# samuel-watson/glmmrMCML

Hardware: AMD Instinct MI355X
Metric: MCML iters/sec x m chains (simlik evals/sec) (higher is better)
Workload: dtype f64

## Files before the change

glmmrmcml_amd/api.py:

```python
import ctypes as C

import numpy as np

from . import _lib

c_dp = C.POINTER(C.c_double)
c_ip = C.POINTER(C.c_int32)

REDUCE_FN = C.CFUNCTYPE(C.c_int, C.c_void_p, C.c_void_p, C.c_int)


class Problem(C.Structure):
    _fields_ = [("cov", c_ip), ("cov_rows", C.c_int), ("data", c_dp), ("data_len", C.c_int),
                ("eff_range", c_dp), ("eff_len", C.c_int), ("Z", c_dp), ("X", c_dp), ("y", c_dp),
                ("n", C.c_int), ("Q", C.c_int), ("P", C.c_int), ("family", C.c_char_p),
                ("link", C.c_char_p)]


class DevOpts(C.Structure):
    _fields_ = [("device", C.c_int), ("stream", C.c_void_p), ("rank", C.c_int), ("world", C.c_int),
                ("reduce", REDUCE_FN), ("reduce_user", C.c_void_p)]


class HmcOpts(C.Structure):
# ... 62 lines not shown

def get_default_la_operator():
    return _LA_OP_NAME[_lib.lib().glmmr_mcml_get_default_la_operator()]


def la_component_launches():
    f = _lib.lib().glmmr_mcml_dbg_la_component_launches
    f.restype = C.c_longlong
    return int(f())


class _default_la_operator:

    def __init__(self, operator):
        self.operator = operator

    def __enter__(self):
        if self.operator is not None:
            self.prev = get_default_la_operator()
            set_default_la_operator(self.operator)

    def __exit__(self, *a):
        if self.operator is not None:
            set_default_la_operator(self.prev)


def traj_launches():
    f = _lib.lib().glmmr_mcml_dbg_traj_launches
    f.restype = C.c_longlong
    return int(f())


def dbg_dgemm_at(A, B, C0, K, alpha=1.0, beta=0.0, tile=-1):
    A = np.array(A, dtype=np.float64, order="F"); B = np.array(B, dtype=np.float64, order="F")
    K2 = K + (K & 1)
    assert A.shape[0] == K2 and B.shape[0] == K2, "operands hold round_up(K, 2) rows"
    M, N = A.shape[1], B.shape[1]
    out = B if C0 is None else np.array(C0, dtype=np.float64, order="F")
    assert C0 is None or out.shape == (M, N)
    _lib.check(_lib.lib().glmmr_mcml_dbg_dgemm_at(M, N, int(K), _p(A), K2, _p(B), K2, C.c_double(alpha), C.c_double(beta),
                                                  _p(out), out.shape[0], int(tile)))
    return out[:M]


def rccl_unique_id():
    buf = (C.c_ubyte * 128)()
    _lib.check(_lib.lib().glmmr_mcml_rccl_unique_id(buf))
    return bytes(buf)


def _f(a):
    return np.asfortranarray(np.asarray(a, dtype=np.float64))


def _i(a):
    return np.asfortranarray(np.asarray(a, dtype=np.int32))


def _p(a):
    return None if a is None else a.ctypes.data_as(c_dp)


class Context:

    def __init__(self, cov, data, eff_range, Z=None, X=None, y=None, family=None, link=None,
                 device=0, stream=None, rank=0, world=1, reduce=None):
        L = _lib.lib()
        self._cov = _i(cov)
        assert self._cov.ndim == 2 and self._cov.shape[1] == 5, "cov must be rows x 5"
        self._data = _f(data).ravel()
        self._eff = _f(eff_range).ravel()
        p = Problem()
        p.cov = self._cov.ctypes.data_as(c_ip); p.cov_rows = self._cov.shape[0]
        p.data = _p(self._data); p.data_len = self._data.size
        p.eff_range = _p(self._eff); p.eff_len = self._eff.size
        self.n = self.P = 0
        if Z is not None:
            self._Z = _f(Z); self._X = _f(X); self._y = _f(y).ravel()
            self.n, self.Q = self._Z.shape
            self.P = self._X.shape[1]
            assert self._X.shape[0] == self.n and self._y.size == self.n
            p.Z = _p(self._Z); p.X = _p(self._X); p.y = _p(self._y)
            p.n = self.n; p.Q = self.Q; p.P = self.P
            p.family = family.encode(); p.link = link.encode()
        o = DevOpts()
        o.device = device; o.stream = stream; o.rank = rank; o.world = world
        self._reduce_cb = REDUCE_FN(reduce) if reduce is not None else REDUCE_FN()
        o.reduce = self._reduce_cb
        self._h = C.c_void_p()
        self._world = int(world)
        _lib.check(L.glmmr_mcml_ctx_create(C.byref(p), C.byref(o), C.byref(self._h)))
        self.family, self.link = family, link
        if Z is None:
            self.Q = int(sum(self._cov[np.r_[True, self._cov[1:, 0] != self._cov[:-1, 0]], 1]))
        self.mcols = 0

    def close(self):
        if getattr(self, "_h", None) is not None and self._h.value:
            _lib.lib().glmmr_mcml_ctx_destroy(self._h)
            self._h = C.c_void_p()

    def __del__(self):
        try:
            self.close()
        except Exception:
            pass

    def __enter__(self):
        return self

    def __exit__(self, *a):
        self.close()

    def comm_init_rccl(self, unique_id, rank, world):
        buf = (C.c_ubyte * 128).from_buffer_copy(bytes(unique_id))
        _lib.check(_lib.lib().glmmr_mcml_ctx_comm_init_rccl(self._h, buf, int(rank), int(world)))
        self._world = int(world)

    def comm_allreduce(self, vals):
        v = np.ascontiguousarray(vals, dtype=np.float64).copy()
        _lib.check(_lib.lib().glmmr_mcml_ctx_comm_allreduce(self._h, _p(v), v.size))
        return v

    def comm_stats(self):
        calls = C.c_longlong(); dbl = C.c_longlong(); nat = C.c_int()
        _lib.check(_lib.lib().glmmr_mcml_ctx_comm_stats(self._h, C.byref(calls), C.byref(dbl), C.byref(nat)))
        return dict(calls=calls.value, doubles=dbl.value, native=bool(nat.value))

    def set_u(self, u, niter=None):
        u = _f(u)
        if u.ndim == 1:
            u = u.reshape(-1, 1, order="F")
        self.mcols = u.shape[1]
        _lib.check(_lib.lib().glmmr_mcml_set_u(self._h, _p(u), u.shape[0], u.shape[1],
                                               u.shape[1] if niter is None else niter))

    def get_u(self):
        u = np.zeros((self.Q, self.mcols), order="F")
        _lib.check(_lib.lib().glmmr_mcml_get_u(self._h, _p(u), self.Q))
        return u

    def get_u_all(self, world=None):
        w = int(world) if world else max(1, int(getattr(self, "_world", 1)))
        u = np.zeros((self.Q, self.mcols * w), order="F")
        nc = C.c_int()
        _lib.check(_lib.lib().glmmr_mcml_get_u_all(self._h, _p(u), self.Q, C.byref(nc)))
        assert nc.value == u.shape[1], (nc.value, u.shape)
        return u

    def shard_stats(self):
        out = (C.c_longlong * 6)()
        _lib.check(_lib.lib().glmmr_mcml_ctx_shard_stats(self._h, out))
        return dict(gathers=out[0], gather_doubles=out[1], theta_rounds=out[2], theta_evals_own=out[3],
                    theta_evals_all=out[4])

    def emulate_world(self, world, mode):
        _lib.check(_lib.lib().glmmr_mcml_dbg_emulate_world(self._h, int(world), int(mode)))
        self._world = int(world) if world and world > 1 else 1

    def mvn_ll(self, theta):
        theta = _f(theta).ravel()
        out = C.c_double()
        _lib.check(_lib.lib().glmmr_mcml_ctx_mvn_ll(self._h, _p(theta), C.byref(out)))
        return out.value

    def mvn_ll_batch(self, thetas):
        th = np.ascontiguousarray(np.atleast_2d(np.asarray(thetas, dtype=np.float64)))
        out = np.zeros(th.shape[0])
        _lib.check(_lib.lib().glmmr_mcml_ctx_mvn_ll_batch(self._h, _p(th), th.shape[0], _p(out)))
        return out

    def mvn_workspace(self, cand=-1):
        f = _lib.lib().glmmr_mcml_dbg_mvn_workspace
        dims = (C.c_int * 4)()
        _lib.check(f(self._h, int(cand), None, 0, None, 0, dims))
        d, m = dims[0], dims[2]
        L = np.zeros((d, d), order="F"); X = np.zeros((m, d), order="F")
        _lib.check(f(self._h, int(cand), _p(L), d, _p(X), m, dims))
        return L, X, tuple(dims)

    def dbg_chol(self, A, B=None, linv=True):
        A = np.array(A, dtype=np.float64, order="F")
        n = A.shape[0]
        assert A.shape == (n, n)
        out = dict(A=A)
        m = 0
        if B is not None:
            B = _f(B).reshape(n, -1, order="F")
            m = B.shape[1]
            for k in ("fwd", "trans", "potrs"):
                out[k] = np.zeros((n, m), order="F")
        nblk = (n + 127) // 128
        li = np.zeros((nblk, 128, 128)) if linv else None
        _lib.check(_lib.lib().glmmr_mcml_dbg_chol(self._h, n, _p(A), n, m, _p(B), n, _p(out.get("fwd")), _p(out.get("trans")),
                                                  _p(out.get("potrs")), _p(li)))
        if linv:
            out["linv"] = li.transpose(0, 2, 1)
        return out

    def gen_D(self, theta, chol=False):
        theta = _f(theta).ravel()
        D = np.zeros((self.Q, self.Q), order="F")
        _lib.check(_lib.lib().glmmr_mcml_ctx_gen_D(self._h, _p(theta), int(chol), _p(D), self.Q))
        return D

    def loglik(self, beta, var_par):
        beta = _f(beta).ravel()
        out = C.c_double()
        _lib.check(_lib.lib().glmmr_mcml_ctx_loglik(self._h, _p(beta), C.c_double(var_par), C.byref(out)))
        return out.value

    def mcnr(self, beta, var_par):
        beta = _f(beta).ravel()
        bout = np.zeros(self.P); sig = C.c_double()
        stats = np.zeros(self.P * self.P + self.P + 1)
        _lib.check(_lib.lib().glmmr_mcml_ctx_mcnr(self._h, _p(beta), C.c_double(var_par), _p(bout),
                                                  C.byref(sig), _p(stats)))
        P = self.P
        return dict(beta=bout, sigma=sig.value, XtWX=stats[:P * P].reshape(P, P, order="F"),
                    XtWr=stats[P * P:P * P + P], sigma_sum=stats[-1])

    def update_L(self, theta):
        theta = _f(theta).ravel()
        _lib.check(_lib.lib().glmmr_mcml_ctx_update_L(self._h, _p(theta)))

    def set_L(self, Lmat):
        Lmat = _f(Lmat)
        _lib.check(_lib.lib().glmmr_mcml_ctx_set_L(self._h, _p(Lmat), Lmat.shape[0]))

    def log_prob_grad(self, beta, var_par, V):
        beta = _f(beta).ravel(); V = _f(V)
        lp = np.zeros(V.shape[1]); G = np.zeros_like(V, order="F")
        _lib.check(_lib.lib().glmmr_mcml_dbg_log_prob_grad(self._h, _p(beta), C.c_double(var_par), _p(V),
                                                           V.shape[1], _p(lp), _p(G)))
        return lp, G

    def hmc_sample(self, beta, var_par, warmup, nsamp, lambda_, max_steps, target_accept, seed,
                   chains=1, chain_offset=0, iter_idx=0, adapt=100, inj_init=None, inj_mom=None,
                   want_trace=False):
        beta = _f(beta).ravel()
        o = HmcOpts(warmup, nsamp, adapt, lambda_, max_steps, target_accept, chains, chain_offset)
        d = HmcDiag()
        ii = None if inj_init is None else _f(inj_init)
        im = None if inj_mom is None else _f(inj_mom)
        total = warmup + (nsamp if chains == 1 else -(-nsamp // chains))
        flags = np.zeros((chains, total), dtype=np.uint8, order="F") if want_trace else None
        probs = np.zeros((chains, total), order="F") if want_trace else None
        ncols = C.c_int()
        _lib.check(_lib.lib().glmmr_mcml_ctx_hmc_sample(
            self._h, _p(beta), C.c_double(var_par), C.byref(o), C.c_uint64(seed), C.c_uint32(iter_idx),
            _p(ii), _p(im), None if flags is None else flags.ctypes.data_as(C.POINTER(C.c_uint8)),
            _p(probs), C.byref(d), C.byref(ncols)))
        self.mcols = ncols.value
        diag = dict(accept_rate=d.accept_rate, mean_e=d.mean_e, min_e=d.min_e, max_e=d.max_e,
                    max_steps_used=d.max_steps_used, leapfrog_total=d.leapfrog_total)
        if want_trace:
            return diag, flags, probs
        return diag

    def nuts_sample(self, beta, var_par, warmup, nsamp, seed, chains=1, chain_offset=0, iter_idx=0, max_treedepth=10,
                    adapt_delta=0.8, stepsize=1.0, want_trace=False, metric="diag_e"):
        beta = _f(beta).ravel()
        o = NutsOpts(warmup, nsamp, max_treedepth, adapt_delta, stepsize, chains, chain_offset,
                     {"diag_e": 0, "unit_e": 1}[metric])
        d = NutsDiag()
        total = warmup + -(-nsamp // chains)
        c_ip_ = C.POINTER(C.c_int)
        tr = None
        if want_trace:
            tr = dict(depth=np.zeros((chains, total), dtype=np.int32, order="F"),
                      nleap=np.zeros((chains, total), dtype=np.int32, order="F"),
                      eps=np.zeros((chains, total), order="F"), accept=np.zeros((chains, total), order="F"))
        ncols = C.c_int()
        _lib.check(_lib.lib().glmmr_mcml_ctx_nuts_sample(
            self._h, _p(beta), C.c_double(var_par), C.byref(o), C.c_uint64(seed), C.c_uint32(iter_idx),
            None if tr is None else tr["depth"].ctypes.data_as(c_ip_), None if tr is None else tr["nleap"].ctypes.data_as(c_ip_),
            None if tr is None else _p(tr["eps"]), None if tr is None else _p(tr["accept"]), C.byref(d), C.byref(ncols)))
        self.mcols = ncols.value
        diag = dict(mean_e=d.mean_e, min_e=d.min_e, max_e=d.max_e, divergent=d.divergent, treedepth_hits=d.treedepth_hits,
                    batched_leapfrogs=d.batched_leapfrogs, stepsize_search_leapfrogs=d.stepsize_search_leapfrogs,
                    packs=d.packs)
        return (diag, tr) if want_trace else diag

    def _ext(self, seed, chains, maxfun, theta_batch=0):
        return Ext(int(seed or 0), int(chains or 1), int(maxfun or 0), 0, int(theta_batch or 0))

    def npar(self):
        return _lib.lib().glmmr_mcml_ctx_npar(self._h)

    def theta_log(self, enable=None, last=None):
        w = self.npar() + 1
        n = C.c_int()
        _lib.check(_lib.lib().glmmr_mcml_dbg_theta_log(self._h, -1, None, 0, C.byref(n)))
        rows = n.value if last is None else min(int(last), n.value)
        out = np.zeros((rows, w))
        _lib.check(_lib.lib().glmmr_mcml_dbg_theta_log(self._h, -1 if enable is None else int(bool(enable)),
                                                       _p(out) if rows else None, rows, C.byref(n)))
        return out

    def last_kernels(self):
        names = {-1: None, 0: "skinny", 1: "band", 2: "dlds", 3: "reg", 4: "sparse", 5: "component", 6: "exact"}
        f = C.c_int(); b = C.c_int()
        _lib.check(_lib.lib().glmmr_mcml_ctx_last_kernels(self._h, C.byref(f), C.byref(b)))
        return names[f.value], names[b.value]

    def band_plan(self, chains, which="fwd"):
        out = (C.c_int * 10)()
# ... 339 lines not shown
```

glmmrmcml_amd/csrc/cabi.hip:

```cpp
#include "../../include/glmmr_mcml_c.h"
#include "ctx.h"
#include <algorithm>
#include <atomic>
#include <random>
#include "sparse_plan.h"

using namespace mcml;


namespace mcml {
int hmc_sample(Ctx& c, const double* beta, double var_par, const glmmr_mcml_hmc_opts* o, uint64_t seed,
               uint32_t iter_idx, const double* inj_init, const double* inj_mom, uint8_t* flags_out,
               double* probs_out, glmmr_mcml_hmc_diag* diag, int* ncols_out);
int nuts_sample(Ctx& c, const double* beta, double var_par, const glmmr_mcml_nuts_opts* o, uint64_t seed, uint32_t iter_idx,
                int* depth_out, int* nleap_out, double* eps_out, double* accept_out, glmmr_mcml_nuts_diag* diag,
                int* ncols_out);
bool hmc_exact_applicable(const Ctx& c);
int hmc_exact_sample(Ctx& c, const double* beta, double var_par, const glmmr_mcml_hmc_opts* o, uint64_t seed, uint32_t iter_idx,
                     const double* inj_z, glmmr_mcml_hmc_diag* diag, int* ncols_out);
}

static std::atomic<int> g_default_traj{-1};
static int default_trajectory()
{
// ... 230 lines not shown
    if (!sp.active) return MCML_OK;
    out12[1] = sp.factored ? 1 : 0; out12[2] = sp.W; out12[3] = sp.nnz; out12[4] = sp.nnz_z; out12[5] = sp.nnz_l;
    out12[6] = sp.nblk; out12[7] = sp.max_blk; out12[8] = cm_long_rows(c) ? 1 : 0; out12[9] = cm_fuse_width(c);
    return MCML_OK;
}

extern "C" int glmmr_mcml_set_default_trajectory(int mode)
{
    MCML_REQUIRE(mode == 0 || mode == 1, "set_default_trajectory: mode must be 0 (per step) or 1 (component)");
    g_default_traj.store(mode);
    return MCML_OK;
}

extern "C" int glmmr_mcml_get_default_trajectory(void) { return default_trajectory(); }

namespace mcml { long long cm_traj_launch_count(); }
extern "C" long long glmmr_mcml_dbg_traj_launches(void) { return cm_traj_launch_count(); }

extern "C" int glmmr_mcml_ctx_set_trajectory(glmmr_mcml_ctx* h, int mode)
{
    MCML_REQUIRE(h && (mode == 0 || mode == 1), "set_trajectory: mode must be 0 (per step) or 1 (component)");
    h->c.traj_mode = mode;
    return MCML_OK;
}

extern "C" int glmmr_mcml_dbg_component_plan(glmmr_mcml_ctx* h, int chains, long long* out11)
{
    MCML_REQUIRE(h && chains >= 1 && out11, "dbg_component_plan: bad argument");
    const Ctx& c = h->c;
    const ComponentPlan& p = c.cp.plan;
    for (int i = 0; i < 11; ++i) out11[i] = 0;
    out11[0] = c.traj_mode; out11[9] = CP_MAX_VARS;
    if (!c.sp.active) return MCML_OK;
    const bool feasible = c.cp.ready && p.feasible;
    out11[1] = feasible ? 1 : 0; out11[2] = (feasible && c.traj_mode == 1) ? 1 : 0;
    out11[3] = p.ncomp; out11[4] = p.max_vars; out11[5] = p.max_rows; out11[6] = p.empty_comps;
    if (!feasible) return MCML_OK;
    const int waves = cp_waves(p, cp_forced_waves());
    out11[7] = p.nitems(); out11[8] = waves; out11[10] = cp_lds_bytes(p.max_vars, waves);
    return MCML_OK;
}

extern "C" int glmmr_mcml_set_default_draws(int mode)
{
    MCML_REQUIRE(mode == 0 || mode == 1, "set_default_draws: mode must be 0 (hmc) or 1 (exact)");
    g_default_draws.store(mode);
    return MCML_OK;
}

extern "C" int glmmr_mcml_get_default_draws(void) { return default_draws(); }

extern "C" int glmmr_mcml_ctx_set_draws(glmmr_mcml_ctx* h, int mode)
{
    MCML_REQUIRE(h && (mode == 0 || mode == 1), "set_draws: mode must be 0 (hmc) or 1 (exact)");
    h->c.draws_mode = mode;
    return MCML_OK;
}

extern "C" int glmmr_mcml_dbg_draws_plan(glmmr_mcml_ctx* h, int* out4)
{
    MCML_REQUIRE(h && out4, "dbg_draws_plan: null argument");
    const Ctx& c = h->c;
    const long long bytes = (long long)sizeof(double) * pad_ld(c.Q) * c.Q;
    out4[0] = c.draws_mode; out4[1] = hmc_exact_applicable(c) ? 1 : 0; out4[2] = c.Q;
    out4[3] = bytes > 0x7fffffffLL ? 0x7fffffff : (int)bytes;
    return MCML_OK;
}

extern "C" int glmmr_mcml_ctx_exact_sample(glmmr_mcml_ctx* h, const double* beta, double var_par,
                                           const glmmr_mcml_hmc_opts* opts, uint64_t seed, uint32_t iter_idx,
                                           const double* inj_z, glmmr_mcml_hmc_diag* diag, int* ncols_out)
{
    MCML_REQUIRE(h && beta && opts, "exact_sample: null argument");
    MCML_HIP(hipSetDevice(h->c.device));
    return hmc_exact_sample(h->c, beta, var_par, opts, seed, iter_idx, inj_z, diag, ncols_out);
}

extern "C" int glmmr_mcml_dbg_exact_phases(glmmr_mcml_ctx* h, int enable, double* out5)
{
    MCML_REQUIRE(h, "dbg_exact_phases: null context");
    if (out5) for (int i = 0; i < 5; ++i) out5[i] = h->c.exact.ms[i];
    h->c.exact.prof = enable != 0;
    return MCML_OK;
}

extern "C" int glmmr_mcml_dbg_trsm_compare(glmmr_mcml_ctx* h, int m, int reps, double* trans_ms, double* fwd_ms)
{
    MCML_REQUIRE(h && m > 0 && reps > 0 && reps <= 64, "dbg_trsm_compare: bad argument");
    Ctx& c = h->c;
    MCML_HIP(hipSetDevice(c.device));
    MCML_REQUIRE(c.last_kernel[0] == KERNEL_EXACT && c.exact.M.d() && c.exact.M.rows == c.Q && c.U.d() && c.mcols >= m,
                 "dbg_trsm_compare: the last sampler call on this context must be an exact one with at least %d columns", m);
    DevMat T;
    MCML_TRY(T.alloc(c.Q, m));
    hipEvent_t e0, e1;
    MCML_HIP(hipEventCreate(&e0)); MCML_HIP(hipEventCreate(&e1));
    int rc = MCML_OK;
    for (int which = 0; which < 2 && rc == MCML_OK; ++which) {
        double* out = which ? fwd_ms : trans_ms;
        if (!out) continue;
        std::vector<float> ms;
        for (int r = 0; r < reps && rc == MCML_OK; ++r) {
            if (hipMemcpy2DAsync(T.d(), sizeof(double) * T.ld, c.U.d(), sizeof(double) * c.U.ld, sizeof(double) * c.Q, m,
                                 hipMemcpyDeviceToDevice, c.stream) != hipSuccess) { rc = MCML_EHIP; break; }
            (void)hipEventRecord(e0, c.stream);
            rc = which ? trsm_left_lower(c, c.exact.M.d(), c.exact.M.ld, c.Q, T.d(), T.ld, m)
                       : trsm_left_lower_trans(c, c.exact.M.d(), c.exact.M.ld, c.Q, T.d(), T.ld, m);
            (void)hipEventRecord(e1, c.stream);
            if (hipEventSynchronize(e1) != hipSuccess) rc = MCML_EHIP;
            float t = 0;
            if (rc == MCML_OK && hipEventElapsedTime(&t, e0, e1) == hipSuccess) ms.push_back(t);
        }
        if (rc == MCML_OK && !ms.empty()) { std::sort(ms.begin(), ms.end()); *out = ms[ms.size() / 2]; }
    }
    (void)hipEventDestroy(e0); (void)hipEventDestroy(e1);
    if (rc == MCML_EHIP) set_error("dbg_trsm_compare: HIP call failed");
    return rc;
}

extern "C" int glmmr_mcml_set_default_la_operator(int mode)
{
    MCML_REQUIRE(mode >= 0 && mode <= 2, "set_default_la_operator: mode must be 0 (dense), 1 (component) or 2 (component_wide)");
    g_default_la.store(mode);
    return MCML_OK;
}

extern "C" int glmmr_mcml_get_default_la_operator(void) { return default_la_operator(); }

extern "C" int glmmr_mcml_ctx_set_la_operator(glmmr_mcml_ctx* h, int mode)
{
    MCML_REQUIRE(h && mode >= 0 && mode <= 2, "set_la_operator: mode must be 0 (dense), 1 (component) or 2 (component_wide)");
    h->c.la_mode = mode;
    return MCML_OK;
}

namespace mcml { long long la_component_launch_count(); }
extern "C" long long glmmr_mcml_dbg_la_component_launches(void) { return la_component_launch_count(); }

extern "C" int glmmr_mcml_dbg_la_plan(glmmr_mcml_ctx* h, long long* out8)
{
    MCML_REQUIRE(h && out8, "dbg_la_plan: null argument");
    const Ctx& c = h->c;
    const ComponentPlan& p = c.cp.plan;
    const long long v[8] = {c.la_mode, c.la_last_op, p.ncomp, p.max_vars, p.max_rows, c.la_launches, c.la_dense_bytes, c.la_waves};
    for (int i = 0; i < 8; ++i) out8[i] = v[i];
    return MCML_OK;
}

extern "C" int glmmr_mcml_ctx_shard_stats(glmmr_mcml_ctx* h, long long* out6)
{
    MCML_REQUIRE(h && out6, "shard_stats: null argument");
    const Ctx& c = h->c;
    out6[0] = c.gather_calls; out6[1] = c.gather_doubles; out6[2] = c.theta_rounds; out6[3] = c.theta_evals_own;
    out6[4] = c.theta_evals_all; out6[5] = 0;
    return MCML_OK;
}

extern "C" int glmmr_mcml_dbg_emulate_world(glmmr_mcml_ctx* h, int world, int mode)
{
    MCML_REQUIRE(h, "emulate_world: null context");
    Ctx& c = h->c;
    MCML_REQUIRE(c.world <= 1 && !c.comm, "emulate_world: the context is rank %d of a real group of %d", c.rank, c.world);
    MCML_REQUIRE(world <= 1 || mode == 1 || mode == 2, "emulate_world: mode must be 1 (record) or 2 (replay)");
    if (world <= 1) { c.emu_world = 0; c.emu_mode = 0; c.emu_trace.clear(); c.emu_pos = 0; c.uall_valid = false; return MCML_OK; }
    if (c.emu_world != world) { c.emu_trace.clear(); c.uall_valid = false; }
    c.emu_world = world; c.emu_mode = mode; c.emu_pos = 0;
    if (mode == 1) c.emu_trace.clear();
    return MCML_OK;
}

extern "C" int glmmr_mcml_ctx_mvn_ll(glmmr_mcml_ctx* h, const double* theta, double* out)
{
    MCML_REQUIRE(h && theta && out, "mvn_ll: null argument");
    Ctx& c = h->c;
    MCML_HIP(hipSetDevice(c.device));
    double s = 0;
    MCML_TRY(mvn_loglik_sum(c, theta, &s));
    double tot[2] = {s, (double)c.mcols};
    MCML_TRY(allreduce_host(c, tot, 2));
    *out = tot[0] / tot[1];
    return MCML_OK;
}

extern "C" int glmmr_mcml_ctx_mvn_ll_batch(glmmr_mcml_ctx* h, const double* thetas, int k, double* out)
{
    MCML_REQUIRE(h && thetas && out && k >= 1 && k <= 64, "mvn_ll_batch: bad argument");
    Ctx& c = h->c;
    MCML_HIP(hipSetDevice(c.device));
    MCML_REQUIRE(c.mcols > 0 && c.U.d(), "mvn_ll: no samples set");
    std::vector<double> tot(k + 1, 0.0);
    std::vector<int> rcs(k, 0);
    MCML_TRY(mvn_loglik_batch(c, thetas, k, c.U.d(), c.U.ld, c.mcols, tot.data(), rcs.data()));
    for (int j = 0; j < k; ++j) if (rcs[j] == MCML_ENOTPD) tot[j] = NAN;
    tot[k] = (double)c.mcols;
    MCML_TRY(allreduce_host(c, tot.data(), k + 1));
    for (int j = 0; j < k; ++j) out[j] = tot[j] / tot[k];
    return MCML_OK;
}

extern "C" int glmmr_mcml_ctx_gen_D(glmmr_mcml_ctx* h, const double* theta, int chol, double* out, int ldo)
{
    MCML_REQUIRE(h && theta && out, "gen_D: null argument");
    Ctx& c = h->c;
    MCML_REQUIRE(ldo >= c.Q, "gen_D: ldo too small");
    MCML_HIP(hipSetDevice(c.device));
    MCML_TRY(mvn_gen_L(c, theta, chol != 0));
    return download_matrix(out, ldo, c.L.d(), c.L.ld, c.Q, c.Q, c.stream);
}

int mcml::mcnr_finish(int P, const double* stats, const double* beta, double* beta_out, double* sigma_out)
{
    const double m = stats[P * P + P + 1];
    MCML_REQUIRE(m > 0, "mcnr: no samples");
    std::vector<double> A(stats, stats + P * P), B((size_t)P * P, 0.0);
    for (auto& v : A) v *= (double)1 / m;
    for (int i = 0; i < P; i++) B[i + (size_t)i * P] = 1.0;
    for (int c = 0; c < P; c++) {
        int p = c; double best = fabs(A[c + (size_t)c * P]);
        for (int i = c + 1; i < P; i++) if (fabs(A[i + (size_t)c * P]) > best) { best = fabs(A[i + (size_t)c * P]); p = i; }
        if (best == 0.0 || best != best) { set_error("mcnr: X'WX is singular"); return MCML_ESINGULAR; }
        if (p != c) for (int j = 0; j < P; j++) { std::swap(A[c + (size_t)j * P], A[p + (size_t)j * P]); std::swap(B[c + (size_t)j * P], B[p + (size_t)j * P]); }
        double d = A[c + (size_t)c * P];
        for (int j = 0; j < P; j++) { A[c + (size_t)j * P] /= d; B[c + (size_t)j * P] /= d; }
        for (int i = 0; i < P; i++) if (i != c) {
            double f = A[i + (size_t)c * P];
            if (f != 0.0) for (int j = 0; j < P; j++) { A[i + (size_t)j * P] -= f * A[c + (size_t)j * P]; B[i + (size_t)j * P] -= f * B[c + (size_t)j * P]; }
        }
    }
    for (int a = 0; a < P; a++) {
        double inc = 0;
        for (int b = 0; b < P; b++) inc += B[a + (size_t)b * P] * (stats[P * P + b] / m);
        beta_out[a] = beta[a] + inc;
    }
    *sigma_out = stats[P * P + P] / m;
    return MCML_OK;
}

extern "C" int glmmr_mcml_ctx_loglik(glmmr_mcml_ctx* h, const double* beta, double var_par, double* out)
{
    MCML_REQUIRE(h && beta && out, "loglik: null argument");
    Ctx& c = h->c;
    MCML_HIP(hipSetDevice(c.device));
    MCML_TRY(model_update_beta(c, beta));
    double s = 0;
    MCML_TRY(model_loglik_sum(c, var_par, &s));
    double tot[2] = {s, (double)c.niter};
    MCML_TRY(allreduce_host(c, tot, 2));
    *out = tot[0] / tot[1];
    return MCML_OK;
}

extern "C" int glmmr_mcml_ctx_mcnr(glmmr_mcml_ctx* h, const double* beta, double var_par,
                                   double* beta_out, double* sigma_out, double* stats_out)
{
    MCML_REQUIRE(h && beta && beta_out && sigma_out, "mcnr: null argument");
    Ctx& c = h->c;
    MCML_HIP(hipSetDevice(c.device));
    MCML_TRY(model_update_beta(c, beta));
    std::vector<double> st((size_t)c.P * c.P + c.P + 2);
    MCML_TRY(model_mcnr_stats(c, var_par, st.data()));
    if (stats_out) memcpy(stats_out, st.data(), sizeof(double) * ((size_t)c.P * c.P + c.P + 1));
    return mcnr_finish(c.P, st.data(), beta, beta_out, sigma_out);
}

extern "C" int glmmr_mcml_ctx_update_L(glmmr_mcml_ctx* h, const double* theta)
{
    MCML_REQUIRE(h && theta, "update_L: null argument");
    Ctx& c = h->c;
    MCML_HIP(hipSetDevice(c.device));
    MCML_TRY(mvn_gen_L(c, theta, true));
    MCML_TRY(model_update_L(c));
    return c.sync();
}

extern "C" int glmmr_mcml_ctx_set_L(glmmr_mcml_ctx* h, const double* L, int ldl)
{
    MCML_REQUIRE(h && L, "set_L: null argument");
    Ctx& c = h->c;
    MCML_REQUIRE(ldl >= c.Q, "set_L: ldl too small");
    MCML_HIP(hipSetDevice(c.device));
    MCML_TRY(upload_matrix(c.L, L, c.Q, c.Q, ldl, c.stream));
    c.have_L = true;
    c.l_foreign = true;
    MCML_TRY(model_update_L(c));
    return c.sync();
}

extern "C" int glmmr_mcml_ctx_hmc_sample(glmmr_mcml_ctx* h, const double* beta, double var_par,
                                         const glmmr_mcml_hmc_opts* opts, uint64_t seed, uint32_t iter_idx,
                                         const double* inj_init, const double* inj_mom, uint8_t* flags_out,
                                         double* probs_out, glmmr_mcml_hmc_diag* diag, int* ncols_out)
{
    MCML_REQUIRE(h && beta && opts, "hmc_sample: null argument");
    MCML_HIP(hipSetDevice(h->c.device));
    return hmc_sample(h->c, beta, var_par, opts, seed, iter_idx, inj_init, inj_mom, flags_out, probs_out,
                      diag, ncols_out);
}

extern "C" int glmmr_mcml_ctx_nuts_sample(glmmr_mcml_ctx* h, const double* beta, double var_par,
                                          const glmmr_mcml_nuts_opts* opts, uint64_t seed, uint32_t iter_idx,
                                          int* depth_out, int* nleap_out, double* eps_out, double* accept_out,
                                          glmmr_mcml_nuts_diag* diag, int* ncols_out)
{
    MCML_REQUIRE(h && beta && opts, "nuts_sample: null argument");
    MCML_HIP(hipSetDevice(h->c.device));
    return nuts_sample(h->c, beta, var_par, opts, seed, iter_idx, depth_out, nleap_out, eps_out, accept_out, diag,
                       ncols_out);
}

extern "C" int glmmr_mcml_dbg_log_prob_grad(glmmr_mcml_ctx* h, const double* beta, double var_par,
                                            const double* V, int ncols, double* lp, double* G)
{
    MCML_REQUIRE(h && beta && V && lp && G && ncols > 0, "log_prob_grad: bad argument");
    MCML_HIP(hipSetDevice(h->c.device));
    return hmc_dbg_log_prob_grad(h->c, beta, var_par, V, ncols, lp, G);
}

extern "C" int glmmr_mcml_mvn_ll(const int32_t* cov, int cov_rows, const double* data, int data_len,
                                 const double* eff_range, int eff_len, const double* gamma, int ngamma,
                                 const double* u, int Q, int m, double* out)
{
    glmmr_mcml_problem p{};
    p.cov = cov; p.cov_rows = cov_rows; p.data = data; p.data_len = data_len;
    p.eff_range = eff_range; p.eff_len = eff_len; p.Q = Q;
    glmmr_mcml_ctx* h = nullptr;
    MCML_TRY(glmmr_mcml_ctx_create(&p, nullptr, &h));
    int rc = MCML_OK;
    if (ngamma < h->c.cov.npar) {
        set_error("mvn_ll: %d covariance parameters given, the functions need %d", ngamma, h->c.cov.npar);
        rc = MCML_EINVAL;
    }
    if (!rc) rc = glmmr_mcml_set_u(h, u, Q, m, m);
    if (!rc) rc = glmmr_mcml_ctx_mvn_ll(h, gamma, out);
    glmmr_mcml_ctx_destroy(h);
    return rc;
}

namespace mcml {
int drv_optim(Ctx& c, const double* start, int nstart, int trace, int mcnr, const glmmr_mcml_ext* e,
              double* beta, double* theta, double* sigma);
int drv_simlik(Ctx& c, const double* start, int nstart, int trace, const glmmr_mcml_ext* e, double* beta,
               double* theta, double* sigma);
int drv_hess(Ctx& c, const double* start, int nstart, double tol, int trace, double* H);
int drv_aic(Ctx& c, const double* beta_par, int nbeta, const double* cov_par, int ncov, double* out);
int drv_full(Ctx& c, const double* start, int nstart, int mcnr, int m, int maxiter, int warmup, double tol,
             int verbose, double lambda, int trace, int refresh, int maxsteps, double target_accept,
             const glmmr_mcml_ext* e, double* beta_out, double* theta_out, double* sigma_out,
             int* converged_out, int* iters_out, glmmr_mcml_hmc_diag* last_diag);
int drv_la(Ctx& c, const double* start, int nstart, int nr, int usehess, double tol, int verbose, int trace,
           int maxiter, const glmmr_mcml_ext* e, double* beta, double* theta, double* sigma, double* se, double* u,
           int* converged, int* iters);
int drv_la_probe(Ctx& c, const double* start, int nstart, int kind, const double* v, double var_par,
                 const double* par, int npar, double* out, double* v_out, double* beta_out, double* sigma_out);
}

extern "C" int glmmr_mcml_sample_cols(int m, int chains)
{
    if (m <= 0) return 0;
    if (chains <= 1) return m + 1;
    return chains * ((m + chains - 1) / chains);
}

extern "C" int glmmr_mcml_ctx_profile(glmmr_mcml_ctx* h, int enable, int reset, double* out8)
{
    MCML_REQUIRE(h, "profile: null context");
    Ctx& c = h->c;
    KernelProf& p = c.prof;
    if (out8) {
        out8[0] = p.ms[0]; out8[1] = (double)p.cnt[0]; out8[2] = p.ms[1]; out8[3] = (double)p.cnt[1];
        const double C = (double)c.hmc.C, dense = 2.0 * c.n * (double)c.Q * C;
        double ff = dense, fb = dense, kind = 0;
        if (c.sp.active) { ff = fb = 2.0 * (double)c.sp.nnz * C; kind = 2; }
        else {
            if (c.band_fwd) { ff = 2.0 * 80.0 * 32.0 * (double)c.band_fwd_tiles * C; kind = 1; }
            if (c.band_bwd) { fb = 2.0 * 80.0 * 32.0 * (double)c.band_bwd_tiles * C; kind = 1; }
        }
        out8[4] = ff; out8[5] = fb; out8[6] = dense; out8[7] = kind;
    }
    if (reset) for (int i = 0; i < 4; ++i) { p.ms[i] = 0; p.cnt[i] = 0; p.seen[i] = 0; }
    if (enable && !p.on) {
        MCML_HIP(hipSetDevice(c.device));
        while (p.ev.size() < 4096) { hipEvent_t e; if (hipEventCreate(&e) != hipSuccess) { (void)hipGetLastError(); break; } p.ev.push_back(e); }
    }
    p.on = enable != 0;
    return MCML_OK;
}

extern "C" int glmmr_mcml_ctx_profile_launches(glmmr_mcml_ctx* h, long long* fwd, long long* bwd)
{
    MCML_REQUIRE(h, "profile_launches: null context");
    if (fwd) *fwd = h->c.prof.seen[0];
    if (bwd) *bwd = h->c.prof.seen[1];
    return MCML_OK;
}

extern "C" int glmmr_mcml_ctx_ncols(glmmr_mcml_ctx* h) { return h ? h->c.mcols : 0; }
extern "C" int glmmr_mcml_ctx_npar(glmmr_mcml_ctx* h) { return h ? h->c.cov.npar : 0; }

extern "C" int glmmr_mcml_ctx_optim(glmmr_mcml_ctx* h, const double* start, int nstart, int trace, int mcnr,
                                    const glmmr_mcml_ext* ext, double* beta, double* theta, double* sigma)
{
    MCML_REQUIRE(h && start && beta && theta && sigma, "optim: null argument");
    MCML_REQUIRE(h->c.n > 0, "optim: context has no model");
    MCML_HIP(hipSetDevice(h->c.device));
    return drv_optim(h->c, start, nstart, trace, mcnr, ext, beta, theta, sigma);
}

extern "C" int glmmr_mcml_ctx_simlik(glmmr_mcml_ctx* h, const double* start, int nstart, int trace,
                                     const glmmr_mcml_ext* ext, double* beta, double* theta, double* sigma)
{
    MCML_REQUIRE(h && start && beta && theta && sigma, "simlik: null argument");
    MCML_REQUIRE(h->c.n > 0, "simlik: context has no model");
    MCML_HIP(hipSetDevice(h->c.device));
    return drv_simlik(h->c, start, nstart, trace, ext, beta, theta, sigma);
}

extern "C" int glmmr_mcml_ctx_hess(glmmr_mcml_ctx* h, const double* start, int nstart, double tol, int trace,
                                   double* H)
{
    MCML_REQUIRE(h && start && H, "hess: null argument");
    MCML_REQUIRE(h->c.n > 0 && tol > 0, "hess: context has no model / bad tol");
    MCML_HIP(hipSetDevice(h->c.device));
    return drv_hess(h->c, start, nstart, tol, trace, H);
}

extern "C" int glmmr_mcml_ctx_aic(glmmr_mcml_ctx* h, const double* beta_par, int nbeta, const double* cov_par,
                                  int ncov, double* out)
{
    MCML_REQUIRE(h && beta_par && cov_par && out, "aic: null argument");
    MCML_REQUIRE(h->c.n > 0, "aic: context has no model");
    MCML_HIP(hipSetDevice(h->c.device));
    return drv_aic(h->c, beta_par, nbeta, cov_par, ncov, out);
}

extern "C" int glmmr_mcml_ctx_full(glmmr_mcml_ctx* h, const double* start, int nstart, int mcnr, int m,
                                   int maxiter, int warmup, double tol, int verbose, double lambda, int trace,
                                   int refresh, int maxsteps, double target_accept, const glmmr_mcml_ext* ext,
                                   double* beta, double* theta, double* sigma, int* converged, int* iters,
                                   glmmr_mcml_hmc_diag* diag)
{
    MCML_REQUIRE(h && start && beta && theta && sigma, "mcml_full: null argument");
    MCML_REQUIRE(h->c.n > 0, "mcml_full: context has no model");
    MCML_HIP(hipSetDevice(h->c.device));
    return drv_full(h->c, start, nstart, mcnr, m, maxiter, warmup, tol, verbose, lambda, trace, refresh, maxsteps,
                    target_accept, ext, beta, theta, sigma, converged, iters, diag);
}

extern "C" int glmmr_mcml_ctx_la(glmmr_mcml_ctx* h, const double* start, int nstart, int nr, int usehess, double tol,
                                 int verbose, int trace, int maxiter, const glmmr_mcml_ext* ext, double* beta,
                                 double* theta, double* sigma, double* se, double* u, int* converged, int* iters)
{
    MCML_REQUIRE(h && start && beta && theta && sigma, "mcml_la: null argument");
    MCML_HIP(hipSetDevice(h->c.device));
    return drv_la(h->c, start, nstart, nr, usehess, tol, verbose, trace, maxiter, ext, beta, theta, sigma, se, u,
                  converged, iters);
}

extern "C" int glmmr_mcml_dbg_leaf_profile(glmmr_mcml_ctx* h, unsigned long long* out10)
{
    MCML_REQUIRE(h && out10, "leaf_profile: null argument");
    return potrf_leaf_profile(h->c, out10);
}

extern "C" int glmmr_mcml_dbg_la_probe(glmmr_mcml_ctx* h, const double* start, int nstart, int kind, const double* v,
                                       double var_par, const double* par, int npar, double* out, double* v_out,
                                       double* beta_out, double* sigma_out)
{
    MCML_REQUIRE(h && start, "la_probe: null argument");
    MCML_REQUIRE(kind >= 0 && kind <= 3, "la_probe: kind %d", kind);
    MCML_REQUIRE(kind == 3 ? (v_out && beta_out && sigma_out) : (par && out && npar > 0), "la_probe: null output");
    MCML_HIP(hipSetDevice(h->c.device));
    return drv_la_probe(h->c, start, nstart, kind, v, var_par, par, npar, out, v_out, beta_out, sigma_out);
}

namespace {
struct CtxGuard {
    glmmr_mcml_ctx* h = nullptr;
    ~CtxGuard() { if (h) glmmr_mcml_ctx_destroy(h); }
};
int open_ctx(const glmmr_mcml_problem* prob, const glmmr_mcml_ext* ext, CtxGuard& g)
{
    glmmr_mcml_dev_opts o{};
    o.device = ext ? ext->device : 0; o.world = 1;
    return glmmr_mcml_ctx_create(prob, &o, &g.h);
}
int check_pattern(const Ctx& c, const int32_t* Ap, const int32_t* Ai, int nnz)
{
    MCML_REQUIRE(Ap && Ai && nnz >= 0, "sparse: null pattern");
    std::vector<int> blk(c.Q);
    for (int b = 0; b < c.cov.B; ++b) for (int k = 0; k < c.cov.blocks[b].dim; ++k) blk[c.cov.blocks[b].matstart + k] = b;
    MCML_REQUIRE(Ap[0] == 0 && Ap[c.Q] == nnz, "sparse: Ap does not describe %d columns / %d entries", c.Q, nnz);
    for (int j = 0; j < c.Q; ++j)
        for (int p = Ap[j]; p < Ap[j + 1]; ++p) {
            MCML_REQUIRE(Ai[p] >= 0 && Ai[p] < c.Q, "sparse: row index out of range");
            MCML_REQUIRE(blk[Ai[p]] == blk[j], "sparse: entry (%d,%d) lies outside the covariance blocks", Ai[p], j);
        }
    return MCML_OK;
}
}

extern "C" int glmmr_mcml_optim(const glmmr_mcml_problem* prob, const double* u, int ucols, const double* start,
                                int nstart, int trace, int mcnr, const glmmr_mcml_ext* ext, double* beta,
                                double* theta, double* sigma)
{
    CtxGuard g;
    MCML_TRY(open_ctx(prob, ext, g));
    MCML_TRY(glmmr_mcml_set_u(g.h, u, prob->Q, ucols, ucols));
    return glmmr_mcml_ctx_optim(g.h, start, nstart, trace, mcnr, ext, beta, theta, sigma);
}

extern "C" int glmmr_mcml_simlik(const glmmr_mcml_problem* prob, const double* u, int ucols, const double* start,
                                 int nstart, int trace, const glmmr_mcml_ext* ext, double* beta, double* theta,
                                 double* sigma)
{
    CtxGuard g;
    MCML_TRY(open_ctx(prob, ext, g));
    MCML_TRY(glmmr_mcml_set_u(g.h, u, prob->Q, ucols, ucols));
    return glmmr_mcml_ctx_simlik(g.h, start, nstart, trace, ext, beta, theta, sigma);
}

static int sparse_factor_nnz(const Ctx& c)
{
    long nnz = 0;
    for (const auto& b : c.cov.blocks) if (!b.all_gr) nnz += (long)b.dim * (b.dim - 1) / 2;
    return (int)nnz;
}

extern "C" int glmmr_mcml_sparse_factor_nnz(const int32_t* cov, int cov_rows, const double* data, int data_len)
{
    CovSpec cs;
    if (cs.parse(cov, cov_rows, data, data_len, nullptr, 0)) return -1;
    long nnz = 0;
    for (const auto& b : cs.blocks) if (!b.all_gr) nnz += (long)b.dim * (b.dim - 1) / 2;
    return (int)nnz;
}

static int sparse_factor(Ctx& c, const double* theta, int32_t* Lp, int32_t* Li, double* Lx, double* D)
{
    MCML_TRY(mvn_gen_L(c, theta, true));
    std::vector<double> blk;
    int nz = 0;
    for (const auto& b : c.cov.blocks) {
        blk.assign((size_t)b.dim * b.dim, 0.0);
        MCML_TRY(download_matrix(blk.data(), b.dim, c.L.at(b.matstart, b.matstart), c.L.ld, b.dim, b.dim, c.stream));
        for (int j = 0; j < b.dim; ++j) {
            const double d = blk[j + (size_t)j * b.dim];
            Lp[b.matstart + j] = nz;
            D[b.matstart + j] = d * d;
            if (!b.all_gr)
                for (int i = j + 1; i < b.dim; ++i) { Li[nz] = b.matstart + i; Lx[nz] = blk[i + (size_t)j * b.dim] / d; ++nz; }
        }
    }
    Lp[c.Q] = nz;
    return MCML_OK;
}

extern "C" int glmmr_mcml_optim_sparse(const glmmr_mcml_problem* prob, const int32_t* Ap, const int32_t* Ai,
                                       int nnz, const double* u, int ucols, const double* start, int nstart,
                                       int trace, int mcnr, const glmmr_mcml_ext* ext, double* beta, double* theta,
                                       double* sigma, int32_t* Lp, int32_t* Li, double* Lx, double* D, int lcap)
{
    CtxGuard g;
    MCML_TRY(open_ctx(prob, ext, g));
    MCML_TRY(check_pattern(g.h->c, Ap, Ai, nnz));
    MCML_TRY(glmmr_mcml_set_u(g.h, u, prob->Q, ucols, ucols));
    MCML_TRY(glmmr_mcml_ctx_optim(g.h, start, nstart, trace, mcnr, ext, beta, theta, sigma));
    if (Lp && Li && Lx && D) {
        MCML_REQUIRE(lcap >= sparse_factor_nnz(g.h->c), "optim_sparse: factor needs %d entries, %d given",
                     sparse_factor_nnz(g.h->c), lcap);
        MCML_TRY(sparse_factor(g.h->c, theta, Lp, Li, Lx, D));
    }
    return MCML_OK;
}

extern "C" int glmmr_mcml_simlik_sparse(const glmmr_mcml_problem* prob, const int32_t* Ap, const int32_t* Ai,
                                        int nnz, const double* u, int ucols, const double* start, int nstart,
// ... 174 lines not shown
```

glmmrmcml_amd/csrc/covspec.h:

```cpp
#pragma once
#include "common.h"

namespace mcml {

constexpr int MAX_COV_PAR = 32;
struct ThetaArg { double v[MAX_COV_PAR]; };

struct CovBlock {
    int dim;
    int r0, r1;
    int ncol;
    int doff;
    int matstart;
    int all_gr;
};

struct CovSpec {
    int rows = 0, B = 0, N = 0, npar = 0;
    std::vector<int32_t> cov;
    std::vector<double> data;
    std::vector<double> eff;
    std::vector<CovBlock> blocks;

    static int fn_npar(int fn) {
        static const int t[15] = {0, 1, 1, 1, 2, 2, 1, 2, 2, 2, 2, 2, 2, 2, 1};
        return (fn >= 1 && fn <= 14) ? t[fn] : -1;
    }
    static bool fn_built(int fn) { return fn == 1 || fn == 2 || fn == 3 || fn == 4 || fn == 7 || fn == 14; }
    int c(int r, int col) const { return cov[r + (size_t)col * rows]; }

    int parse(const int32_t* cov_, int rows_, const double* data_, int data_len,
              const double* eff_, int eff_len)
    {
        MCML_REQUIRE(cov_ && rows_ > 0, "cov: empty");
        rows = rows_;
        cov.assign(cov_, cov_ + (size_t)rows * 5);
        eff.assign(eff_ ? eff_ : nullptr, eff_ ? eff_ + (eff_len > 0 ? eff_len : 0) : nullptr);
        blocks.clear();
        N = 0; npar = 0;
        int r = 0;
        size_t doff = 0;
        while (r < rows) {
            CovBlock b{};
            b.dim = c(r, 1); b.r0 = r; b.ncol = 0; b.all_gr = 1; b.matstart = N; b.doff = (int)doff;
            MCML_REQUIRE(b.dim > 0, "cov row %d: block dimension %d", r, b.dim);
            int id = c(r, 0);
            while (r < rows && c(r, 0) == id) {
                int fn = c(r, 2), nv = c(r, 3), pi = c(r, 4);
                MCML_REQUIRE(c(r, 1) == b.dim, "cov row %d: dimension differs within block", r);
                if (fn_npar(fn) < 0 || !fn_built(fn)) {
                    set_error("cov row %d: covariance function id %d is not built (gr, fexp0, ar1, "
                              "sqexp, fexp, sqexp0 only)", r, fn);
                    return MCML_EUNSUPPORTED;
                }
                MCML_REQUIRE(nv >= 0 && pi >= 0, "cov row %d: negative field", r);
                MCML_REQUIRE(pi + fn_npar(fn) <= MAX_COV_PAR, "more than %d covariance parameters", MAX_COV_PAR);
                if (pi + fn_npar(fn) > npar) npar = pi + fn_npar(fn);
                if (fn != 1) b.all_gr = 0;
                b.ncol += nv;
                ++r;
            }
            b.r1 = r;
            doff += (size_t)b.dim * b.ncol;
            N += b.dim;
            blocks.push_back(b);
        }
        B = (int)blocks.size();
        MCML_REQUIRE((size_t)data_len >= doff, "data has %d values, the blocks need %zu", data_len, doff);
        data.assign(data_, data_ + doff);
        return MCML_OK;
    }
};

__host__ __device__ static inline double cov_term(int fn, double dist, const double* g, double val)
{
    switch (fn) {
    case 1: return (dist == 0) ? val * g[0] * g[0] : 0.0;
    case 2: return val * exp(-1.0 * dist / g[0]);
    case 3: return val * pow(g[0], dist);
    case 4: return val * g[0] * exp(-1.0 * dist * dist / (g[1] * g[1]));
    case 7: return val * g[0] * exp(-1.0 * dist / g[1]);
    case 14: return val * exp(-1.0 * dist * dist / (g[0] * g[0]));
    }
    return val;
}

}
```

glmmrmcml_amd/csrc/ctx.h:

```cpp
#pragma once
#include "common.h"
#include "covspec.h"
#include "band_plan.h"
#include "component_plan.h"
#include "step_ahead.h"

namespace mcml {

constexpr int CHOL_NB = 128;
constexpr int SMALL_BLOCK = 32;

typedef int (*reduce_fn)(void* user, double* dev_buf, int n);

enum { KERNEL_SKINNY = 0, KERNEL_BAND = 1, KERNEL_DLDS = 2, KERNEL_REG = 3, KERNEL_SPARSE = 4, KERNEL_COMPONENT = 5,
       KERNEL_EXACT = 6 };

struct StepRing {
    static constexpr int SLOTS = StepAhead::SLOTS;
    unsigned long long* h = nullptr;
    unsigned long long* d = nullptr;
    unsigned seq = 0;
    StepRing() = default;
    StepRing(const StepRing&) = delete;
    StepRing& operator=(const StepRing&) = delete;
// ... 57 lines not shown
        if (nev >= ev.size())
            for (int i = 0; i < 512; ++i) { hipEvent_t e; if (hipEventCreate(&e) != hipSuccess) return -1; ev.push_back(e); }
        return (int)nev++;
    }
    int begin(hipStream_t s, int k, bool chain = false) {
        if (!on) return -1;
        ++seen[k];
        if (skip) return -1;
        int st = (chain && last_stop >= 0) ? last_stop : fresh();
        if (st < 0) return -1;
        if (!(chain && last_stop >= 0)) (void)hipEventRecord(ev[st], s);
        if (used >= kind.size()) { kind.resize(used + 512); e0.resize(used + 512); e1.resize(used + 512); }
        kind[used] = k; e0[used] = st; e1[used] = -1;
        return (int)used++;
    }
    void end(hipStream_t s, int slot) {
        if (slot < 0) return;
        const int sp = fresh();
        if (sp < 0) return;
        (void)hipEventRecord(ev[sp], s);
        e1[slot] = sp; last_stop = sp;
    }
    void unchain() { last_stop = -1; }
    void collect() {
        for (size_t i = 0; i < used; ++i) {
            float t = 0;
            if (e1[i] >= 0 && hipEventElapsedTime(&t, ev[e0[i]], ev[e1[i]]) == hipSuccess) { ms[kind[i]] += t; cnt[kind[i]] += 1; }
        }
        used = 0; nev = 0; last_stop = -1;
    }
    ~KernelProf() { for (auto e : ev) (void)hipEventDestroy(e); }
};

struct CholGraph {
    hipGraphExec_t exec = nullptr;
    const double* A = nullptr; const double* linv = nullptr; int lda = 0, n = 0, extra = 0, seen = 0;
    long long used = 0;
    hipGraph_t tmpl = nullptr;
    hipEvent_t t0 = nullptr, t1 = nullptr;
    float eager_ms = 0.f, best_ms = 0.f;
    hipGraphExec_t best = nullptr;
    int tries = 0, trial_launches = 0;
    bool timed = false, settled = false;
    void release() {
        if (best && best != exec) (void)hipGraphExecDestroy(best);
        best = nullptr;
        if (exec) { (void)hipGraphExecDestroy(exec); exec = nullptr; }
        if (tmpl) { (void)hipGraphDestroy(tmpl); tmpl = nullptr; }
        if (t0) { (void)hipEventDestroy(t0); t0 = nullptr; }
        if (t1) { (void)hipEventDestroy(t1); t1 = nullptr; }
    }
};
struct CholGraphCache {
    static constexpr int CAP = 2;
    std::vector<CholGraph> g;
    long long tick = 0;
    void clear() { for (CholGraph& e : g) e.release(); g.clear(); }
    ~CholGraphCache() { clear(); }
    CholGraphCache() = default;
    CholGraphCache(const CholGraphCache&) = delete;
    CholGraphCache& operator=(const CholGraphCache&) = delete;
    CholGraphCache(CholGraphCache&& o) noexcept : g(std::move(o.g)), tick(o.tick) { o.g.clear(); }
    CholGraphCache& operator=(CholGraphCache&& o) noexcept { if (this != &o) { clear(); g = std::move(o.g); tick = o.tick; o.g.clear(); } return *this; }
    CholGraph& find(const double* A, const double* linv, int lda, int n, int extra) {
        ++tick;
        for (CholGraph& e : g)
            if (e.A == A && e.linv == linv && e.lda == lda && e.n == n && e.extra == extra) { e.used = tick; return e; }
        size_t old = 0;
        for (size_t i = 1; i < g.size(); ++i)
            if (g[i].used < g[old].used) old = i;
        if ((int)g.size() >= CAP) {
            g[old].release();
            g[old] = CholGraph();
            std::swap(g[old], g.back());
        } else g.push_back(CholGraph());
        CholGraph& e = g.back();
        e.A = A; e.linv = linv; e.lda = lda; e.n = n; e.extra = extra; e.seen = 0; e.used = tick;
        return e;
    }
};

struct ExactState {
    DevMat M, T;
    DevBuf b;
    bool prof = false;
    double ms[5] = {0, 0, 0, 0, 0};
};

struct Ctx {
    int device = 0;
    hipStream_t stream = nullptr;
    bool own_stream = false;

    int n = 0, Q = 0, P = 0, flink = 0, link_code = 0;
    int z_width = 0;
    DevBuf z_idx, z_val;
    std::vector<int> h_zidx; std::vector<double> h_zval;
    SparseZL sp;
    ComponentDev cp;
    int traj_mode = 0;
    int draws_mode = 0;
    ExactState exact;
    bool no_sparse_zl = false;
    int la_mode = 0;
    int la_last_op = 0;
    int la_waves = 0;
    long long la_launches = 0, la_dense_bytes = 0;
    bool l_foreign = false;
    CovSpec cov;
    DevMat Z, X;
    DevBuf y;
    DevBuf d_cov, d_data, d_blocks, d_rowblock;

    DevMat U;
    int mcols = 0;
    int niter = 0;
    int m_global = 0, niter_global = 0;
    DevMat ZU;
    bool zu_valid = false;

    DevMat L, ZL, ZLT;
    BandPlan plan_fwd, plan_bwd;
    DevBuf kr_scratch;
    bool band_fwd = false, band_bwd = false;
    long band_fwd_tiles = 0, band_bwd_tiles = 0;
    DevBuf xb;
    bool have_L = false;

    DevMat Dwork;
    DevBuf linv;
    DevBuf partials;
    DevBuf scalars;
    int* errflag() const { return reinterpret_cast<int*>(scalars.d() + 16); }
    int maxdim_large = 0;
    int n_small = 0, n_diag_rows = 0;
    DevBuf small_ids;

    int last_kernel[2] = {-1, -1};
    HmcState hmc;
    NutsState nuts;
    KernelProf prof;

    int rank = 0, world = 1;
    reduce_fn reduce = nullptr;
    void* reduce_user = nullptr;
    void* comm = nullptr;
    long long coll_calls = 0, coll_doubles = 0;
    long long gather_calls = 0, gather_doubles = 0;
    DevMat Uall;
    bool uall_valid = false;
    bool theta_log_on = false;
    std::vector<double> theta_log;
    long long theta_rounds = 0, theta_evals_own = 0, theta_evals_all = 0;
    int emu_world = 0, emu_mode = 0;
    std::vector<std::vector<double>> emu_trace; size_t emu_pos = 0;
    DevBuf reduce_buf;
    DevBuf scratch;

    hipStream_t aux = nullptr;
    hipStream_t aux_lo = nullptr;
    hipEvent_t ev_col = nullptr, ev_leaf = nullptr;
    CholGraphCache chol_graphs;
    std::vector<hipEvent_t> ev_ring;
    DevMat Dbatch;
    DevBuf bscal;
    struct MvnWs { int d = 0, dp = 0, m = 0, ld = 0, kb = 0; } mvn_ws[2];
    ~Ctx() {
        for (hipEvent_t e : ev_ring) if (e) (void)hipEventDestroy(e);
        comm_release_hook();
        if (ev_col) (void)hipEventDestroy(ev_col);
        if (ev_leaf) (void)hipEventDestroy(ev_leaf);
        if (aux) (void)hipStreamDestroy(aux);
        if (aux_lo) (void)hipStreamDestroy(aux_lo);
    }

    int sync() { MCML_HIP(hipStreamSynchronize(stream)); return MCML_OK; }
    void comm_release_hook();
};

void comm_release(Ctx& c);
int allreduce_dev(Ctx& c, double* dev, int n);
int allgather_dev(Ctx& c, const double* send, double* recv, size_t count);
int gather_samples(Ctx& c);
inline int comm_world(const Ctx& c) { return c.emu_world > 1 ? c.emu_world : c.world; }
inline void Ctx::comm_release_hook() { comm_release(*this); }

int mvn_setup(Ctx& c);
int mvn_loglik_sum(Ctx& c, const double* theta, double* sum_out);
int mvn_loglik_sum_on(Ctx& c, const double* theta, const double* U, int ldu, int m, double* sum_out);
int mvn_loglik_batch(Ctx& c, const double* thetas, int k, const double* U, int ldu, int m, double* sums, int* rcs);
int mvn_gen_L(Ctx& c, const double* theta, bool chol);
int potrf_lower(Ctx& c, double* A, int n, int lda);
int potrf_leaf_profile(Ctx& c, unsigned long long* host10);
int potrf_lower_checked(Ctx& c, double* A, int n, int lda);
int potrs_lower_vec(Ctx& c, const double* L, int ldl, int n, double* x, double* tmp);
int trsm_left_lower(Ctx& c, const double* L, int ldl, int n, double* U, int ldu, int m);
int trsm_left_lower_trans(Ctx& c, const double* R, int ldr, int n, double* T, int ldt, int m);

int build_M_dense(Ctx& c, const double* W, double w0, DevMat& M, DevMat& ZLTW, bool lower_only);

int model_setup(Ctx& c, const double* Z, const double* X, const double* y);
int allreduce_host(Ctx& c, double* vals, int n);
int model_update_beta(Ctx& c, const double* beta);
int model_update_zu(Ctx& c);
int model_update_L(Ctx& c);
int model_sparse_setup(Ctx& c);
int model_loglik_sum(Ctx& c, double var_par, double* sum_out);
int model_mcnr_stats(Ctx& c, double var_par, double* stats );
int mcnr_finish(int P, const double* stats, const double* beta, double* beta_out, double* sigma_out);

struct glmmr_mcml_hmc_opts_fwd;
int hmc_dbg_log_prob_grad(Ctx& c, const double* beta, double var_par, const double* V, int ncols, double* lp,
                          double* G);

int device_sum(Ctx& c, const double* partials, int n, double* dev_out);

}

struct glmmr_mcml_ctx { mcml::Ctx c; };
```

glmmrmcml_amd/csrc/debug_hooks.hip:

```cpp
#include "dgemm_mfma.h"
#include "dgemm_dl.h"
#include "dgemm_band.h"

using namespace mcml;

extern "C" int glmmr_mcml_dbg_dgemm(int M, int N, int K, const double* A, int lda,
                                    const double* B, int ldb, int b_nmajor,
                                    double alpha, double beta, double* C, int ldc,
                                    int lower_only, int force_tile)
{
    int ndev = 0;
    if (hipGetDeviceCount(&ndev) != hipSuccess || ndev == 0) {
        set_error("no HIP device: libglmmr_mcml_hip has no CPU fallback");
        return MCML_ENODEVICE;
    }
    hipStream_t s = nullptr;
    DevMat dA, dB, dC;
    if (force_tile == 40) {
        MCML_REQUIRE(!b_nmajor && !lower_only, "dbg_dgemm: the direct-to-LDS kernel takes a K-major B and all tiles");
        const int kpad = round_up(K, 32);
        MCML_TRY(dA.alloc(M, K, 32));
        MCML_HIP(hipMemset(dA.d(), 0, sizeof(double) * (size_t)dA.ld * dA.cols_alloc));
        MCML_HIP(hipMemcpy2D(dA.d(), sizeof(double) * dA.ld, A, sizeof(double) * lda, sizeof(double) * M, K, hipMemcpyHostToDevice));
        MCML_TRY(dB.alloc(kpad, N));
// ... 130 lines not shown
    BandPlan plan;
    plan.reset(M, K, hk);
    if (tiles_executed) *tiles_executed = (int)plan.tiles;
    EpiAxpby epi{dC.d(), dC.ld, 1.0, 0.0};
    MCML_TRY(launch_gemm_band(s, plan, N, dA.d(), dA.ld, dB.d(), dB.ld, epi));
    MCML_TRY(download_matrix(C, ldc, dC.d(), dC.ld, M, N, s));
    return MCML_OK;
}

extern "C" int glmmr_mcml_dbg_band_clocks(int M, int N, int iters, int mode, double* out3)
{
    int ndev = 0;
    if (hipGetDeviceCount(&ndev) != hipSuccess || ndev == 0) {
        set_error("no HIP device: libglmmr_mcml_hip has no CPU fallback");
        return MCML_ENODEVICE;
    }
    hipStream_t s = nullptr;
    if (getenv("GLMMR_MCML_DBG_STREAM")) MCML_HIP(hipStreamCreateWithFlags(&s, hipStreamNonBlocking));
    std::vector<double> hA((size_t)M * M, 0.0), hB((size_t)M * N);
    uint64_t x = 88172645463325252ULL;
    auto rnd = [&]() { x ^= x << 13; x ^= x >> 7; x ^= x << 17; return (double)(x >> 11) / 9007199254740992.0 * 2 - 1; };
    const bool cst = getenv("GLMMR_MCML_DBG_DATA") && !strcmp(getenv("GLMMR_MCML_DBG_DATA"), "const");
    const bool dec = getenv("GLMMR_MCML_DBG_DATA") && !strcmp(getenv("GLMMR_MCML_DBG_DATA"), "decay");
    for (int j = 0; j < M; ++j) for (int i = j; i < M; ++i) hA[i + (size_t)j * M] = cst ? 1.0 : dec ? rnd() * std::exp(-(double)(i - j) / 40.0) : rnd();
    for (auto& v : hB) v = cst ? 1.0 : rnd();
    DevMat dA, dB, dC;
    MCML_TRY(dA.alloc(M, M, 32));
    MCML_HIP(hipMemset(dA.d(), 0, sizeof(double) * (size_t)dA.ld * dA.cols_alloc));
    MCML_HIP(hipMemcpy2D(dA.d(), sizeof(double) * dA.ld, hA.data(), sizeof(double) * M, sizeof(double) * M, M, hipMemcpyHostToDevice));
    MCML_TRY(dB.alloc(round_up(M, 32), N));
    MCML_HIP(hipMemset(dB.d(), 0, sizeof(double) * (size_t)dB.ld * N));
    MCML_HIP(hipMemcpy2D(dB.d(), sizeof(double) * dB.ld, hB.data(), sizeof(double) * M, sizeof(double) * M, N, hipMemcpyHostToDevice));
    MCML_TRY(dC.alloc(M, N));
    const int nbands = (M + BD_BM - 1) / BD_BM;
    DevBuf kr, clk;
    MCML_TRY(kr.ensure(sizeof(int) * 2 * nbands));
    MCML_TRY(clk.ensure(16));
    MCML_HIP(hipMemset(clk.p, 0, 16));
    hipLaunchKernelGGL(k_band_ranges, dim3(nbands), dim3(256), 0, s, dA.d(), dA.ld, M, M, kr.as<int>());
    std::vector<int> hk(2 * nbands);
    MCML_HIP(hipMemcpy(hk.data(), kr.p, sizeof(int) * 2 * nbands, hipMemcpyDeviceToHost));
    BandPlan plan;
    plan.reset(M, M, hk);
    const double tiles = (double)plan.tiles;
    EpiAxpby epi{dC.d(), dC.ld, 1.0, 0.0};
    if (mode < 0) {
        for (int i = 0; i < 3; i++)
            MCML_TRY((launch_gemm_band<EpiAxpby, false>(s, plan, N, dA.d(), dA.ld, dB.d(), dB.ld, epi)));
        hipEvent_t f0, f1;
        MCML_HIP(hipEventCreate(&f0));
        MCML_HIP(hipEventCreate(&f1));
        MCML_HIP(hipEventRecord(f0, s));
        for (int i = 0; i < iters; i++)
            MCML_TRY((launch_gemm_band<EpiAxpby, false>(s, plan, N, dA.d(), dA.ld, dB.d(), dB.ld, epi)));
        MCML_HIP(hipEventRecord(f1, s));
        MCML_HIP(hipEventSynchronize(f1));
        float fms = 0;
        MCML_HIP(hipEventElapsedTime(&fms, f0, f1));
        out3[0] = fms / iters; out3[1] = 0;
        out3[2] = 2.0 * 80.0 * 32.0 * tiles * N / (fms / iters * 1e-3) / 1e12;
        (void)hipEventDestroy(f0);
        (void)hipEventDestroy(f1);
        return MCML_OK;
    }
    if (mode & 16) {
        BandPlanDev* d = nullptr;
        MCML_TRY(plan.device_plan((N + BD_BN - 1) / BD_BN, s, &d));
        const int nb = d->nwg * d->gn;
        DevBuf st;
        MCML_TRY(st.ensure(sizeof(unsigned long long) * (8 + 8 * (size_t)nb)));
        for (int rep = 0; rep < 3; ++rep) {
            MCML_HIP(hipMemset(st.p, 0, sizeof(unsigned long long) * (8 + 8 * (size_t)nb)));
            MCML_TRY((launch_gemm_band<EpiAxpby, true>(s, plan, N, dA.d(), dA.ld, dB.d(), dB.ld, epi, st.as<unsigned long long>(), mode)));
            MCML_HIP(hipDeviceSynchronize());
        }
        std::vector<unsigned long long> h(8 + 8 * (size_t)nb);
        MCML_HIP(hipMemcpy(h.data(), st.p, sizeof(unsigned long long) * h.size(), hipMemcpyDeviceToHost));
        unsigned long long t0 = ~0ULL;
        for (int w = 0; w < nb; ++w) if (h[8 + 8 * w] && h[8 + 8 * w] < t0) t0 = h[8 + 8 * w];
        double mx[5] = {0, 0, 0, 0, 0}, sm[5] = {0, 0, 0, 0, 0};
        for (int w = 0; w < nb; ++w)
            for (int i = 0; i < 5; ++i) { double v = (double)(h[8 + 8 * w + i] - t0) * 0.01; sm[i] += v; if (v > mx[i]) mx[i] = v; }
        printf("band stamps (us from the first workgroup's start; %d workgroups, mean / max):\n", nb);
        const char* nm[5] = {"start", "ring filled", "K loop done", "epilogue issued", "end"};
        for (int i = 0; i < 5; ++i) printf("  %-16s %7.2f / %7.2f\n", nm[i], sm[i] / nb, mx[i]);
        if (mode & 32) for (int w = 0; w < nb; ++w) {
            printf("  wg %3d:", w);
            for (int i = 0; i < 5; ++i) printf(" %7.2f", (double)(h[8 + 8 * w + i] - t0) * 0.01);
            printf("\n");
        }
        fflush(stdout);
        out3[0] = out3[1] = out3[2] = 0;
        return MCML_OK;
    }
    for (int i = 0; i < 3; i++)
        MCML_TRY((launch_gemm_band<EpiAxpby, true>(s, plan, N, dA.d(), dA.ld, dB.d(), dB.ld, epi)));
    hipEvent_t e0, e1;
    MCML_HIP(hipEventCreate(&e0));
    MCML_HIP(hipEventCreate(&e1));
    MCML_HIP(hipEventRecord(e0, s));
    for (int i = 0; i < iters; i++)
        MCML_TRY((launch_gemm_band<EpiAxpby, true>(s, plan, N, dA.d(), dA.ld, dB.d(), dB.ld, epi, clk.as<unsigned long long>(), mode)));
    MCML_HIP(hipEventRecord(e1, s));
    MCML_HIP(hipEventSynchronize(e1));
    float ms = 0;
    MCML_HIP(hipEventElapsedTime(&ms, e0, e1));
    unsigned long long hc[2] = {0, 0};
    MCML_HIP(hipMemcpy(hc, clk.p, 16, hipMemcpyDeviceToHost));
    out3[0] = ms / iters;
    out3[1] = hc[1] ? (double)hc[0] / (double)hc[1] * 100.0 : 0.0;
    out3[2] = 2.0 * 80.0 * 32.0 * tiles * N / (ms / iters * 1e-3) / 1e12;
    (void)hipEventDestroy(e0);
    (void)hipEventDestroy(e1);
    return MCML_OK;
}

extern "C" const char* glmmr_mcml_last_error(void) { return mcml::last_error(); }

#include "rng.h"
__global__ void k_dbg_normals(uint64_t seed, uint32_t chain, uint32_t prop, uint32_t tag, int n, double* out)
{
    int i = blockIdx.x * blockDim.x + threadIdx.x;
    if (i < n) out[i] = rng_normal(seed, (uint32_t)i, chain, prop, tag);
}
__global__ void k_dbg_minstd(uint32_t seed, int n, double* out)
{
    if (threadIdx.x || blockIdx.x) return;
    uint32_t x = seed % 2147483647u;
    if (x == 0) x = 1;
    for (int i = 0; i < n; ++i) out[i] = minstd_canonical(x);
}
extern "C" int glmmr_mcml_dbg_normals(uint64_t seed, uint32_t chain, uint32_t prop, uint32_t tag, int n,
                                      double* out)
{
    DevBuf b;
    MCML_TRY(b.ensure(sizeof(double) * (size_t)n));
    hipLaunchKernelGGL(k_dbg_normals, dim3((n + 255) / 256), dim3(256), 0, nullptr, seed, chain, prop, tag, n, b.d());
    MCML_HIP(hipGetLastError());
    MCML_HIP(hipMemcpy(out, b.p, sizeof(double) * (size_t)n, hipMemcpyDeviceToHost));
    return MCML_OK;
}
extern "C" int glmmr_mcml_dbg_minstd(uint32_t seed, int n, double* out)
{
    DevBuf b;
    MCML_TRY(b.ensure(sizeof(double) * (size_t)n));
    hipLaunchKernelGGL(k_dbg_minstd, dim3(1), dim3(64), 0, nullptr, seed, n, b.d());
    MCML_HIP(hipGetLastError());
    MCML_HIP(hipMemcpy(out, b.p, sizeof(double) * (size_t)n, hipMemcpyDeviceToHost));
    return MCML_OK;
}

#include "../../include/glmmr_mcml_c.h"
#include "optim.h"
#include <cmath>
extern "C" int glmmr_mcml_dbg_bobyqa(glmmr_mcml_objective f, void* user, int n, const double* x0,
                                     const double* lower, const double* upper, double rhobeg, double rhoend,
                                     int maxfun, double* x_out, double* f_out, int* nfev_out)
{
    MCML_REQUIRE(f && n > 0 && x0 && x_out, "dbg_bobyqa: bad argument");
    objective_fn obj = [&](const std::vector<double>& x, double* v) { *v = f(x.data(), n, user); return 0; };
    std::vector<double> x(x0, x0 + n), lo(n, -HUGE_VAL), up(n, HUGE_VAL);
    if (lower) lo.assign(lower, lower + n);
    if (upper) up.assign(upper, upper + n);
    BobyqaOpts o; o.rhobeg = rhobeg; o.rhoend = rhoend; if (maxfun > 0) o.maxfun = maxfun;
    BobyqaResult r;
    MCML_TRY(bobyqa(obj, x, lo, up, o, &r));
    for (int i = 0; i < n; ++i) x_out[i] = r.x[i];
    if (f_out) *f_out = r.fval;
    if (nfev_out) *nfev_out = r.nfev;
    return MCML_OK;
}
extern "C" int glmmr_mcml_dbg_bobyqa_batch(glmmr_mcml_objective f, void* user, int n, const double* x0,
                                           const double* lower, const double* upper, double rhobeg, double rhoend,
                                           int maxfun, int width, double* x_out, double* f_out, int* nfev_out,
                                           int* rounds_out)
{
    MCML_REQUIRE(f && n > 0 && x0 && x_out && width >= 1, "dbg_bobyqa_batch: bad argument");
    batch_objective_fn obj = [&](const std::vector<std::vector<double>>& X, std::vector<double>* F) {
        F->resize(X.size());
        for (size_t i = 0; i < X.size(); ++i) (*F)[i] = f(X[i].data(), n, user);
        return 0; };
    std::vector<double> x(x0, x0 + n), lo(n, -HUGE_VAL), up(n, HUGE_VAL);
    if (lower) lo.assign(lower, lower + n);
    if (upper) up.assign(upper, upper + n);
    BobyqaOpts o; o.rhobeg = rhobeg; o.rhoend = rhoend; if (maxfun > 0) o.maxfun = maxfun;
    BobyqaResult r;
    MCML_TRY(bobyqa_batch(obj, x, lo, up, o, width, &r));
    for (int i = 0; i < n; ++i) x_out[i] = r.x[i];
    if (f_out) *f_out = r.fval;
    if (nfev_out) *nfev_out = r.nfev;
    if (rounds_out) *rounds_out = r.rounds;
    return MCML_OK;
}
extern "C" int glmmr_mcml_dbg_bobyqa_rounds(glmmr_mcml_batch_objective fb, void* user, int n, const double* x0,
                                            const double* lower, const double* upper, double rhobeg, double rhoend,
                                            int maxfun, int width, double* x_out, double* f_out, int* nfev_out,
                                            int* rounds_out)
{
    MCML_REQUIRE(fb && n > 0 && x0 && x_out && width >= 1, "dbg_bobyqa_rounds: bad argument");
    batch_objective_fn obj = [&](const std::vector<std::vector<double>>& X, std::vector<double>* F) {
        const int k = (int)X.size();
        std::vector<double> flat((size_t)n * k);
        for (int j = 0; j < k; ++j) for (int i = 0; i < n; ++i) flat[(size_t)j * n + i] = X[j][i];
        F->assign(k, 0.0);
        return fb(flat.data(), n, k, F->data(), user); };
    std::vector<double> x(x0, x0 + n), lo(n, -HUGE_VAL), up(n, HUGE_VAL);
    if (lower) lo.assign(lower, lower + n);
    if (upper) up.assign(upper, upper + n);
    BobyqaOpts o; o.rhobeg = rhobeg; o.rhoend = rhoend; if (maxfun > 0) o.maxfun = maxfun;
    BobyqaResult r;
    MCML_TRY(bobyqa_batch(obj, x, lo, up, o, width, &r));
    for (int i = 0; i < n; ++i) x_out[i] = r.x[i];
    if (f_out) *f_out = r.fval;
    if (nfev_out) *nfev_out = r.nfev;
    if (rounds_out) *rounds_out = r.rounds;
    return MCML_OK;
}
extern "C" int glmmr_mcml_dbg_fd_hessian(glmmr_mcml_objective f, void* user, int n, const double* x, double ndeps,
                                         int usebounds, const double* lower, const double* upper, double* H)
{
    MCML_REQUIRE(f && n > 0 && x && H, "dbg_fd_hessian: bad argument");
    objective_fn obj = [&](const std::vector<double>& xx, double* v) { *v = f(xx.data(), n, user); return 0; };
    std::vector<double> xv(x, x + n), nd(n, ndeps), lo(n, -HUGE_VAL), up(n, HUGE_VAL), h;
    if (lower) lo.assign(lower, lower + n);
    if (upper) up.assign(upper, upper + n);
    MCML_TRY(fd_hessian(obj, xv, nd, usebounds != 0, lo, up, &h));
    for (int i = 0; i < n * n; ++i) H[i] = h[i];
    return MCML_OK;
}

extern "C" int glmmr_mcml_dbg_copy_roundtrip(const double* in, long long ld_in, double* out, long long ld_out, long long rows, long long cols)
{
    MCML_REQUIRE(in && out && rows > 0 && cols > 0 && ld_in >= rows && ld_out >= rows, "copy_roundtrip: bad arguments");
    const size_t ldd = (size_t)rows + 3;
    DevBuf buf;
    MCML_TRY(buf.ensure(sizeof(double) * ldd * (size_t)cols));
    MCML_HIP(hipMemset(buf.p, 0xff, sizeof(double) * ldd * (size_t)cols));
    MCML_TRY(copy_h2d_2d(buf.p, sizeof(double) * ldd, in, sizeof(double) * (size_t)ld_in, sizeof(double) * (size_t)rows, (size_t)cols, 0));
    MCML_TRY(copy_d2h_2d(out, sizeof(double) * (size_t)ld_out, buf.p, sizeof(double) * ldd, sizeof(double) * (size_t)rows, (size_t)cols, 0));
    MCML_HIP(hipDeviceSynchronize());
    return MCML_OK;
}
```

glmmrmcml_amd/csrc/drivers.hip:

```cpp
#include "../../include/glmmr_mcml_c.h"
#include "ctx.h"
#include "optim.h"
#include "trace.h"
#include <algorithm>
#include <cmath>
#include <cstring>
#include <map>
#include <memory>
#include <random>

namespace mcml {

int hmc_sample(Ctx& c, const double* beta, double var_par, const glmmr_mcml_hmc_opts* o, uint64_t seed,
               uint32_t iter_idx, const double* inj_init, const double* inj_mom, uint8_t* flags_out,
               double* probs_out, glmmr_mcml_hmc_diag* diag, int* ncols_out);

static bool is_gaussian(int flink) { return flink == 7 || flink == 8; }
static bool has_var_par(int flink) { return flink == 7 || flink == 8 || flink == 12; }

static int eval_loglik(Ctx& c, const double* beta, double var_par, double* ll)
{
    MCML_TRY(model_update_beta(c, beta));
    double s = 0;
    MCML_TRY(model_loglik_sum(c, var_par, &s));
    double tot[2] = {s, (double)c.niter};
    MCML_TRY(allreduce_host(c, tot, 2));
    *ll = tot[0] / tot[1];
    return MCML_OK;
}

static int eval_mvn(Ctx& c, const double* theta, double* logl)
{
    double s = 0;
    int rc = mvn_loglik_sum(c, theta, &s);
    if (rc == MCML_ENOTPD) { *logl = -HUGE_VAL; return MCML_OK; }
    MCML_TRY(rc);
    double tot[2] = {s, (double)c.mcols};
    MCML_TRY(allreduce_host(c, tot, 2));
    *logl = tot[0] / tot[1];
    if (c.theta_log_on) { c.theta_log.insert(c.theta_log.end(), theta, theta + c.cov.npar); c.theta_log.push_back(*logl); }
    return MCML_OK;
}

struct McmlOptim {
    Ctx& c;
    int P, R;
    std::vector<double> beta, theta, cov_par_fix;
    double sigma;
    int trace, maxfun;
    int theta_batch = 0;
    double model_var_par;

    McmlOptim(Ctx& ctx, const double* start, int trace_, int maxfun_, double var_par0)
        : c(ctx), P(ctx.P), R(ctx.cov.npar), trace(trace_), maxfun(maxfun_), model_var_par(var_par0)
    {
        beta.assign(start, start + P);
        theta.assign(start + P, start + P + R);
        cov_par_fix = theta;
        sigma = is_gaussian(c.flink) ? start[P + R] : 0;
    }

    BobyqaOpts bopts() const { BobyqaOpts o; o.iprint = trace; if (maxfun > 0) o.maxfun = maxfun; return o; }

    int d_optim_sharded(int width)
    {
        MCML_TRY(gather_samples(c));
        const int wr = comm_world(c), mall = c.mcols * wr;
        batch_objective_fn fb = [&](const std::vector<std::vector<double>>& Zs, std::vector<double>* F) -> int {
            const int nc = (int)Zs.size();
            std::vector<double> vals(nc, 0.0);
            const bool emu = c.world <= 1 && !c.comm && c.emu_world > 1;
            int first_rc = MCML_OK;
            const int r_lo = (emu && c.emu_mode == 1) ? 0 : c.rank, r_hi = (emu && c.emu_mode == 1) ? wr : c.rank + 1;
            for (int rr = r_lo; rr < r_hi; ++rr) {
                std::vector<int> own;
                for (int j = 0; j < nc; ++j) if ((j % wr) == rr) own.push_back(j);
                if (own.empty()) continue;
                std::vector<double> ths((size_t)R * own.size()), sums(own.size(), 0.0);
                std::vector<int> rcs(own.size(), 0);
                for (size_t q = 0; q < own.size(); ++q)
                    for (int i = 0; i < R; ++i) ths[q * R + i] = std::exp(Zs[own[q]][i]);
                const int brc = mvn_loglik_batch(c, ths.data(), (int)own.size(), c.Uall.d(), c.Uall.ld, mall, sums.data(), rcs.data());
                for (size_t q = 0; q < own.size(); ++q) {
                    const int j = own[q];
                    const int rc = (rcs[q] == MCML_OK && brc != MCML_OK) ? brc : rcs[q];
                    if (rc != MCML_OK && getenv("GLMMR_MCML_BOBYQA_TRACE")) fprintf(stderr, "theta-step: candidate %d (theta %.6g %.6g) rc %d brc %d: %s\n", j, ths[q * R], R > 1 ? ths[q * R + 1] : 0.0, rcs[q], brc, last_error());
                    if (rc == MCML_ENOTPD) vals[j] = HUGE_VAL;
                    else if (rc != MCML_OK) { vals[j] = NAN; if (first_rc == MCML_OK) first_rc = rc; }
                    else vals[j] = -1 * (sums[q] / mall);
                    if (rr == c.rank) ++c.theta_evals_own;
                    if (c.theta_log_on && rc == MCML_OK) { c.theta_log.insert(c.theta_log.end(), ths.begin() + q * R, ths.begin() + (q + 1) * R); c.theta_log.push_back(sums[q] / mall); }
                }
            }
            c.theta_rounds += 1; c.theta_evals_all += nc;
            if (!emu) MCML_TRY(allreduce_host(c, vals.data(), nc));
            else if (c.emu_mode == 1) c.emu_trace.push_back(vals);
            else {
                MCML_REQUIRE(c.emu_pos < c.emu_trace.size() && (int)c.emu_trace[c.emu_pos].size() == nc,
                             "rank emulation: replay ran past its record (round %zu)", c.emu_pos);
                const std::vector<double>& rec = c.emu_trace[c.emu_pos++];
                for (int j = 0; j < nc; ++j) {
                    if ((j % wr) == c.rank) MCML_REQUIRE(vals[j] == rec[j] || (vals[j] != vals[j]), "rank emulation: replayed value differs from the recorded one (%.17g vs %.17g)", vals[j], rec[j]);
                    else vals[j] = rec[j];
                }
            }
            if (first_rc != MCML_OK) return first_rc;
            for (double v : vals)
                if (v != v) { set_error("theta-step: a rank failed to evaluate its candidate"); return MCML_EHIP; }
            *F = vals;
            return MCML_OK; };
        std::vector<double> z(R), lo(R, std::log(1e-6)), up(R, HUGE_VAL);
        for (int i = 0; i < R; ++i) z[i] = std::log(std::max(theta[i], 1e-6));
        BobyqaOpts o = bopts();
        o.rhobeg = 0.25; o.rhoend = 1e-7;
        BobyqaResult r;
        MCML_TRY(bobyqa_batch(fb, z, lo, up, o, width, &r));
        for (int i = 0; i < R; ++i) theta[i] = std::exp(r.x[i]);
        return MCML_OK;
    }

    int d_optim()
    {
        static const bool shard = !(getenv("GLMMR_MCML_THETA_SHARD") && !strcmp(getenv("GLMMR_MCML_THETA_SHARD"), "0"));
        const int wr = comm_world(c);
        const bool dense_only = c.maxdim_large > 0 && c.n_small == 0 && c.n_diag_rows == 0;
        const int k = wr > 1 ? (theta_batch > 0 ? theta_batch : dense_only ? std::max(1, 8 / wr) : 1) : batch_width();
        if ((wr > 1 && shard) || k > 1) return d_optim_sharded(wr * std::max(1, k));
        objective_fn f = [&](const std::vector<double>& par, double* v) {
            double logl; MCML_TRY(eval_mvn(c, par.data(), &logl)); *v = -1 * logl; return (int)MCML_OK; };
        std::vector<double> lo(R, 1e-6), up(R, HUGE_VAL);
        BobyqaResult r;
        MCML_TRY(bobyqa(f, theta, lo, up, bopts(), &r));
        theta = r.x;
        return MCML_OK;
    }

    int l_optim()
    {
        if (c.flink == 12) { set_error("l_optim: beta family is not built (reference reads par[P] out of range, defect D8)"); return MCML_EUNSUPPORTED; }
        const bool g = is_gaussian(c.flink);
        objective_fn f = [&](const std::vector<double>& par, double* v) {
            model_var_par = has_var_par(c.flink) ? par[P] : 0.0;
            double ll; MCML_TRY(eval_loglik(c, par.data(), model_var_par, &ll)); *v = -1 * ll; return (int)MCML_OK; };
        std::vector<double> x = beta, lo(P, -HUGE_VAL), up(P, HUGE_VAL);
        if (g) { x.push_back(sigma); lo.push_back(0.0); up.push_back(HUGE_VAL); }
        BobyqaResult r;
        MCML_TRY(bobyqa(f, x, lo, up, bopts(), &r));
        beta.assign(r.x.begin(), r.x.begin() + P);
        if (g) sigma = r.x[P];
        return MCML_OK;
    }

    int mcnr()
    {
        MCML_TRY(model_update_beta(c, beta.data()));
        std::vector<double> st((size_t)P * P + P + 2), nb(P);
        MCML_TRY(model_mcnr_stats(c, model_var_par, st.data()));
        double s = 0;
        MCML_TRY(mcnr_finish(P, st.data(), beta.data(), nb.data(), &s));
        beta = nb; sigma = s;
        return MCML_OK;
    }

    typedef std::map<std::vector<double>, double> ThetaMemo;
    objective_fn make_F(bool importance, double fix_var_par, double denomD, bool memoise = false,
                        std::shared_ptr<ThetaMemo> memo = std::make_shared<ThetaMemo>())
    {
        return [this, importance, fix_var_par, denomD, memoise, memo](const std::vector<double>& par, double* v) {
            model_var_par = fix_var_par;
            double ll, logl;
            MCML_TRY(eval_loglik(c, par.data(), model_var_par, &ll));
            if (memoise) {
                const std::vector<double> th(par.begin() + P, par.begin() + P + R);
                auto it = memo->find(th);
                if (it != memo->end()) logl = it->second;
                else { MCML_TRY(eval_mvn(c, th.data(), &logl)); (*memo)[th] = logl; }
            } else
            MCML_TRY(eval_mvn(c, par.data() + P, &logl));
            *v = importance ? -1.0 * (ll + logl - denomD) : -1.0 * (ll + logl);
            return (int)MCML_OK; };
    }

    int batch_width() const
    {
        if (theta_batch > 0) return theta_batch;
        static const int envk = getenv("GLMMR_MCML_THETA_BATCH") ? atoi(getenv("GLMMR_MCML_THETA_BATCH")) : 0;
        if (envk > 0) return envk;
        return (c.maxdim_large > 0 && c.n_small == 0 && c.n_diag_rows == 0) ? 8 : 1;
    }

    int f_optim_batch(int width, double denomD)
    {
        const double fix_var_par = sigma;
        batch_objective_fn fb = [&](const std::vector<std::vector<double>>& Zs, std::vector<double>* F) -> int {
            const int nc = (int)Zs.size();
            std::vector<double> ths((size_t)R * nc), sums(nc, 0.0);
            std::vector<int> rcs(nc, 0);
            for (int j = 0; j < nc; ++j) for (int i = 0; i < R; ++i) ths[(size_t)j * R + i] = std::exp(Zs[j][P + i]);
            MCML_TRY(mvn_loglik_batch(c, ths.data(), nc, c.U.d(), c.U.ld, c.mcols, sums.data(), rcs.data()));
            F->assign(nc, 0.0);
            for (int j = 0; j < nc; ++j) {
                model_var_par = fix_var_par;
                double ll = 0;
                MCML_TRY(eval_loglik(c, Zs[j].data(), model_var_par, &ll));
                const double logl = rcs[j] == MCML_OK ? sums[j] / c.mcols : -HUGE_VAL;
                (*F)[j] = -1.0 * (ll + logl - denomD);
            }
            return MCML_OK; };
        std::vector<double> x = beta, lo(P, -HUGE_VAL), up;
        for (int i = 0; i < R; ++i) { x.push_back(std::log(std::max(theta[i], 1e-6))); lo.push_back(std::log(1e-6)); }
        up.assign(x.size(), HUGE_VAL);
        BobyqaOpts o = bopts();
        o.rhobeg = 0.25; o.rhoend = 1e-7;
        BobyqaResult r;
        MCML_TRY(bobyqa_batch(fb, x, lo, up, o, width, &r));
        beta.assign(r.x.begin(), r.x.begin() + P);
        for (int i = 0; i < R; ++i) theta[i] = std::exp(r.x[P + i]);
        return MCML_OK;
    }

    int f_optim()
    {
        const bool g = is_gaussian(c.flink);
        double denomD = 0;
        MCML_TRY(eval_mvn(c, cov_par_fix.data(), &denomD));
        if (comm_world(c) == 1 && batch_width() > 1) return f_optim_batch(batch_width(), denomD);
        objective_fn f = make_F(true, sigma, denomD);
        std::vector<double> x = beta, lo(P, -HUGE_VAL), up;
        for (int i = 0; i < R; ++i) { x.push_back(theta[i]); lo.push_back(1e-6); }
        if (g) { x.push_back(sigma); lo.push_back(0.0); }
        up.assign(x.size(), HUGE_VAL);
        BobyqaResult r;
        MCML_TRY(bobyqa(f, x, lo, up, bopts(), &r));
        beta.assign(r.x.begin(), r.x.begin() + P);
        theta.assign(r.x.begin() + P, r.x.begin() + P + R);
        if (g) sigma = r.x[P + R];
        return MCML_OK;
    }

    int f_hess(double tol, double* H)
    {
        auto memo = std::make_shared<ThetaMemo>();
        objective_fn f = make_F(false, sigma, 0.0, true, memo);
        const int nv = P + R;
        std::vector<double> x = beta, lo(P, -HUGE_VAL), up(nv, HUGE_VAL), nd(nv, tol), h;
        for (int i = 0; i < R; ++i) { x.push_back(theta[i]); lo.push_back(1e-6); }
        if (comm_world(c) == 1 && c.maxdim_large > 0) {
            std::vector<std::vector<double>> want;
            objective_fn dry = [&](const std::vector<double>& par, double* v) {
                std::vector<double> th(par.begin() + P, par.begin() + P + R);
                if (std::find(want.begin(), want.end(), th) == want.end()) want.push_back(th);
                *v = 0.0; return (int)MCML_OK; };
            std::vector<double> hdry;
            MCML_TRY(fd_hessian(dry, x, nd, true, lo, up, &hdry));
            std::vector<double> ths((size_t)R * want.size()), sums(want.size(), 0.0);
            std::vector<int> rcs(want.size(), 0);
            for (size_t q = 0; q < want.size(); ++q) for (int i = 0; i < R; ++i) ths[q * R + i] = want[q][i];
            MCML_TRY(mvn_loglik_batch(c, ths.data(), (int)want.size(), c.U.d(), c.U.ld, c.mcols, sums.data(), rcs.data()));
            for (size_t q = 0; q < want.size(); ++q)
                (*memo)[want[q]] = rcs[q] == MCML_OK ? sums[q] / c.mcols : -HUGE_VAL;
        }
        MCML_TRY(fd_hessian(f, x, nd, true, lo, up, &h));
        memcpy(H, h.data(), sizeof(double) * (size_t)nv * nv);
        return MCML_OK;
    }
};

static uint64_t default_seed(const glmmr_mcml_ext* e)
{
    if (e && e->seed) return e->seed;
    std::random_device rd;
    return ((uint64_t)rd() << 32) | rd();
}

int drv_optim(Ctx& c, const double* start, int nstart, int trace, int mcnr, const glmmr_mcml_ext* e,
              double* beta, double* theta, double* sigma)
{
    const int P = c.P, R = c.cov.npar;
    MCML_REQUIRE(start && nstart >= P + R + (is_gaussian(c.flink) ? 1 : 0), "start has %d values, need %d", nstart, P + R + (is_gaussian(c.flink) ? 1 : 0));
    MCML_REQUIRE(c.mcols > 0, "no samples u set");
    McmlOptim mc(c, start, trace, e ? e->maxfun : 0, 1.0);
    mc.theta_batch = e ? e->theta_batch : 0;
    {
        PhaseRange r("mcml:beta-step");
        if (!mcnr) MCML_TRY(mc.l_optim()); else MCML_TRY(mc.mcnr());
    }
    PhaseRange r("mcml:theta-step");
    MCML_TRY(mc.d_optim());
    memcpy(beta, mc.beta.data(), sizeof(double) * P);
    memcpy(theta, mc.theta.data(), sizeof(double) * R);
    *sigma = mc.sigma;
    return MCML_OK;
}

int drv_simlik(Ctx& c, const double* start, int nstart, int trace, const glmmr_mcml_ext* e, double* beta,
               double* theta, double* sigma)
{
    const int P = c.P, R = c.cov.npar;
    MCML_REQUIRE(start && nstart >= P + R + (is_gaussian(c.flink) ? 1 : 0), "start too short");
    MCML_REQUIRE(c.mcols > 0, "no samples u set");
    McmlOptim mc(c, start, trace, e ? e->maxfun : 0, 1.0);
    mc.theta_batch = e ? e->theta_batch : 0;
    MCML_TRY(mc.f_optim());
    memcpy(beta, mc.beta.data(), sizeof(double) * P);
    memcpy(theta, mc.theta.data(), sizeof(double) * R);
    *sigma = mc.sigma;
    return MCML_OK;
}

int drv_hess(Ctx& c, const double* start, int nstart, double tol, int trace, double* H)
{
    const int P = c.P, R = c.cov.npar;
    MCML_REQUIRE(start && nstart >= P + R + (is_gaussian(c.flink) ? 1 : 0), "start too short");
    MCML_REQUIRE(c.mcols > 0, "no samples u set");
    McmlOptim mc(c, start, trace, 0, 1.0);
    return mc.f_hess(tol, H);
}

int drv_aic(Ctx& c, const double* beta_par, int nbeta, const double* cov_par, int ncov, double* out)
{
    const int P = c.P;
    const bool var = (c.flink == 7 || c.flink == 8 || c.flink == 12);
    MCML_REQUIRE(nbeta >= P + (var ? 1 : 0) && ncov >= c.cov.npar, "aic_mcml: parameter vectors too short");
    MCML_REQUIRE(c.mcols > 0, "no samples u set");
    const double var_par = var ? beta_par[P] : 0;
    const int dof = nbeta + ncov;
    double dmv, ll;
    MCML_TRY(eval_mvn(c, cov_par, &dmv));
    MCML_TRY(eval_loglik(c, beta_par, var_par, &ll));
    *out = (-2 * (ll + dmv) + 2 * dof);
    return MCML_OK;
}

int drv_full(Ctx& c, const double* start, int nstart, int mcnr, int m, int maxiter, int warmup, double tol,
             int verbose, double lambda, int trace, int refresh, int maxsteps, double target_accept,
             const glmmr_mcml_ext* e, double* beta_out, double* theta_out, double* sigma_out,
             int* converged_out, int* iters_out, glmmr_mcml_hmc_diag* last_diag)
{
    (void)refresh;
    const int P = c.P, R = c.cov.npar;
    MCML_REQUIRE(start && nstart >= P + R + 1, "mcml_full: start needs c(beta, theta, sigma|1) = %d values", P + R + 1);
    MCML_REQUIRE(m > 0 && maxiter >= 1, "mcml_full: bad m / maxiter");
    std::vector<double> theta(start + P, start + P + R), beta(start, start + P);
    double var_par = is_gaussian(c.flink) ? start[nstart - 1] : 1;
    const uint64_t seed = default_seed(e);
    const int chains = (e && e->chains > 0) ? e->chains : 1;
    MCML_TRY(mvn_gen_L(c, theta.data(), true));
    MCML_TRY(model_update_beta(c, beta.data()));
    MCML_TRY(model_update_L(c));
    McmlOptim mc(c, start, trace, e ? e->maxfun : 0, var_par);
    mc.theta_batch = e ? e->theta_batch : 0;
    double maxdiff = 1;
    int iter = 1;
    bool converged = false;
    glmmr_mcml_hmc_opts ho{};
    ho.warmup = warmup; ho.nsamp = m; ho.adapt = 100; ho.lambda = lambda; ho.max_steps = maxsteps;
    ho.target_accept = target_accept; ho.chains = chains; ho.chain_offset = c.rank * chains;
    while (maxdiff > tol && iter <= maxiter) {
        glmmr_mcml_hmc_diag dg{};
        {
            PhaseRange r("mcml:sample");
            MCML_TRY(hmc_sample(c, beta.data(), var_par, &ho, seed, (uint32_t)iter, nullptr, nullptr, nullptr,
                                nullptr, &dg, nullptr));
        }
        if (last_diag) *last_diag = dg;
        mc.model_var_par = var_par;
        {
            PhaseRange r("mcml:beta-step");
            if (!mcnr) MCML_TRY(mc.l_optim()); else MCML_TRY(mc.mcnr());
        }
        {
            PhaseRange r("mcml:theta-step");
            MCML_TRY(mc.d_optim());
        }
        const std::vector<double>& nb = mc.beta; const std::vector<double>& nt = mc.theta;
        double new_var_par = 1;
        if (is_gaussian(c.flink)) new_var_par = mc.sigma;
        else new_var_par = var_par;
        maxdiff = 0;
        for (int i = 0; i < P; ++i) maxdiff = std::max(maxdiff, std::fabs(beta[i] - nb[i]));
        for (int i = 0; i < R; ++i) maxdiff = std::max(maxdiff, std::fabs(theta[i] - nt[i]));
        maxdiff = std::max(maxdiff, std::fabs(var_par - new_var_par));
        if (maxdiff < tol) converged = true;
        beta = nb; theta = nt; var_par = new_var_par;
        if (!converged) {
            PhaseRange r("mcml:refresh");
            MCML_TRY(mvn_gen_L(c, theta.data(), true));
            MCML_TRY(model_update_beta(c, beta.data()));
            MCML_TRY(model_update_L(c));
        }
        if (verbose && c.rank == 0) {
            printf("Iter %d  beta:", iter);
            for (double b : beta) printf(" %.6g", b);
            printf("  theta:");
            for (double t : theta) printf(" %.6g", t);
            if (is_gaussian(c.flink)) printf("  sigma: %.6g", var_par);
            printf("  max diff %.4g  accept %.3f%s\n", maxdiff, dg.accept_rate, converged ? "  CONVERGED" : "");
            fflush(stdout);
        }
        ++iter;
    }
    memcpy(beta_out, beta.data(), sizeof(double) * P);
    memcpy(theta_out, theta.data(), sizeof(double) * R);
    *sigma_out = var_par;
    if (converged_out) *converged_out = converged ? 1 : 0;
    if (iters_out) *iters_out = iter - 1;
    return MCML_OK;
}

}

extern "C" int glmmr_mcml_dbg_phase_ms(int enable, int reset, double* out8)
{
    mcml::PhaseClock& pc = mcml::phase_clock();
    std::lock_guard<std::mutex> g(pc.mu);
    if (out8) for (int i = 0; i < 4; ++i) { out8[i] = pc.ms[i]; out8[4 + i] = (double)pc.n[i]; }
    if (reset) for (int i = 0; i < 4; ++i) { pc.ms[i] = 0; pc.n[i] = 0; }
    pc.on.store(enable != 0, std::memory_order_relaxed);
    return 0;
}
```

glmmrmcml_amd/csrc/mvn.hip:

```cpp
#include "ctx.h"
#include "dgemm_mfma.h"
#include "dgemm_dl.h"
#include "reduce.h"

namespace mcml {

#define LOG_2PI 1.8378770664093454835606594728112

__global__ __launch_bounds__(256) void k_sum_partials(const double* partials, int n, double* out, int accumulate)
{
    __shared__ double sh[4];
    double v = 0;
    for (int i = threadIdx.x; i < n; i += 256) v += partials[i];
    double r = block_sum(v, sh);
    if (threadIdx.x == 0) out[0] = (accumulate ? out[0] : 0.0) + r;
}

int device_sum(Ctx& c, const double* partials, int n, double* dev_out)
{
    hipLaunchKernelGGL(k_sum_partials, dim3(1), dim3(256), 0, c.stream, partials, n, dev_out, 0);
    MCML_HIP(hipGetLastError());
    return MCML_OK;
}

__device__ __forceinline__ double diag_variance(const CovBlock& blk, const int32_t* cov, int rows, const ThetaArg& th)
{
    double val = 1.0;
    for (int r = blk.r0; r < blk.r1; ++r) val = cov_term(1, 0.0, &th.v[cov[r + 4 * rows]], val);
    return val;
}

__global__ void k_diag_prep(int Q, const int* rowblock, const CovBlock* blocks, const int32_t* cov,
                            int rows, ThetaArg th, double* dd, double* dc)
{
    int k = blockIdx.x * blockDim.x + threadIdx.x;
    if (k >= Q) return;
    int b = rowblock[k];
    if (b < 0) { dd[k] = 1.0; dc[k] = 0.0; return; }
    double d = sqrt(diag_variance(blocks[b], cov, rows, th));
    dd[k] = d * d;
    dc[k] = -0.5 * log(d * d) - 0.5 * LOG_2PI;
}

__global__ __launch_bounds__(256) void k_diag_ll(const double* U, int ldu, int Q, int mcols,
                                                 const int* rowblock, const double* dd,
                                                 const double* dc, double* partials)
{
    __shared__ double sh[4];
    int k = blockIdx.x * 256 + threadIdx.x;
    double acc = 0;
    if (k < Q && rowblock[k] >= 0) {
        const double idd = dd[k], c0 = dc[k];
        for (int col = blockIdx.y; col < mcols; col += gridDim.y) {
            double u = U[k + (size_t)col * ldu];
            acc += c0 - 0.5 * u * u / idd;
        }
    }
    double r = block_sum(acc, sh);
    if (threadIdx.x == 0) partials[blockIdx.y * gridDim.x + blockIdx.x] = r;
}

__device__ __forceinline__ double cov_entry(const CovBlock& blk, const int32_t* cov, int rows,
                                            const double* bd, const ThetaArg& th, int i, int j)
{
    double val = 1.0;
    int coff = 0;
    for (int r = blk.r0; r < blk.r1; ++r) {
        const int fn = cov[r + 2 * rows], nv = cov[r + 3 * rows], pi = cov[r + 4 * rows];
        double d2 = 0.0;
        for (int p = 0; p < nv; ++p) {
            double df = bd[i + (size_t)(coff + p) * blk.dim] - bd[j + (size_t)(coff + p) * blk.dim];
            d2 += df * df;
        }
        val = cov_term(fn, sqrt(d2), &th.v[pi], val);
        coff += nv;
    }
    return val;
}

__global__ __launch_bounds__(64) void k_small_ll(const double* U, int ldu, int mcols,
                                                 const int* small_ids, const CovBlock* blocks,
                                                 const int32_t* cov, int rows, const double* data,
                                                 ThetaArg th, double* partials, int* errflag)
{
    __shared__ double S[SMALL_BLOCK * (SMALL_BLOCK + 1)];
    __shared__ double Zs[SMALL_BLOCK * 64];
    const CovBlock blk = blocks[small_ids[blockIdx.x]];
    const int dim = blk.dim, lane = threadIdx.x;
    constexpr int LS = SMALL_BLOCK + 1;
    const double* bd = data + blk.doff;
    for (int e = lane; e < dim * dim; e += 64) {
        int i = e % dim, j = e / dim;
        if (i >= j) S[i * LS + j] = cov_entry(blk, cov, rows, bd, th, i, j);
    }
    __syncthreads();
    for (int j = 0; j < dim; ++j) {
        if (lane == j) {
            double d = S[j * LS + j];
            for (int k = 0; k < j; ++k) d -= S[j * LS + k] * S[j * LS + k];
            if (!(d > 0.0)) { atomicExch(errflag, 1); d = 1.0; }
            S[j * LS + j] = sqrt(d);
        }
        __syncthreads();
        if (lane > j && lane < dim) {
            double s = S[lane * LS + j];
            for (int k = 0; k < j; ++k) s -= S[lane * LS + k] * S[j * LS + k];
            S[lane * LS + j] = s / S[j * LS + j];
        }
        __syncthreads();
    }
    double logdet = 0;
    for (int i = 0; i < dim; ++i) logdet += 2 * log(S[i * LS + i]);
    double acc = 0;
    for (int col = blockIdx.y * 64 + lane; col < mcols; col += gridDim.y * 64) {
        const double* u = U + blk.matstart + (size_t)col * ldu;
        double quad = 0;
        for (int i = 0; i < dim; ++i) {
            double lsum = 0;
            for (int j = 0; j < i; ++j) lsum += S[i * LS + j] * Zs[j * 64 + lane];
            double z = (u[i] - lsum) / S[i * LS + i];
            Zs[i * 64 + lane] = z;
            quad += z * z;
        }
        acc += (-0.5 * dim * LOG_2PI - 0.5 * logdet - 0.5 * quad);
    }
    acc = wave_sum(acc);
    if (lane == 0) partials[blockIdx.x * gridDim.y + blockIdx.y] = acc;
}

__device__ __forceinline__ void build_dense_body(double* A, int lda, int bidx, const CovBlock* blocks, const int32_t* cov,
                                                 int rows, const double* data, const ThetaArg& th, int mirror, int dpad)
{
    if ((int)blockIdx.x * 64 + 63 < (int)blockIdx.y * 16) return;
    const CovBlock blk = blocks[bidx];
    const int i = blockIdx.x * 64 + (threadIdx.x & 63);
#pragma unroll
    for (int u = 0; u < 4; ++u) {
        const int j = blockIdx.y * 16 + (threadIdx.x >> 6) * 4 + u;
        if (i >= blk.dim && i < dpad && j <= i) { A[i + (size_t)j * lda] = (i == j) ? 1.0 : 0.0; continue; }
        if (i >= blk.dim || j >= blk.dim || i < j) continue;
        const double v = cov_entry(blk, cov, rows, data + blk.doff, th, i, j);
        A[i + (size_t)j * lda] = v;
        if (mirror && i != j) A[j + (size_t)i * lda] = v;
    }
}

constexpr int MVN_MAXBATCH = 8;
struct ThetaBatch { ThetaArg t[MVN_MAXBATCH]; };

__global__ __launch_bounds__(256) void k_build_dense_batch(double* A, int lda, size_t bsA, int bidx, const CovBlock* blocks,
                                                           const int32_t* cov, int rows, const double* data,
                                                           ThetaBatch tb, int dpad)
{
    build_dense_body(A + (size_t)blockIdx.z * bsA, lda, bidx, blocks, cov, rows, data, tb.t[blockIdx.z], 0, dpad);
}

// ... 172 lines not shown
            if constexpr (PROF) prof.u = prof.now();
            const int lrow = lane < 32 ? kb + l15 : (pvalid ? prow : 0);
            const bool ld_row = lane < 16 ? (kb + lane < n) : pvalid;
            const double* srow = S + lrow * LS + kb;
#pragma unroll
            for (int c = 0; c < 16; ++c) {
                const double v = srow[c];
                const bool use = ld_row && (lane >= 32 || kb + c < n);
                a[c] = use ? v : ((lane < 32 && l15 == c) ? 1.0 : 0.0);
            }
            asm volatile("s_waitcnt lgkmcnt(0)" ::: "memory");
            if constexpr (PROF) { prof.q0 += prof.now() - prof.u; prof.u = prof.now(); }
            potrf16_col<0>(a, lane, bad, yv);  potrf16_col<1>(a, lane, bad, yv);
            potrf16_col<2>(a, lane, bad, yv);  potrf16_col<3>(a, lane, bad, yv);
            potrf16_col<4>(a, lane, bad, yv);  potrf16_col<5>(a, lane, bad, yv);
            potrf16_col<6>(a, lane, bad, yv);  potrf16_col<7>(a, lane, bad, yv);
            potrf16_col<8>(a, lane, bad, yv);  potrf16_col<9>(a, lane, bad, yv);
            potrf16_col<10>(a, lane, bad, yv); potrf16_col<11>(a, lane, bad, yv);
            potrf16_col<12>(a, lane, bad, yv); potrf16_col<13>(a, lane, bad, yv);
            potrf16_col<14>(a, lane, bad, yv); potrf16_col<15>(a, lane, bad, yv);
            if constexpr (PROF) { prof.q1 += prof.now() - prof.u; prof.u = prof.now(); }
            double* drow = S + lrow * LS + kb;
            if (n == 128) {
                double* dmy = dummy + lane;
                double* w1 = (lane < 16 || pvalid) ? drow : nullptr;
#pragma unroll
                for (int c = 0; c < 16; ++c) *(w1 ? w1 + c : dmy) = a[c];
#pragma unroll
                for (int c = 0; c < 16; ++c) *((lk == 1 && c > l15) ? drow + c : dmy) = a[c];
                if (lane < 16) xd[kb + lane] = yv;
                if (lk == 1) {
                    double* g = Linv + (kb + l15) * 128 + kb;
#pragma unroll
                    for (int c = 0; c < 16; ++c) g[c] = a[c];
                }
            } else {
#pragma unroll
                for (int c = 0; c < 16; ++c) {
                    const bool st = lane < 16 ? (l15 >= c && kb + l15 < n && kb + c < n) : (lane < 32 ? c > l15 : pvalid);
                    if (st) drow[c] = a[c];
                }
                if (lane < 16) xd[kb + lane] = yv;
                if (lk == 1) {
                    double* g = Linv + (kb + l15) * 128 + kb;
#pragma unroll
                    for (int c = 0; c < 16; ++c)
                        if (c >= l15 && kb + c < n && kb + l15 < n) g[c] = a[c];
                }
            }
            if (bad && lane == 0) atomicExch(errflag, 1);
            if constexpr (PROF) { prof.q2 += prof.now() - prof.u; prof.u = prof.now(); }
        } else if (kt >= 1) {
            rest_update(kt - 1);
            inverse_row(kt - 1);
        }
        leaf_sync();
        if constexpr (PROF) {
            prof.q3 += prof.now() - prof.u;
            prof.ta += prof.now() - prof.t; prof.t = prof.now();
        }
        for (int t = kt + 3 + wave; t < ntile; t += LEAF_NW) {
            const int r0 = t * 16;
            d4 acc = {0.0, 0.0, 0.0, 0.0};
            double pa[4], pb[4];
#pragma unroll
            for (int kc = 0; kc < 4; ++kc) {
                const int k = kc * 4 + lk;
                pa[kc] = S[(r0 + l15) * LS + kb + k];
                pb[kc] = (l15 == k) ? xd[kb + k] : (l15 > k ? S[(kb + k) * LS + kb + l15] : 0.0);
            }
#pragma unroll
            for (int kc = 0; kc < 4; ++kc) acc = __builtin_amdgcn_mfma_f64_16x16x4f64(pa[kc], pb[kc], acc, 0, 0, 0);
#pragma unroll
            for (int r = 0; r < 4; ++r) S[(r0 + lk + 4 * r) * LS + kb + l15] = acc[r];
        }
        leaf_sync();
        if constexpr (PROF) { prof.tb += prof.now() - prof.t; prof.t = prof.now(); }
        if (wave == 0) {
            for (int ti = kt + 1; ti < ntile && ti <= kt + 3; ++ti) upd_tile(ti, kt + 1, kb);
            asm volatile("" ::: "memory");
        }
        if constexpr (PROF) prof.tc += prof.now() - prof.t;
    }
    leaf_sync();
    if constexpr (PROF) prof.stamp(5);
    {
        const int i = tid & 127, j0 = tid >> 7;
        if (i < n)
            for (int j = j0; j <= i && j < n; j += LEAF_NT / 128) A[i + (size_t)j * lda] = S[i * LS + j];
    }
    if (wave >= 1) inverse_row(ntile - 1);
    if constexpr (PROF) {
        prof.stamp(9);
        if (threadIdx.x == 0) {
            prof.out[1] = prof.q3; prof.out[2] = prof.ta; prof.out[3] = prof.tb; prof.out[4] = prof.tc;
            prof.out[6] = prof.q0; prof.out[7] = prof.q1; prof.out[8] = prof.q2;
        }
    }
}

__global__ __launch_bounds__(256) void k_transpose_in(const double* A, int lda, int rows, int cols, double* AT, int ldt,
                                                      size_t bsT = 0)
{
    AT += (size_t)blockIdx.z * bsT;
    __shared__ double tile[32][33];
    const int bx = blockIdx.x * 32, by = blockIdx.y * 32;
    const int tx = threadIdx.x & 31, ty = threadIdx.x >> 5;
    for (int r = ty; r < 32; r += 8) {
        const int i = bx + tx, j = by + r;
        tile[r][tx] = (i < rows && j < cols) ? A[i + (size_t)j * lda] : 0.0;
    }
    __syncthreads();
    for (int r = ty; r < 32; r += 8) {
        const int j = by + tx, i = bx + r;
        if (i < rows && j < cols) AT[j + (size_t)i * ldt] = tile[tx][r];
    }
}

__global__ void k_copy_block(double* dst, int ldd, const double* src, int lds, int rows, int cols)
{
    int i = blockIdx.x * blockDim.x + threadIdx.x;
    if (i >= rows) return;
    for (int j = blockIdx.y; j < cols; j += gridDim.y) dst[i + (size_t)j * ldd] = src[i + (size_t)j * lds];
}

__global__ __launch_bounds__(256) void k_sumsq(const double* U, int ldu, int rows, int cols, double* partials)
{
    __shared__ double sh[4];
    int i = blockIdx.x * 256 + threadIdx.x;
    double acc = 0;
    if (i < rows)
        for (int j = blockIdx.y; j < cols; j += gridDim.y) {
            double u = U[i + (size_t)j * ldu];
            acc += u * u;
        }
    double r = block_sum(acc, sh);
    if (threadIdx.x == 0) partials[blockIdx.y * gridDim.x + blockIdx.x] = r;
}

__global__ __launch_bounds__(256) void k_logdet(const double* A, int lda, int n, double* out)
{
    __shared__ double sh[4];
    double acc = 0;
    for (int i = threadIdx.x; i < n; i += 256) acc += 2 * log(A[i + (size_t)i * lda]);
    double r = block_sum(acc, sh);
    if (threadIdx.x == 0) out[0] = r;
}

__global__ void k_finish_large(double* scal, int dim, int mcols)
{
    scal[0] += (double)mcols * (-0.5 * dim * LOG_2PI - 0.5 * scal[1]) - 0.5 * scal[2];
}

__global__ void k_zero_upper(double* A, int lda, int n)
{
    int i = blockIdx.x * blockDim.x + threadIdx.x;
    int j = blockIdx.y;
    if (i < n && j < n && i < j) A[i + (size_t)j * lda] = 0.0;
}

struct Bat { int n = 1; size_t sA = 0, sL = 0; int* err = nullptr; };

template <bool BNMAJOR>
static int chol_gemm(hipStream_t s, int M, int N, int K, const double* A, int lda, const double* B, int ldb,
                     const EpiAxpby& epi, bool lower_only, int tile, int inplace, int shift = 0, int nbatch = 1,
                     size_t bsA = 0, size_t bsB = 0)
{
    if (dl_applicable(M, N, K, A, lda, B, ldb, BNMAJOR))
        return launch_gemm_dl<BNMAJOR>(s, M, N, K, A, lda, B, ldb, epi, lower_only, tile, inplace, shift, nbatch, bsA, bsB);
    MCML_REQUIRE(nbatch == 1, "potrf: a batch of factorisations needs the LDS-DMA kernel for every panel product");
    MCML_REQUIRE(shift == 0 || !lower_only, "potrf: shifted lower-only update needs the LDS-DMA kernel");
    return launch_gemm<BNMAJOR>(s, M, N, K, A, lda, B, ldb, epi, lower_only, inplace ? inplace : -1);
}

static size_t linv_size(int n) { return (size_t)(n / CHOL_NB + 1) * CHOL_NB * CHOL_NB; }

static int leaf_prepare(Ctx& c, int n, int nbatch)
{
    const size_t bytes = sizeof(double) * linv_size(n) * nbatch;
    MCML_TRY(c.linv.ensure(bytes));
    MCML_HIP(hipMemsetAsync(c.linv.p, 0, bytes, c.stream));
    return ensure_dynamic_lds(reinterpret_cast<const void*>(&k_potrf_leaf<false>), (int)POTRF_LDS);
}

struct PotrfLaunch {
    Ctx& c; double* A; int lda; Bat bt; int* errflag;
    PotrfLaunch(Ctx& c_, double* A_, int lda_, const Bat& b)
        : c(c_), A(A_), lda(lda_), bt(b), errflag(b.err ? b.err : c_.errflag()) {}
    double* linv(int k) const { return c.linv.d() + (size_t)(k / CHOL_NB) * CHOL_NB * CHOL_NB; }
    int leaf(hipStream_t s, int k, int nb) const {
        hipLaunchKernelGGL(k_potrf_leaf<false>, dim3(bt.n), dim3(LEAF_NT), POTRF_LDS, s, A + k + (size_t)k * lda, lda, nb,
                           linv(k), errflag, bt.sA, bt.sL, LeafProf<false>());
        MCML_HIP(hipGetLastError());
        return MCML_OK;
    }
    int gemm_nt(hipStream_t s, int M, int N, int K, const double* Ap, const double* Bp, int ldb, double* Cp,
                double alpha, double beta, bool lower, int tile, int inplace, int shift) const {
        EpiAxpby epi{Cp, lda, alpha, beta, bt.sA};
        const size_t sB = (ldb == CHOL_NB) ? bt.sL : bt.sA;
        return chol_gemm<true>(s, M, N, K, Ap, lda, Bp, ldb, epi, lower, tile, inplace, shift, bt.n, bt.sA, sB);
    }
    struct Step { int k, nb, rem, R, nb2; double *A11, *A21; const double* Linv; };
    Step step(int t, int n, int extra) const {
        const int k = t * CHOL_NB, nb = (n - k < CHOL_NB) ? n - k : CHOL_NB, rem = n - k - nb;
        double* A11 = A + k + (size_t)k * lda;
        return Step{k, nb, rem, rem + extra, rem < CHOL_NB ? rem : CHOL_NB, A11, A11 + nb, linv(k)};
    }
};

static int lookahead_setup(Ctx& c)
{
    if (c.aux) return MCML_OK;
    int lo = 0, hi = 0;
    MCML_HIP(hipDeviceGetStreamPriorityRange(&lo, &hi));
    MCML_HIP(hipStreamCreateWithPriority(&c.aux, hipStreamNonBlocking, hi));
    MCML_HIP(hipStreamCreateWithPriority(&c.aux_lo, hipStreamNonBlocking, lo));
    MCML_HIP(hipEventCreateWithFlags(&c.ev_col, hipEventDisableTiming));
    MCML_HIP(hipEventCreateWithFlags(&c.ev_leaf, hipEventDisableTiming));
    return MCML_OK;
}

static int potrf_blocked(Ctx& c, double* A, int lda, int n, int extra, Bat bt = Bat())
{
    const PotrfLaunch L(c, A, lda, bt);
    const bool two = n > 2 * CHOL_NB;
    hipStream_t sM = c.stream, sL = c.stream;
    if (two) { MCML_TRY(lookahead_setup(c)); sL = c.aux; }
    const int nsteps = (n + CHOL_NB - 1) / CHOL_NB;
    constexpr int SPW = CHOL_NB * 8;
    const bool twolevel = bt.n > 1 && n > SPW + CHOL_NB;
    MCML_TRY(L.leaf(sM, 0, n < CHOL_NB ? n : CHOL_NB));
    bool forked = false;
    for (int t = 0; t < nsteps; ++t) {
        const PotrfLaunch::Step s = L.step(t, n, extra);
        const int k = s.k, nb = s.nb, rem = s.rem, R = s.R, nb2 = s.nb2;
        if (R <= 0) break;
        if (forked) { MCML_HIP(hipStreamWaitEvent(sM, c.ev_leaf, 0)); forked = false; }
        const int sp0 = twolevel ? (k / SPW) * SPW : 0, sp1 = twolevel ? (sp0 + SPW < n ? sp0 + SPW : n) : n;
        const int inner = sp1 - (k + nb);
        if (twolevel && inner == 0 && rem > 0) {
            MCML_TRY(L.gemm_nt(sM, R, nb, nb, s.A21, s.Linv, CHOL_NB, s.A21, 1.0, 0.0, false, 0, 1, 0));
            const double* Asp = A + sp1 + (size_t)sp0 * lda;
            double* Csp = A + sp1 + (size_t)sp1 * lda;
            MCML_TRY(L.gemm_nt(sM, R, rem, sp1 - sp0, Asp, Asp, lda, Csp, -1.0, 1.0, true, 0, 0, 0));
            MCML_TRY(L.leaf(sM, k + nb, nb2));
            continue;
        }
        if (nb2 > 0) {
            MCML_TRY(L.gemm_nt(sM, nb2, nb, nb, s.A21, s.Linv, CHOL_NB, s.A21, 1.0, 0.0, false, 7, 1, 0));
            double* T = s.A11 + nb + (size_t)nb * lda;
            MCML_TRY(L.gemm_nt(sM, nb2, nb2, nb, s.A21, s.A21, lda, T, -1.0, 1.0, false, 8, 0, 0));
            if (two) {
                MCML_HIP(hipEventRecord(c.ev_col, sM));
                MCML_HIP(hipStreamWaitEvent(sL, c.ev_col, 0));
            }
            MCML_TRY(L.leaf(sL, k + nb, nb2));
            if (two) { MCML_HIP(hipEventRecord(c.ev_leaf, sL)); forked = true; }
        }
        if (R - nb2 > 0)
            MCML_TRY(L.gemm_nt(sM, R - nb2, nb, nb, s.A21 + nb2, s.Linv, CHOL_NB, s.A21 + nb2, 1.0, 0.0, false, 0, 1, 0));
        if (rem > 0 && R - nb2 > 0) {
            double* C2 = s.A11 + nb + nb2 + (size_t)nb * lda;
            MCML_TRY(L.gemm_nt(sM, R - nb2, twolevel ? inner : rem, nb, s.A21 + nb2, s.A21, lda, C2, -1.0, 1.0, true, 0, 0, nb2));
        }
    }
    if (forked) MCML_HIP(hipStreamWaitEvent(sM, c.ev_leaf, 0));
    return MCML_OK;
}

static hipEvent_t ring_event(Ctx& c, size_t idx)
{
    while (c.ev_ring.size() <= idx) {
        hipEvent_t e = nullptr;
        if (hipEventCreateWithFlags(&e, hipEventDisableTiming) != hipSuccess) return nullptr;
        c.ev_ring.push_back(e);
    }
    return c.ev_ring[idx];
}
static int potrf_la2_capture(Ctx& c, double* A, int lda, int n, int extra, Bat bt = Bat())
{
    const PotrfLaunch L(c, A, lda, bt);
    hipStream_t sC = c.stream, sB = c.aux_lo;
    const int nsteps = (n + CHOL_NB - 1) / CHOL_NB;
    auto EV = [&](int step, int kind) -> hipEvent_t { return ring_event(c, (size_t)3 * (step + 1) + kind); };
    MCML_REQUIRE(ring_event(c, (size_t)3 * (nsteps + 2)) != nullptr, "potrf: could not create the capture's events");
    MCML_TRY(L.leaf(sC, 0, n < CHOL_NB ? n : CHOL_NB));
    MCML_HIP(hipEventRecord(EV(-1, 0), sC));
    MCML_HIP(hipStreamWaitEvent(sB, EV(-1, 0), 0));
    hipEvent_t last_b = nullptr;
    for (int t = 0; t < nsteps; ++t) {
        const PotrfLaunch::Step s = L.step(t, n, extra);
        const int k = s.k, nb = s.nb, rem = s.rem, R = s.R, nb2 = s.nb2;
        if (R <= 0) break;
        const int nb3 = (rem - nb2 < CHOL_NB) ? rem - nb2 : CHOL_NB;
        const int w = nb2 + nb3;
        if (nb2 > 0) {
            if (last_b) MCML_HIP(hipStreamWaitEvent(sC, last_b, 0));
            MCML_TRY(L.gemm_nt(sC, nb2, nb, nb, s.A21, s.Linv, CHOL_NB, s.A21, 1.0, 0.0, false, 7, 1, 0));
            double* T = s.A11 + nb + (size_t)nb * lda;
            MCML_TRY(L.gemm_nt(sC, nb2, nb2, nb, s.A21, s.A21, lda, T, -1.0, 1.0, false, 8, 0, 0));
            MCML_HIP(hipEventRecord(EV(t, 1), sC));
            MCML_TRY(L.leaf(sC, k + nb, nb2));
            MCML_HIP(hipEventRecord(EV(t, 0), sC));
        }
        const int Rb = R - nb2;
        if (Rb > 0) {
            MCML_TRY(L.gemm_nt(sB, Rb, nb, nb, s.A21 + nb2, s.Linv, CHOL_NB, s.A21 + nb2, 1.0, 0.0, false, 0, 1, 0));
            if (nb2 > 0) {
                MCML_HIP(hipStreamWaitEvent(sB, EV(t, 1), 0));
                double* Cb = s.A11 + nb + nb2 + (size_t)nb * lda;
                MCML_TRY(L.gemm_nt(sB, Rb, w, nb, s.A21 + nb2, s.A21, lda, Cb, -1.0, 1.0, false, 0, 0, 0));
                MCML_HIP(hipEventRecord(EV(t, 2), sB));
                last_b = EV(t, 2);
                if (rem - w > 0) {
                    double* Cc = s.A11 + nb + w + (size_t)(nb + w) * lda;
                    MCML_TRY(L.gemm_nt(sB, R - w, rem - w, nb, s.A21 + w, s.A21 + w, lda, Cc, -1.0, 1.0, true, 0, 0, 0));
                }
            }
        } else if (nb2 > 0) {
            MCML_HIP(hipStreamWaitEvent(sB, EV(t, 1), 0));
            MCML_HIP(hipEventRecord(EV(t, 2), sB));
            last_b = EV(t, 2);
        }
        if (nb2 > 0) MCML_HIP(hipStreamWaitEvent(sB, EV(t, 0), 0));
    }
    MCML_HIP(hipEventRecord(EV(nsteps, 0), sB));
    MCML_HIP(hipStreamWaitEvent(sC, EV(nsteps, 0), 0));
    return MCML_OK;
}

static bool chol_graph_on()
{
    static const bool on = !(getenv("GLMMR_MCML_CHOL_GRAPH") && !strcmp(getenv("GLMMR_MCML_CHOL_GRAPH"), "0"));
    return on;
}
static bool graph_timer_begin(Ctx& c, CholGraph& g)
{
    if (!g.t0 && (hipEventCreate(&g.t0) != hipSuccess || hipEventCreate(&g.t1) != hipSuccess)) { (void)hipGetLastError(); return false; }
    return hipEventRecord(g.t0, c.stream) == hipSuccess;
}
static void calibrate(CholGraph& g)
{
    float ms = 0.f;
    g.timed = false;
    bool done = true;
    const hipError_t ee = hipEventElapsedTime(&ms, g.t0, g.t1);
    static const bool cal_trace = getenv("GLMMR_MCML_GRAPH_TRACE") != nullptr;
    if (cal_trace) fprintf(stderr, "graph calibration: n=%d extra=%d trial %d: %.3f ms (eager %.3f, best %.3f) rc=%d\n", g.n, g.extra, g.tries, ms, g.eager_ms, g.best_ms, (int)ee);
    if (ee == hipSuccess && g.eager_ms > 0.f && g.tmpl) {
        if (!g.best || ms < g.best_ms) {
            if (g.best && g.best != g.exec) (void)hipGraphExecDestroy(g.best);
            g.best = g.exec; g.best_ms = ms;
        } else if (g.exec != g.best) (void)hipGraphExecDestroy(g.exec);
        g.exec = g.best;
        if (!(g.best_ms <= 0.93f * g.eager_ms) && g.tries < 3) {
            hipGraphExec_t ex2 = nullptr;
            if (hipGraphInstantiate(&ex2, g.tmpl, nullptr, nullptr, 0) == hipSuccess) { g.exec = ex2; ++g.tries; g.trial_launches = 0; done = false; }
            else (void)hipGetLastError();
        }
    } else (void)hipGetLastError();
    if (done) {
        g.settled = true; g.best = nullptr;
        if (g.tmpl) { (void)hipGraphDestroy(g.tmpl); g.tmpl = nullptr; }
    }
}
static int capture_and_instantiate(Ctx& c, CholGraph& g, double* A, int lda, int n, int extra, const Bat& bt)
{
    MCML_TRY(lookahead_setup(c));
    if (hipStreamBeginCapture(c.stream, hipStreamCaptureModeThreadLocal) != hipSuccess) { (void)hipGetLastError(); return MCML_OK; }
    const int rc = potrf_la2_capture(c, A, lda, n, extra, bt);
    hipGraph_t graph = nullptr;
    const hipError_t e = hipStreamEndCapture(c.stream, &graph);
    if (rc != MCML_OK || e != hipSuccess || !graph || hipGraphInstantiate(&g.exec, graph, nullptr, nullptr, 0) != hipSuccess) {
        if (graph) (void)hipGraphDestroy(graph);
        (void)hipGetLastError();
        g.exec = nullptr;
        return MCML_OK;
    }
    g.tmpl = graph; g.tries = 0; g.settled = !(g.eager_ms > 0.f); g.timed = false; g.best = nullptr; g.best_ms = 0.f;
    if (g.settled) { (void)hipGraphDestroy(g.tmpl); g.tmpl = nullptr; }
    return MCML_OK;
}
static void eager_for_good(CholGraph& g) { g.seen = -(1 << 30); }

static int potrf_graphed(Ctx& c, double* A, int lda, int n, int extra, Bat bt = Bat())
{
    if (!chol_graph_on() || n <= 2 * CHOL_NB) return potrf_blocked(c, A, lda, n, extra, bt);
    CholGraph& g = c.chol_graphs.find(A, c.linv.d(), lda, n, extra);
    if (g.exec) {
        if (!g.settled && g.timed) calibrate(g);
        const bool tm = !g.settled && g.trial_launches >= 1 && graph_timer_begin(c, g);
        MCML_HIP(hipGraphLaunch(g.exec, c.stream));
        if (tm) g.timed = hipEventRecord(g.t1, c.stream) == hipSuccess;
        ++g.trial_launches;
        return MCML_OK;
    }
    if (g.seen++ <= 1) {
        const bool tm = graph_timer_begin(c, g);
        MCML_TRY(potrf_blocked(c, A, lda, n, extra, bt));
        if (tm && hipEventRecord(g.t1, c.stream) == hipSuccess && hipEventSynchronize(g.t1) == hipSuccess)
            (void)hipEventElapsedTime(&g.eager_ms, g.t0, g.t1);
        (void)hipGetLastError();
        return MCML_OK;
    }
    MCML_TRY(capture_and_instantiate(c, g, A, lda, n, extra, bt));
    if (!g.exec) {
        eager_for_good(g);
        return potrf_blocked(c, A, lda, n, extra, bt);
    }
    g.trial_launches = 1;
    MCML_HIP(hipGraphLaunch(g.exec, c.stream));
    return MCML_OK;
}

int potrf_lower(Ctx& c, double* A, int n, int lda)
{
    MCML_REQUIRE(n > 0 && lda >= n && (lda & 1) == 0, "potrf: bad shape n=%d lda=%d", n, lda);
    MCML_TRY(leaf_prepare(c, n, 1));
    return potrf_blocked(c, A, lda, n, 0);
}

int potrf_leaf_profile(Ctx& c, unsigned long long* host10)
{
    DevMat A; DevBuf prof;
    MCML_TRY(A.alloc(128, 128));
    MCML_TRY(prof.ensure(80));
    std::vector<double> h((size_t)A.ld * 128, 0.0);
    for (int j = 0; j < 128; ++j) for (int i = 0; i < 128; ++i) h[i + (size_t)j * A.ld] = (i == j ? 130.0 : 1.0 / (1 + abs(i - j)));
    MCML_TRY(leaf_prepare(c, 128, 1));
    MCML_TRY(ensure_dynamic_lds(reinterpret_cast<const void*>(&k_potrf_leaf<true>), (int)POTRF_LDS));
    LeafProf<true> lp;
    lp.out = prof.as<unsigned long long>();
    for (int rep = 0; rep < 3; ++rep) {
        MCML_TRY(copy_h2d(A.d(), h.data(), sizeof(double) * h.size(), 0)); MCML_HIP(hipDeviceSynchronize());
        hipLaunchKernelGGL(k_potrf_leaf<true>, dim3(1), dim3(LEAF_NT), POTRF_LDS, c.stream, A.d(), A.ld, 128, c.linv.d(),
                           c.errflag(), (size_t)0, (size_t)0, lp);
        MCML_HIP(hipStreamSynchronize(c.stream));
    }
    MCML_HIP(hipMemcpy(host10, prof.p, 80, hipMemcpyDeviceToHost));
    return MCML_OK;
}

int trsm_left_lower(Ctx& c, const double* L, int ldl, int n, double* U, int ldu, int m)
{
    for (int k = 0; k < n; k += CHOL_NB) {
        const int nb = (n - k < CHOL_NB) ? n - k : CHOL_NB;
        const double* Linv = c.linv.d() + (size_t)(k / CHOL_NB) * CHOL_NB * CHOL_NB;
        double* Uk = U + k;
        {
            EpiAxpby epi{Uk, ldu, 1.0, 0.0};
            MCML_TRY(chol_gemm<false>(c.stream, nb, m, nb, Linv, CHOL_NB, Uk, ldu, epi, false, 0, 2));
        }
        const int rem = n - k - nb;
        if (rem <= 0) break;
        const double* L21 = L + (k + nb) + (size_t)k * ldl;
        EpiAxpby epi{Uk + nb, ldu, -1.0, 1.0};
        MCML_TRY(chol_gemm<false>(c.stream, rem, m, nb, L21, ldl, Uk, ldu, epi, false, 0, 0));
    }
    return MCML_OK;
}

int trsm_left_lower_trans(Ctx& c, const double* R, int ldr, int n, double* T, int ldt, int m)
{
    MCML_REQUIRE(R && T && n > 0 && m > 0, "trsm_left_lower_trans: empty operand");
    MCML_REQUIRE(ldr >= n + (n & 1) && ldt >= n + (n & 1) && (ldr & 1) == 0 && (ldt & 1) == 0,
                 "trsm_left_lower_trans: bad leading dimensions %d, %d for n = %d", ldr, ldt, n);
    MCML_REQUIRE(c.linv.bytes >= sizeof(double) * linv_size(n), "trsm_left_lower_trans: no factorisation of this size before it");
    for (int k = (n - 1) / CHOL_NB * CHOL_NB; k >= 0; k -= CHOL_NB) {
        const int nb = (n - k < CHOL_NB) ? n - k : CHOL_NB;
        const double* Linv = c.linv.d() + (size_t)(k / CHOL_NB) * CHOL_NB * CHOL_NB;
        double* Tk = T + k;
        {
            EpiAxpby epi{Tk, ldt, 1.0, 0.0};
            MCML_TRY(launch_gemm_at(c.stream, nb, m, nb, Linv, CHOL_NB, Tk, ldt, epi, 2));
        }
        if (k == 0) break;
        EpiAxpby epi{T, ldt, -1.0, 1.0};
        MCML_TRY(launch_gemm_at(c.stream, k, m, nb, R + k, ldr, Tk, ldt, epi));
    }
    return MCML_OK;
}

int mvn_setup(Ctx& c)
{
    const CovSpec& cs = c.cov;
    MCML_TRY(c.d_cov.ensure(sizeof(int32_t) * cs.cov.size()));
    MCML_TRY(copy_h2d(c.d_cov.p, cs.cov.data(), sizeof(int32_t) * cs.cov.size(), c.stream));
    MCML_TRY(c.d_data.ensure(sizeof(double) * (cs.data.size() + 1)));
    if (!cs.data.empty())
        MCML_TRY(copy_h2d(c.d_data.p, cs.data.data(), sizeof(double) * cs.data.size(), c.stream));
    MCML_TRY(c.d_blocks.ensure(sizeof(CovBlock) * cs.blocks.size()));
    MCML_TRY(copy_h2d(c.d_blocks.p, cs.blocks.data(), sizeof(CovBlock) * cs.blocks.size(), c.stream));
    std::vector<int> rowblock(cs.N, -1), small;
    c.maxdim_large = 0; c.n_small = 0; c.n_diag_rows = 0;
    for (int b = 0; b < cs.B; ++b) {
        const CovBlock& blk = cs.blocks[b];
        if (blk.all_gr) {
            for (int k = 0; k < blk.dim; ++k) rowblock[blk.matstart + k] = b;
            c.n_diag_rows += blk.dim;
        } else if (blk.dim <= SMALL_BLOCK) {
            ++c.n_small;
            small.push_back(b);
        } else if (blk.dim > c.maxdim_large) {
            c.maxdim_large = blk.dim;
        }
    }
    MCML_TRY(c.d_rowblock.ensure(sizeof(int) * (size_t)(cs.N + 1)));
    MCML_TRY(copy_h2d(c.d_rowblock.p, rowblock.data(), sizeof(int) * cs.N, c.stream));
    MCML_TRY(c.scalars.ensure(sizeof(double) * 64));
    MCML_HIP(hipMemsetAsync(c.scalars.p, 0, sizeof(double) * 64, c.stream));
    if (c.n_small) {
        MCML_TRY(c.small_ids.ensure(sizeof(int) * small.size()));
        MCML_TRY(copy_h2d(c.small_ids.p, small.data(), sizeof(int) * small.size(), c.stream));
    }
    if (c.maxdim_large) {
        MCML_TRY(c.Dwork.alloc(c.maxdim_large, c.maxdim_large));
        MCML_HIP(hipMemsetAsync(c.Dwork.d(), 0, sizeof(double) * (size_t)c.Dwork.ld * c.maxdim_large, c.stream));
        MCML_TRY(c.linv.ensure(sizeof(double) * linv_size(round_up(c.maxdim_large, 16)) * MVN_MAXBATCH));
    }
    MCML_HIP(hipStreamSynchronize(c.stream));
    return MCML_OK;
}

static int theta_arg(const Ctx& c, const double* theta, ThetaArg& th)
{
    MCML_REQUIRE(theta, "theta is null");
    memset(&th, 0, sizeof th);
    for (int i = 0; i < c.cov.npar; ++i) th.v[i] = theta[i];
    return MCML_OK;
}

static int check_errflag(Ctx& c, const char* what)
{
    int flag = 0;
    MCML_TRY(copy_d2h(&flag, c.errflag(), sizeof(int), c.stream));
    MCML_HIP(hipStreamSynchronize(c.stream));
    if (flag) {
        MCML_HIP(hipMemsetAsync(c.errflag(), 0, sizeof(int), c.stream));
        set_error("%s: covariance block is not positive definite", what);
        return MCML_ENOTPD;
    }
    return MCML_OK;
}

int potrf_lower_checked(Ctx& c, double* A, int n, int lda)
{
    MCML_TRY(potrf_lower(c, A, n, lda));
    return check_errflag(c, "potrf");
}

int mvn_loglik_sum(Ctx& c, const double* theta, double* sum_out)
{
    MCML_REQUIRE(c.mcols > 0 && c.U.d(), "mvn_ll: no samples set");
    return mvn_loglik_sum_on(c, theta, c.U.d(), c.U.ld, c.mcols, sum_out);
}

static int mvn_large_blocks(Ctx& c, DevMat& W, int kb, const ThetaArg* th, const double* Us, int ldu, int m,
                            double* scal, int sstride, int* flags)
{
    const CovSpec& cs = c.cov;
    const int32_t* dcov = c.d_cov.as<int32_t>();
    const CovBlock* dblk = c.d_blocks.as<CovBlock>();
    const int ld = W.ld, dmax = round_up(c.maxdim_large, 16);
    Bat bt; bt.n = kb; bt.sA = (size_t)ld * dmax; bt.sL = linv_size(dmax); bt.err = flags;
    ThetaBatch tb;
    memset(&tb, 0, sizeof tb);
    for (int j = 0; j < kb; ++j) tb.t[j] = th[j];
    for (int b = 0; b < cs.B; ++b) {
        const CovBlock& blk = cs.blocks[b];
        if (blk.all_gr || blk.dim <= SMALL_BLOCK) continue;
        const int d = blk.dim;
        const int dp = round_up(d, 16);
        c.mvn_ws[&W == &c.Dbatch] = Ctx::MvnWs{d, dp, m, ld, kb};
        const dim3 gb((dp + 63) / 64, (dp + 15) / 16, kb);
        if (kb == 1)
            hipLaunchKernelGGL(k_build_dense, gb, dim3(256), 0, c.stream, W.d(), ld, b, dblk, dcov, cs.rows, c.d_data.d(),
                               th[0], 0, dp);
        else
            hipLaunchKernelGGL(k_build_dense_batch, gb, dim3(256), 0, c.stream, W.d(), ld, bt.sA, b, dblk, dcov, cs.rows,
                               c.d_data.d(), tb, dp);
        hipLaunchKernelGGL(k_transpose_in, dim3((d + 31) / 32, (m + 31) / 32, kb), dim3(256), 0, c.stream,
                           Us + blk.matstart, ldu, d, m, W.d() + dp, ld, bt.sA);
        MCML_HIP(hipGetLastError());
        if (dp > d)
            for (int j = 0; j < kb; ++j)
                MCML_HIP(hipMemset2DAsync(W.d() + j * bt.sA + dp + (size_t)d * ld, sizeof(double) * ld, 0, sizeof(double) * m, dp - d, c.stream));
        MCML_TRY(leaf_prepare(c, dmax, kb));
        MCML_TRY(kb > 1 ? potrf_blocked(c, W.d(), ld, dp, m, bt) : potrf_graphed(c, W.d(), ld, dp, m, bt));
        const int gx = (m + 255) / 256, gy = d < 64 ? d : 64;
        MCML_TRY(c.partials.ensure(sizeof(double) * (size_t)(gx * gy + 16)));
        for (int j = 0; j < kb; ++j) {
            double* sj = scal + (size_t)j * sstride;
            const double* Aj = W.d() + j * bt.sA;
            hipLaunchKernelGGL(k_sumsq, dim3(gx, gy), dim3(256), 0, c.stream, Aj + dp, ld, m, d, c.partials.d());
            hipLaunchKernelGGL(k_sum_partials, dim3(1), dim3(256), 0, c.stream, c.partials.d(), gx * gy, sj + 2, 0);
            hipLaunchKernelGGL(k_logdet, dim3(1), dim3(256), 0, c.stream, Aj, ld, d, sj + 1);
            hipLaunchKernelGGL(k_finish_large, dim3(1), dim3(1), 0, c.stream, sj, d, m);
        }
        MCML_HIP(hipGetLastError());
    }
    return MCML_OK;
}

static int mvn_loglik_enqueue(Ctx& c, const double* theta, const double* Us, int ldu, int m)
{
    MCML_REQUIRE(m > 0 && Us, "mvn_ll: no samples set");
    ThetaArg th;
    MCML_TRY(theta_arg(c, theta, th));
    const CovSpec& cs = c.cov;
    const int Q = cs.N;
    double* scal = c.scalars.d();
    const int32_t* dcov = c.d_cov.as<int32_t>();
    const CovBlock* dblk = c.d_blocks.as<CovBlock>();
    const int* drb = c.d_rowblock.as<int>();
    MCML_HIP(hipMemsetAsync(scal, 0, sizeof(double) * 4, c.stream));

    if (c.n_diag_rows > 0) {
        MCML_TRY(c.partials.ensure(sizeof(double) * (size_t)(2 * Q + 65536)));
        double* dd = c.partials.d();
        double* dc = dd + Q;
        double* part = dc + Q;
        hipLaunchKernelGGL(k_diag_prep, dim3((Q + 255) / 256), dim3(256), 0, c.stream, Q, drb, dblk, dcov,
                           cs.rows, th, dd, dc);
        dim3 grid((Q + 255) / 256, 1);
        int gy = 65536 / (int)grid.x; if (gy > m) gy = m; if (gy > 64) gy = 64; if (gy < 1) gy = 1;
        grid.y = gy;
        hipLaunchKernelGGL(k_diag_ll, grid, dim3(256), 0, c.stream, Us, ldu, Q, m, drb, dd, dc, part);
        hipLaunchKernelGGL(k_sum_partials, dim3(1), dim3(256), 0, c.stream, part, (int)(grid.x * grid.y), scal, 1);
        MCML_HIP(hipGetLastError());
    }
    if (c.n_small > 0) {
        int ny = (m + 63) / 64; if (ny > 16) ny = 16;
        DevBuf& wb = c.scratch;
        MCML_TRY(wb.ensure(sizeof(double) * (size_t)c.n_small * ny + 1024));
        double* part = wb.d();
        hipLaunchKernelGGL(k_small_ll, dim3((unsigned)c.n_small, ny), dim3(64), 0, c.stream, Us, ldu, m,
                           c.small_ids.as<int>(), dblk, dcov, cs.rows, c.d_data.d(), th, part, c.errflag());
        hipLaunchKernelGGL(k_sum_partials, dim3(1), dim3(256), 0, c.stream, part, c.n_small * ny, scal, 1);
        MCML_HIP(hipGetLastError());
    }
    if (c.maxdim_large > 0) {
        if (c.Dwork.rows < c.maxdim_large + 16 + m || c.Dwork.cols < c.maxdim_large + 16) {
            MCML_TRY(c.Dwork.alloc(c.maxdim_large + 16 + m, c.maxdim_large + 16));
            MCML_HIP(hipMemsetAsync(c.Dwork.d(), 0, sizeof(double) * (size_t)c.Dwork.ld * (c.maxdim_large + 16), c.stream));
        }
        MCML_TRY(mvn_large_blocks(c, c.Dwork, 1, &th, Us, ldu, m, scal, 4, c.errflag()));
    }
    return MCML_OK;
}

int mvn_loglik_sum_on(Ctx& c, const double* theta, const double* Us, int ldu, int m, double* sum_out)
{
    MCML_TRY(mvn_loglik_enqueue(c, theta, Us, ldu, m));
    MCML_TRY(copy_d2h(sum_out, c.scalars.d(), sizeof(double), c.stream));
    MCML_TRY(check_errflag(c, "mvn_ll"));
    return MCML_OK;
}

int mvn_loglik_batch(Ctx& c, const double* thetas, int k, const double* Us, int ldu, int m, double* sums, int* rcs)
{
    MCML_REQUIRE(k >= 1 && thetas && sums && rcs && m > 0 && Us, "mvn_ll batch: bad arguments");
    const int R = c.cov.npar;
    const bool batchable = k > 1 && c.maxdim_large > 0 && c.n_small == 0 && c.n_diag_rows == 0;
    if (!batchable) {
        int first_rc = MCML_OK;
        for (int j = 0; j < k; ++j) {
            rcs[j] = mvn_loglik_sum_on(c, thetas + (size_t)j * R, Us, ldu, m, sums + j);
            if (rcs[j] != MCML_OK && rcs[j] != MCML_ENOTPD && first_rc == MCML_OK) first_rc = rcs[j];
        }
        return first_rc;
    }
    for (int j0 = 0; j0 < k; j0 += MVN_MAXBATCH) {
        const int kb = (k - j0 < MVN_MAXBATCH) ? k - j0 : MVN_MAXBATCH;
        ThetaArg th[MVN_MAXBATCH];
        for (int j = 0; j < kb; ++j) MCML_TRY(theta_arg(c, thetas + (size_t)(j0 + j) * R, th[j]));
        const int dmax = round_up(c.maxdim_large, 16);
        if (c.Dbatch.rows < dmax + m || c.Dbatch.cols < kb * dmax) {
            MCML_TRY(c.Dbatch.alloc(dmax + m, MVN_MAXBATCH * dmax));
            MCML_HIP(hipMemsetAsync(c.Dbatch.d(), 0, sizeof(double) * (size_t)c.Dbatch.ld * MVN_MAXBATCH * dmax, c.stream));
        }
        MCML_TRY(c.bscal.ensure(sizeof(double) * 5 * MVN_MAXBATCH));
        MCML_HIP(hipMemsetAsync(c.bscal.p, 0, sizeof(double) * 5 * MVN_MAXBATCH, c.stream));
        int* bflags = reinterpret_cast<int*>(c.bscal.d() + 4 * MVN_MAXBATCH);
        MCML_TRY(mvn_large_blocks(c, c.Dbatch, kb, th, Us, ldu, m, c.bscal.d(), 4, bflags));
        double hs[4 * MVN_MAXBATCH]; int hf[MVN_MAXBATCH];
        MCML_TRY(copy_d2h(hs, c.bscal.p, sizeof(double) * 4 * kb, c.stream));
        MCML_TRY(copy_d2h(hf, bflags, sizeof(int) * kb, c.stream));
        MCML_HIP(hipStreamSynchronize(c.stream));
        for (int j = 0; j < kb; ++j) { sums[j0 + j] = hs[4 * j]; rcs[j0 + j] = hf[j] ? MCML_ENOTPD : MCML_OK; }
    }
    return MCML_OK;
}

__global__ void k_diag_fill(double* L, int ldl, int Q, const int* rowblock, const CovBlock* blocks,
                            const int32_t* cov, int rows, ThetaArg th, int chol)
{
    int k = blockIdx.x * blockDim.x + threadIdx.x;
    if (k >= Q) return;
    int b = rowblock[k];
    if (b < 0) return;
    const double val = diag_variance(blocks[b], cov, rows, th);
    L[k + (size_t)k * ldl] = chol ? sqrt(val) : val;
}

int mvn_gen_L(Ctx& c, const double* theta, bool chol)
{
    ThetaArg th;
    MCML_TRY(theta_arg(c, theta, th));
    const CovSpec& cs = c.cov;
    const int Q = cs.N;
    MCML_TRY(c.L.alloc(Q, Q));
    MCML_HIP(hipMemsetAsync(c.L.d(), 0, sizeof(double) * (size_t)c.L.ld * Q, c.stream));
    const int32_t* dcov = c.d_cov.as<int32_t>();
    const CovBlock* dblk = c.d_blocks.as<CovBlock>();
    if (c.n_diag_rows > 0)
        hipLaunchKernelGGL(k_diag_fill, dim3((Q + 255) / 256), dim3(256), 0, c.stream, c.L.d(), c.L.ld, Q,
                           c.d_rowblock.as<int>(), dblk, dcov, cs.rows, th, chol ? 1 : 0);
    for (int b = 0; b < cs.B; ++b) {
        const CovBlock& blk = cs.blocks[b];
        if (blk.all_gr) continue;
        const int d = blk.dim;
        double* A = c.L.at(blk.matstart, blk.matstart);
        dim3 g((d + 63) / 64, (d + 15) / 16);
        hipLaunchKernelGGL(k_build_dense, g, dim3(256), 0, c.stream, A, c.L.ld, b, dblk, dcov, cs.rows,
                           c.d_data.d(), th, chol ? 0 : 1, d);
        MCML_HIP(hipGetLastError());
        if (chol) {
            if (d <= CHOL_NB || (blk.matstart & 1) == 0) {
                MCML_TRY(potrf_lower(c, A, d, c.L.ld));
            } else {
                DevMat tmp;
                MCML_TRY(tmp.alloc(d, d));
                hipLaunchKernelGGL(k_copy_block, dim3((d + 255) / 256, d < 256 ? d : 256), dim3(256), 0, c.stream,
                                   tmp.d(), tmp.ld, A, c.L.ld, d, d);
                MCML_TRY(potrf_lower(c, tmp.d(), d, tmp.ld));
                hipLaunchKernelGGL(k_copy_block, dim3((d + 255) / 256, d < 256 ? d : 256), dim3(256), 0, c.stream,
                                   A, c.L.ld, tmp.d(), tmp.ld, d, d);
                MCML_HIP(hipStreamSynchronize(c.stream));
            }
            if (d > CHOL_NB)
                hipLaunchKernelGGL(k_zero_upper, dim3((d + 255) / 256, d), dim3(256), 0, c.stream, A, c.L.ld, d);
        }
    }
    MCML_HIP(hipGetLastError());
    MCML_TRY(check_errflag(c, "genD"));
    if (chol) c.l_foreign = false;
    c.have_L = chol;
    return MCML_OK;
}

}
```

include/glmmr_mcml_c.h:

```cpp
#ifndef GLMMR_MCML_C_H
#define GLMMR_MCML_C_H
#include <stdint.h>

#ifdef __cplusplus
extern "C" {
#endif

#define GLMMR_MCML_OK            0
#define GLMMR_MCML_EINVAL       -1
#define GLMMR_MCML_EUNSUPPORTED -2
#define GLMMR_MCML_ENOTPD       -3
#define GLMMR_MCML_ESINGULAR    -4
#define GLMMR_MCML_EHIP         -5
#define GLMMR_MCML_ENODEVICE    -6
#define GLMMR_MCML_ENOMEM       -7

const char* glmmr_mcml_last_error(void);


typedef struct glmmr_mcml_problem {
    const int32_t* cov;
    int            cov_rows;
    const double*  data;
    int            data_len;
// ... 77 lines not shown
    int    chain_offset;
    int    metric;
} glmmr_mcml_nuts_opts;

typedef struct glmmr_mcml_nuts_diag {
    double    mean_e, min_e, max_e;
    long long divergent;
    long long treedepth_hits;
    long long batched_leapfrogs;
    long long stepsize_search_leapfrogs;
    long long packs;
} glmmr_mcml_nuts_diag;

int glmmr_mcml_ctx_nuts_sample(glmmr_mcml_ctx* ctx, const double* beta, double var_par,
                               const glmmr_mcml_nuts_opts* opts, uint64_t seed, uint32_t iter_idx,
                               int* depth_out, int* nleap_out, double* eps_out, double* accept_out,
                               glmmr_mcml_nuts_diag* diag, int* ncols_out);


typedef struct glmmr_mcml_ext {
    uint64_t seed;
    int      chains;
    int      maxfun;
    int      device;
    int      theta_batch;
} glmmr_mcml_ext;

int glmmr_mcml_gen_u_samples(const double* Z, const double* L, const double* X, const double* y, int n, int Q, int P,
                             const double* beta, const char* family, const char* link, double sigma, int warmup_iter,
                             int m, const glmmr_mcml_nuts_opts* opts, const glmmr_mcml_ext* ext, double* samples,
                             int lds, int* ncols);

int glmmr_mcml_sample_cols(int m, int chains);
int glmmr_mcml_ctx_ncols(glmmr_mcml_ctx* ctx);
int glmmr_mcml_ctx_profile(glmmr_mcml_ctx* ctx, int enable, int reset, double* out8);
int glmmr_mcml_ctx_profile_launches(glmmr_mcml_ctx* ctx, long long* fwd, long long* bwd);
int glmmr_mcml_ctx_last_kernels(glmmr_mcml_ctx* ctx, int* fwd, int* bwd);
int glmmr_mcml_dbg_band_plan(glmmr_mcml_ctx* ctx, int which, int chains, int* out10);
int glmmr_mcml_dbg_sparse_plan(glmmr_mcml_ctx* ctx, int chains, long long* out12);
int glmmr_mcml_ctx_set_trajectory(glmmr_mcml_ctx* ctx, int mode);
int glmmr_mcml_set_default_trajectory(int mode);
int glmmr_mcml_get_default_trajectory(void);
int glmmr_mcml_dbg_component_plan(glmmr_mcml_ctx* ctx, int chains, long long* out11);
long long glmmr_mcml_dbg_traj_launches(void);
int glmmr_mcml_ctx_set_draws(glmmr_mcml_ctx* ctx, int mode);
int glmmr_mcml_set_default_draws(int mode);
int glmmr_mcml_get_default_draws(void);
int glmmr_mcml_dbg_draws_plan(glmmr_mcml_ctx* ctx, int* out4);
int glmmr_mcml_ctx_exact_sample(glmmr_mcml_ctx* ctx, const double* beta, double var_par, const glmmr_mcml_hmc_opts* opts,
                                uint64_t seed, uint32_t iter_idx, const double* inj_z, glmmr_mcml_hmc_diag* diag,
                                int* ncols_out);
int glmmr_mcml_dbg_exact_phases(glmmr_mcml_ctx* ctx, int enable, double* out5);
int glmmr_mcml_dbg_trsm_compare(glmmr_mcml_ctx* ctx, int m, int reps, double* trans_ms, double* fwd_ms);
int glmmr_mcml_ctx_set_la_operator(glmmr_mcml_ctx* ctx, int mode);
int glmmr_mcml_set_default_la_operator(int mode);
int glmmr_mcml_get_default_la_operator(void);
int glmmr_mcml_dbg_la_plan(glmmr_mcml_ctx* ctx, long long* out8);
long long glmmr_mcml_dbg_la_component_launches(void);
int glmmr_mcml_dbg_phase_ms(int enable, int reset, double* out8);
int glmmr_mcml_ctx_npar(glmmr_mcml_ctx* ctx);

int glmmr_mcml_ctx_optim(glmmr_mcml_ctx* ctx, const double* start, int nstart, int trace, int mcnr,
                         const glmmr_mcml_ext* ext, double* beta, double* theta, double* sigma);
int glmmr_mcml_ctx_simlik(glmmr_mcml_ctx* ctx, const double* start, int nstart, int trace,
                          const glmmr_mcml_ext* ext, double* beta, double* theta, double* sigma);
int glmmr_mcml_ctx_hess(glmmr_mcml_ctx* ctx, const double* start, int nstart, double tol, int trace,
                        double* H );
int glmmr_mcml_ctx_aic(glmmr_mcml_ctx* ctx, const double* beta_par, int nbeta, const double* cov_par,
                       int ncov, double* out);
int glmmr_mcml_ctx_full(glmmr_mcml_ctx* ctx, const double* start, int nstart, int mcnr, int m, int maxiter,
                        int warmup, double tol, int verbose, double lambda, int trace, int refresh,
                        int maxsteps, double target_accept, const glmmr_mcml_ext* ext, double* beta,
                        double* theta, double* sigma, int* converged, int* iters,
                        glmmr_mcml_hmc_diag* last_diag);

int glmmr_mcml_full(const glmmr_mcml_problem* prob, const double* start, int nstart, int mcnr, int m,
                    int maxiter, int warmup, double tol, int verbose, double lambda, int trace,
                    int refresh, int maxsteps, double target_accept, const glmmr_mcml_ext* ext,
                    double* beta, double* theta, double* sigma, int* converged, double* u, int ldu,
                    int* ucols);

int glmmr_mcml_mcmc_sample(const double* Z, const double* L, const double* X, const double* y, int n,
                           int Q, int P, const double* beta, const char* family, const char* link,
                           int warmup, int nsamp, double lambda, double var_par, int trace, int refresh,
                           int maxsteps, double target_accept, const glmmr_mcml_ext* ext,
                           double* samples, int lds, int* ncols);

int glmmr_mcml_optim(const glmmr_mcml_problem* prob, const double* u, int ucols, const double* start,
                     int nstart, int trace, int mcnr, const glmmr_mcml_ext* ext, double* beta,
                     double* theta, double* sigma);
int glmmr_mcml_simlik(const glmmr_mcml_problem* prob, const double* u, int ucols, const double* start,
                      int nstart, int trace, const glmmr_mcml_ext* ext, double* beta, double* theta,
                      double* sigma);
int glmmr_mcml_optim_sparse(const glmmr_mcml_problem* prob, const int32_t* Ap, const int32_t* Ai, int nnz,
                            const double* u, int ucols, const double* start, int nstart, int trace,
                            int mcnr, const glmmr_mcml_ext* ext, double* beta, double* theta,
                            double* sigma,
                            int32_t* Lp, int32_t* Li, double* Lx, double* D, int lcap);
int glmmr_mcml_sparse_factor_nnz(const int32_t* cov, int cov_rows, const double* data, int data_len);
int glmmr_mcml_simlik_sparse(const glmmr_mcml_problem* prob, const int32_t* Ap, const int32_t* Ai, int nnz,
                             const double* u, int ucols, const double* start, int nstart, int trace,
                             const glmmr_mcml_ext* ext, double* beta, double* theta, double* sigma);
int glmmr_mcml_hess(const glmmr_mcml_problem* prob, const double* u, int ucols, const double* start,
                    int nstart, double tol, int trace, const glmmr_mcml_ext* ext, double* H);
int glmmr_mcml_hess_sparse(const glmmr_mcml_problem* prob, const int32_t* Ap, const int32_t* Ai, int nnz,
                           const double* u, int ucols, const double* start, int nstart, double tol,
                           int trace, const glmmr_mcml_ext* ext, double* H);
int glmmr_mcml_aic(const glmmr_mcml_problem* prob, const double* u, int ucols, const double* beta_par,
                   int nbeta, const double* cov_par, int ncov, const glmmr_mcml_ext* ext, double* out);

int glmmr_mcml_la(const glmmr_mcml_problem* prob, const double* start, int nstart, int usehess, double tol,
                  int verbose, int trace, int maxiter, const glmmr_mcml_ext* ext, double* beta, double* theta,
                  double* sigma, double* se, double* u);
int glmmr_mcml_la_nr(const glmmr_mcml_problem* prob, const double* start, int nstart, int usehess, double tol,
                     int verbose, int trace, int maxiter, const glmmr_mcml_ext* ext, double* beta, double* theta,
                     double* sigma, double* se, double* u);
int glmmr_mcml_ctx_la(glmmr_mcml_ctx* ctx, const double* start, int nstart, int nr, int usehess, double tol,
                      int verbose, int trace, int maxiter, const glmmr_mcml_ext* ext, double* beta, double* theta,
                      double* sigma, double* se, double* u, int* converged, int* iters);

int glmmr_mcml_mvn_ll(const int32_t* cov, int cov_rows, const double* data, int data_len,
                      const double* eff_range, int eff_len, const double* gamma, int ngamma,
                      const double* u, int Q, int m, double* out);

int glmmr_mcml_dbg_theta_log(glmmr_mcml_ctx* ctx, int enable, double* out, int cap_rows, int* nrows);
int glmmr_mcml_dbg_emulate_world(glmmr_mcml_ctx* ctx, int world, int mode);
int glmmr_mcml_dbg_leaf_profile(glmmr_mcml_ctx* ctx, unsigned long long* out10);
int glmmr_mcml_dbg_la_probe(glmmr_mcml_ctx* ctx, const double* start, int nstart, int kind, const double* v,
                            double var_par, const double* par, int npar, double* out, double* v_out,
                            double* beta_out, double* sigma_out);
int glmmr_mcml_dbg_dgemm(int M, int N, int K, const double* A, int lda, const double* B, int ldb,
                         int b_nmajor, double alpha, double beta, double* C, int ldc,
                         int lower_only, int force_tile );
int glmmr_mcml_dbg_dgemm_at(int M, int N, int K, const double* A, int lda, const double* B, int ldb, double alpha,
                            double beta, double* C, int ldc, int force_tile);
int glmmr_mcml_dbg_chol(glmmr_mcml_ctx* ctx, int n, double* A, int lda, int m, const double* B, int ldb, double* Xfwd,
                        double* Ytrans, double* Zpotrs, double* Linv);
int glmmr_mcml_dbg_mvn_workspace(glmmr_mcml_ctx* ctx, int cand, double* L, int ldl, double* X, int ldx, int* dims);
int glmmr_mcml_dbg_log_prob_grad(glmmr_mcml_ctx* ctx, const double* beta, double var_par, const double* V,
                                 int ncols, double* lp, double* G);
int glmmr_mcml_dbg_normals(uint64_t seed, uint32_t chain, uint32_t prop, uint32_t tag, int n, double* out);
int glmmr_mcml_dbg_minstd(uint32_t seed, int n, double* out);
typedef double (*glmmr_mcml_objective)(const double* x, int n, void* user);
int glmmr_mcml_dbg_bobyqa(glmmr_mcml_objective f, void* user, int n, const double* x0, const double* lower,
                          const double* upper, double rhobeg, double rhoend, int maxfun, double* x_out,
                          double* f_out, int* nfev_out);
int glmmr_mcml_dbg_bobyqa_batch(glmmr_mcml_objective f, void* user, int n, const double* x0, const double* lower,
                                const double* upper, double rhobeg, double rhoend, int maxfun, int width,
                                double* x_out, double* f_out, int* nfev_out, int* rounds_out);
typedef int (*glmmr_mcml_batch_objective)(const double* X, int n, int k, double* F, void* user);
int glmmr_mcml_dbg_bobyqa_rounds(glmmr_mcml_batch_objective fb, void* user, int n, const double* x0, const double* lower,
                                 const double* upper, double rhobeg, double rhoend, int maxfun, int width,
                                 double* x_out, double* f_out, int* nfev_out, int* rounds_out);
int glmmr_mcml_dbg_copy_roundtrip(const double* in, long long ld_in, double* out, long long ld_out, long long rows, long long cols);
int glmmr_mcml_dbg_fd_hessian(glmmr_mcml_objective f, void* user, int n, const double* x, double ndeps,
                              int usebounds, const double* lower, const double* upper, double* H);
int glmmr_mcml_dbg_dgemm_bench(int M, int N, int K, int b_nmajor, int iters, int force_tile,
                               double* ms_per_launch);
int glmmr_mcml_dbg_dgemm_bench2(int M, int N, int K, int b_nmajor, int iters, int force_tile, int lower_only,
                                double beta, double* ms_per_launch);
int glmmr_mcml_dbg_dgemm_band(int M, int N, int K, const double* A, int lda, const double* B, int ldb, double* C,
                              int ldc, int* tiles_executed);
int glmmr_mcml_dbg_band_clocks(int M, int N, int iters, int mode, double* out3);

#ifdef __cplusplus
}
#endif
#endif
```

Baseline: 1139.

## Reuse covariance factorisations across theta candidates differing only in scale parameters

```diff
diff --git a/glmmrmcml_amd/api.py b/glmmrmcml_amd/api.py
--- a/glmmrmcml_amd/api.py
+++ b/glmmrmcml_amd/api.py
@@ -238,7 +238,7 @@
         out = (C.c_longlong * 6)()
         _lib.check(_lib.lib().glmmr_mcml_ctx_shard_stats(self._h, out))
         return dict(gathers=out[0], gather_doubles=out[1], theta_rounds=out[2], theta_evals_own=out[3],
-                    theta_evals_all=out[4])
+                    theta_evals_all=out[4], theta_factorised=out[5])
 
     def emulate_world(self, world, mode):
         _lib.check(_lib.lib().glmmr_mcml_dbg_emulate_world(self._h, int(world), int(mode)))
diff --git a/glmmrmcml_amd/csrc/cabi.hip b/glmmrmcml_amd/csrc/cabi.hip
--- a/glmmrmcml_amd/csrc/cabi.hip
+++ b/glmmrmcml_amd/csrc/cabi.hip
@@ -406,7 +406,7 @@
     MCML_REQUIRE(h && out6, "shard_stats: null argument");
     const Ctx& c = h->c;
     out6[0] = c.gather_calls; out6[1] = c.gather_doubles; out6[2] = c.theta_rounds; out6[3] = c.theta_evals_own;
-    out6[4] = c.theta_evals_all; out6[5] = 0;
+    out6[4] = c.theta_evals_all; out6[5] = c.theta_factorised;
     return MCML_OK;
 }
 
@@ -596,6 +596,7 @@
 int drv_simlik(Ctx& c, const double* start, int nstart, int trace, const glmmr_mcml_ext* e, double* beta,
                double* theta, double* sigma);
 int drv_hess(Ctx& c, const double* start, int nstart, double tol, int trace, double* H);
+int drv_theta_round(Ctx& c, const double* thetas, int k, double* out);
 int drv_aic(Ctx& c, const double* beta_par, int nbeta, const double* cov_par, int ncov, double* out);
 int drv_full(Ctx& c, const double* start, int nstart, int mcnr, int m, int maxiter, int warmup, double tol,
              int verbose, double lambda, int trace, int refresh, int maxsteps, double target_accept,
@@ -676,6 +677,13 @@
     MCML_REQUIRE(h->c.n > 0 && tol > 0, "hess: context has no model / bad tol");
     MCML_HIP(hipSetDevice(h->c.device));
     return drv_hess(h->c, start, nstart, tol, trace, H);
+}
+
+extern "C" int glmmr_mcml_dbg_theta_round(glmmr_mcml_ctx* h, const double* thetas, int k, double* out)
+{
+    MCML_REQUIRE(h, "theta_round: null context");
+    MCML_HIP(hipSetDevice(h->c.device));
+    return drv_theta_round(h->c, thetas, k, out);
 }
 
 extern "C" int glmmr_mcml_ctx_aic(glmmr_mcml_ctx* h, const double* beta_par, int nbeta, const double* cov_par,
diff --git a/glmmrmcml_amd/csrc/covspec.h b/glmmrmcml_amd/csrc/covspec.h
--- a/glmmrmcml_amd/csrc/covspec.h
+++ b/glmmrmcml_amd/csrc/covspec.h
@@ -26,6 +26,7 @@
         static const int t[15] = {0, 1, 1, 1, 2, 2, 1, 2, 2, 2, 2, 2, 2, 2, 1};
         return (fn >= 1 && fn <= 14) ? t[fn] : -1;
     }
+    static int fn_scale_exp(int fn) { return fn == 1 ? 2 : (fn == 4 || fn == 7) ? 1 : 0; }
     static bool fn_built(int fn) { return fn == 1 || fn == 2 || fn == 3 || fn == 4 || fn == 7 || fn == 14; }
     int c(int r, int col) const { return cov[r + (size_t)col * rows]; }
 
diff --git a/glmmrmcml_amd/csrc/ctx.h b/glmmrmcml_amd/csrc/ctx.h
--- a/glmmrmcml_amd/csrc/ctx.h
+++ b/glmmrmcml_amd/csrc/ctx.h
@@ -233,6 +233,8 @@
     bool theta_log_on = false;
     std::vector<double> theta_log;
     long long theta_rounds = 0, theta_evals_own = 0, theta_evals_all = 0;
+    long long theta_factorised = 0;
+    std::vector<int> theta_scale_p;
     int emu_world = 0, emu_mode = 0;
     std::vector<std::vector<double>> emu_trace; size_t emu_pos = 0;
     DevBuf reduce_buf;
@@ -270,6 +272,8 @@
 int mvn_loglik_sum(Ctx& c, const double* theta, double* sum_out);
 int mvn_loglik_sum_on(Ctx& c, const double* theta, const double* U, int ldu, int m, double* sum_out);
 int mvn_loglik_batch(Ctx& c, const double* thetas, int k, const double* U, int ldu, int m, double* sums, int* rcs);
+int mvn_loglik_batch_parts(Ctx& c, const double* thetas, int k, int round, const double* U, int ldu, int m, double* sums,
+                           int* rcs, double* parts);
 int mvn_gen_L(Ctx& c, const double* theta, bool chol);
 int potrf_lower(Ctx& c, double* A, int n, int lda);
 int potrf_leaf_profile(Ctx& c, unsigned long long* host10);
diff --git a/glmmrmcml_amd/csrc/debug_hooks.hip b/glmmrmcml_amd/csrc/debug_hooks.hip
--- a/glmmrmcml_amd/csrc/debug_hooks.hip
+++ b/glmmrmcml_amd/csrc/debug_hooks.hip
@@ -306,6 +306,7 @@
 
 #include "../../include/glmmr_mcml_c.h"
 #include "optim.h"
+#include "theta_scale.h"
 #include <cmath>
 extern "C" int glmmr_mcml_dbg_bobyqa(glmmr_mcml_objective f, void* user, int n, const double* x0,
                                      const double* lower, const double* upper, double rhobeg, double rhoend,
@@ -370,6 +371,46 @@
     if (rounds_out) *rounds_out = r.rounds;
     return MCML_OK;
 }
+extern "C" int glmmr_mcml_dbg_theta_scale_rounds(glmmr_mcml_parts_objective fb, void* user, int n, const int* exps, int dim,
+                                                 int m, int grouped, const double* x0, const double* lower,
+                                                 const double* upper, double rhobeg, double rhoend, int maxfun, int width,
+                                                 double* x_out, double* f_out, int* nfev_out, int* rounds_out,
+                                                 long long* factorised_out)
+{
+    MCML_REQUIRE(fb && n > 0 && exps && x0 && x_out && width >= 1 && dim > 0 && m > 0, "dbg_theta_scale_rounds: bad argument");
+    ThetaScaleMemo ts;
+    ts.reset(grouped ? std::vector<int>(exps, exps + n) : std::vector<int>(n, 0), true);
+    batch_objective_fn obj = [&](const std::vector<std::vector<double>>& X, std::vector<double>* F) {
+        const int k = (int)X.size();
+        std::vector<double> flat((size_t)n * k);
+        for (int j = 0; j < k; ++j) for (int i = 0; i < n; ++i) flat[(size_t)j * n + i] = X[j][i];
+        const std::vector<int> reps = ts.plan(flat.data(), n, k);
+        const int nr = (int)reps.size();
+        std::vector<double> rx((size_t)n * nr + 1), parts((size_t)2 * nr + 2), ld(nr + 1), ss(nr + 1), rsums(nr + 1), sums(k);
+        std::vector<int> st(nr + 1, 0), rcs(k, 0);
+        for (int q = 0; q < nr; ++q) for (int i = 0; i < n; ++i) rx[(size_t)q * n + i] = flat[(size_t)reps[q] * n + i];
+        if (nr > 0) MCML_TRY(fb(rx.data(), n, nr, ld.data(), ss.data(), st.data(), user));
+        for (int q = 0; q < nr; ++q) {
+            parts[2 * q] = ld[q]; parts[2 * q + 1] = ss[q]; st[q] = st[q] ? MCML_ENOTPD : MCML_OK;
+            rsums[q] = theta_scale_value(dim, m, ld[q], ss[q]);
+        }
+        ts.finish(flat.data(), n, k, reps, rsums.data(), parts.data(), st.data(), dim, m, sums.data(), rcs.data());
+        F->resize(k);
+        for (int j = 0; j < k; ++j) (*F)[j] = rcs[j] == MCML_OK ? -1.0 * (sums[j] / m) : HUGE_VAL;
+        return (int)MCML_OK; };
+    std::vector<double> x(x0, x0 + n), lo(n, -HUGE_VAL), up(n, HUGE_VAL);
+    if (lower) lo.assign(lower, lower + n);
+    if (upper) up.assign(upper, upper + n);
+    BobyqaOpts o; o.rhobeg = rhobeg; o.rhoend = rhoend; if (maxfun > 0) o.maxfun = maxfun;
+    BobyqaResult r;
+    MCML_TRY(bobyqa_batch(obj, x, lo, up, o, width, &r));
+    for (int i = 0; i < n; ++i) x_out[i] = r.x[i];
+    if (f_out) *f_out = r.fval;
+    if (nfev_out) *nfev_out = r.nfev;
+    if (rounds_out) *rounds_out = r.rounds;
+    if (factorised_out) *factorised_out = ts.factorised;
+    return MCML_OK;
+}
 extern "C" int glmmr_mcml_dbg_fd_hessian(glmmr_mcml_objective f, void* user, int n, const double* x, double ndeps,
                                          int usebounds, const double* lower, const double* upper, double* H)
 {
diff --git a/glmmrmcml_amd/csrc/drivers.hip b/glmmrmcml_amd/csrc/drivers.hip
--- a/glmmrmcml_amd/csrc/drivers.hip
+++ b/glmmrmcml_amd/csrc/drivers.hip
@@ -1,6 +1,7 @@
 #include "../../include/glmmr_mcml_c.h"
 #include "ctx.h"
 #include "optim.h"
+#include "theta_scale.h"
 #include "trace.h"
 #include <algorithm>
 #include <cmath>
@@ -62,10 +63,35 @@
 
     BobyqaOpts bopts() const { BobyqaOpts o; o.iprint = trace; if (maxfun > 0) o.maxfun = maxfun; return o; }
 
+    bool scale_active() const
+    {
+        return c.maxdim_large > 0 && c.n_small == 0 && c.n_diag_rows == 0 && theta_scale_any(c.theta_scale_p) && theta_scale_enabled();
+    }
+
+    int eval_round(ThetaScaleMemo* ts, const double* X, const double* ths, int k, const double* Us, int ldu, int m,
+                   double* sums, int* rcs)
+    {
+        if (!ts) { c.theta_factorised += k; return mvn_loglik_batch(c, ths, k, Us, ldu, m, sums, rcs); }
+        const std::vector<int> reps = ts->plan(X, R, k);
+        const int nr = (int)reps.size();
+        if (k == 1 && nr == 1) { c.theta_factorised += 1; return mvn_loglik_batch(c, ths, 1, Us, ldu, m, sums, rcs); }
+        std::vector<double> rth((size_t)R * nr), rsums(nr, 0.0), parts((size_t)2 * nr, 0.0);
+        std::vector<int> rrcs(nr, 0);
+        for (int q = 0; q < nr; ++q) memcpy(&rth[(size_t)q * R], ths + (size_t)reps[q] * R, sizeof(double) * R);
+        int brc = MCML_OK;
+        if (nr > 0) brc = mvn_loglik_batch_parts(c, rth.data(), nr, k, Us, ldu, m, rsums.data(), rrcs.data(), parts.data());
+        if (brc != MCML_OK) { for (int j = 0; j < k; ++j) rcs[j] = brc; return brc; }
+        c.theta_factorised += nr;
+        ts->finish(X, R, k, reps, rsums.data(), parts.data(), rrcs.data(), c.cov.N, m, sums, rcs);
+        return MCML_OK;
+    }
+
     int d_optim_sharded(int width)
     {
         MCML_TRY(gather_samples(c));
         const int wr = comm_world(c), mall = c.mcols * wr;
+        std::vector<ThetaScaleMemo> memos(scale_active() ? wr : 0);
+        for (ThetaScaleMemo& ts : memos) ts.reset(c.theta_scale_p, true);
         batch_objective_fn fb = [&](const std::vector<std::vector<double>>& Zs, std::vector<double>* F) -> int {
             const int nc = (int)Zs.size();
             std::vector<double> vals(nc, 0.0);
@@ -76,11 +102,12 @@
                 std::vector<int> own;
                 for (int j = 0; j < nc; ++j) if ((j % wr) == rr) own.push_back(j);
                 if (own.empty()) continue;
-                std::vector<double> ths((size_t)R * own.size()), sums(own.size(), 0.0);
+                std::vector<double> ths((size_t)R * own.size()), zs((size_t)R * own.size()), sums(own.size(), 0.0);
                 std::vector<int> rcs(own.size(), 0);
                 for (size_t q = 0; q < own.size(); ++q)
-                    for (int i = 0; i < R; ++i) ths[q * R + i] = std::exp(Zs[own[q]][i]);
-                const int brc = mvn_loglik_batch(c, ths.data(), (int)own.size(), c.Uall.d(), c.Uall.ld, mall, sums.data(), rcs.data());
+                    for (int i = 0; i < R; ++i) { zs[q * R + i] = Zs[own[q]][i]; ths[q * R + i] = std::exp(Zs[own[q]][i]); }
+                const int brc = eval_round(memos.empty() ? nullptr : &memos[rr], zs.data(), ths.data(), (int)own.size(),
+                                           c.Uall.d(), c.Uall.ld, mall, sums.data(), rcs.data());
                 for (size_t q = 0; q < own.size(); ++q) {
                     const int j = own[q];
                     const int rc = (rcs[q] == MCML_OK && brc != MCML_OK) ? brc : rcs[q];
@@ -192,12 +219,15 @@
     int f_optim_batch(int width, double denomD)
     {
         const double fix_var_par = sigma;
+        ThetaScaleMemo memo;
+        const bool scale = scale_active();
+        if (scale) memo.reset(c.theta_scale_p, true);
         batch_objective_fn fb = [&](const std::vector<std::vector<double>>& Zs, std::vector<double>* F) -> int {
             const int nc = (int)Zs.size();
-            std::vector<double> ths((size_t)R * nc), sums(nc, 0.0);
+            std::vector<double> ths((size_t)R * nc), zs((size_t)R * nc), sums(nc, 0.0);
             std::vector<int> rcs(nc, 0);
-            for (int j = 0; j < nc; ++j) for (int i = 0; i < R; ++i) ths[(size_t)j * R + i] = std::exp(Zs[j][P + i]);
-            MCML_TRY(mvn_loglik_batch(c, ths.data(), nc, c.U.d(), c.U.ld, c.mcols, sums.data(), rcs.data()));
+            for (int j = 0; j < nc; ++j) for (int i = 0; i < R; ++i) { zs[(size_t)j * R + i] = Zs[j][P + i]; ths[(size_t)j * R + i] = std::exp(Zs[j][P + i]); }
+            MCML_TRY(eval_round(scale ? &memo : nullptr, zs.data(), ths.data(), nc, c.U.d(), c.U.ld, c.mcols, sums.data(), rcs.data()));
             F->assign(nc, 0.0);
             for (int j = 0; j < nc; ++j) {
                 model_var_par = fix_var_par;
@@ -256,7 +286,10 @@
             std::vector<double> ths((size_t)R * want.size()), sums(want.size(), 0.0);
             std::vector<int> rcs(want.size(), 0);
             for (size_t q = 0; q < want.size(); ++q) for (int i = 0; i < R; ++i) ths[q * R + i] = want[q][i];
-            MCML_TRY(mvn_loglik_batch(c, ths.data(), (int)want.size(), c.U.d(), c.U.ld, c.mcols, sums.data(), rcs.data()));
+            ThetaScaleMemo ts;
+            const bool scale = scale_active();
+            if (scale) ts.reset(c.theta_scale_p, false);
+            MCML_TRY(eval_round(scale ? &ts : nullptr, ths.data(), ths.data(), (int)want.size(), c.U.d(), c.U.ld, c.mcols, sums.data(), rcs.data()));
             for (size_t q = 0; q < want.size(); ++q)
                 (*memo)[want[q]] = rcs[q] == MCML_OK ? sums[q] / c.mcols : -HUGE_VAL;
         }
@@ -315,6 +348,22 @@
     MCML_REQUIRE(c.mcols > 0, "no samples u set");
     McmlOptim mc(c, start, trace, 0, 1.0);
     return mc.f_hess(tol, H);
+}
+
+int drv_theta_round(Ctx& c, const double* thetas, int k, double* out)
+{
+    MCML_REQUIRE(thetas && out && k >= 1 && k <= 64, "theta_round: bad argument");
+    MCML_REQUIRE(c.mcols > 0 && c.U.d(), "theta_round: no samples set");
+    const std::vector<double> start((size_t)c.P + c.cov.npar + 1, 0.0);
+    McmlOptim mc(c, start.data(), 0, 0, 1.0);
+    ThetaScaleMemo ts;
+    const bool scale = mc.scale_active();
+    if (scale) ts.reset(c.theta_scale_p, false);
+    std::vector<double> sums(k, 0.0);
+    std::vector<int> rcs(k, 0);
+    MCML_TRY(mc.eval_round(scale ? &ts : nullptr, thetas, thetas, k, c.U.d(), c.U.ld, c.mcols, sums.data(), rcs.data()));
+    for (int j = 0; j < k; ++j) out[j] = rcs[j] == MCML_OK ? sums[j] / c.mcols : NAN;
+    return MCML_OK;
 }
 
 int drv_aic(Ctx& c, const double* beta_par, int nbeta, const double* cov_par, int ncov, double* out)
diff --git a/glmmrmcml_amd/csrc/mvn.hip b/glmmrmcml_amd/csrc/mvn.hip
--- a/glmmrmcml_amd/csrc/mvn.hip
+++ b/glmmrmcml_amd/csrc/mvn.hip
@@ -2,6 +2,7 @@
 #include "dgemm_mfma.h"
 #include "dgemm_dl.h"
 #include "reduce.h"
+#include "theta_scale.h"
 
 namespace mcml {
 
@@ -480,6 +481,13 @@
     scal[0] += (double)mcols * (-0.5 * dim * LOG_2PI - 0.5 * scal[1]) - 0.5 * scal[2];
 }
 
+__global__ void k_accum_parts(const double* scal, int sstride, double* parts)
+{
+    const double* sj = scal + (size_t)threadIdx.x * sstride;
+    parts[2 * threadIdx.x] += sj[1];
+    parts[2 * threadIdx.x + 1] += sj[2];
+}
+
 __global__ void k_zero_upper(double* A, int lda, int n)
 {
     int i = blockIdx.x * blockDim.x + threadIdx.x;
@@ -487,7 +495,7 @@
     if (i < n && j < n && i < j) A[i + (size_t)j * lda] = 0.0;
 }
 
-struct Bat { int n = 1; size_t sA = 0, sL = 0; int* err = nullptr; };
+struct Bat { int n = 1; size_t sA = 0, sL = 0; int* err = nullptr; int round = 0; };
 
 template <bool BNMAJOR>
 static int chol_gemm(hipStream_t s, int M, int N, int K, const double* A, int lda, const double* B, int ldb,
@@ -556,7 +564,7 @@
     if (two) { MCML_TRY(lookahead_setup(c)); sL = c.aux; }
     const int nsteps = (n + CHOL_NB - 1) / CHOL_NB;
     constexpr int SPW = CHOL_NB * 8;
-    const bool twolevel = bt.n > 1 && n > SPW + CHOL_NB;
+    const bool twolevel = (bt.round ? bt.round : bt.n) > 1 && n > SPW + CHOL_NB;
     MCML_TRY(L.leaf(sM, 0, n < CHOL_NB ? n : CHOL_NB));
     bool forked = false;
     for (int t = 0; t < nsteps; ++t) {
@@ -812,6 +820,7 @@
 int mvn_setup(Ctx& c)
 {
     const CovSpec& cs = c.cov;
+    c.theta_scale_p = theta_scale_exponents(cs);
     MCML_TRY(c.d_cov.ensure(sizeof(int32_t) * cs.cov.size()));
     MCML_TRY(copy_h2d(c.d_cov.p, cs.cov.data(), sizeof(int32_t) * cs.cov.size(), c.stream));
     MCML_TRY(c.d_data.ensure(sizeof(double) * (cs.data.size() + 1)));
@@ -884,13 +893,14 @@
 }
 
 static int mvn_large_blocks(Ctx& c, DevMat& W, int kb, const ThetaArg* th, const double* Us, int ldu, int m,
-                            double* scal, int sstride, int* flags)
-{
+                            double* scal, int sstride, int* flags, int round = 0, double* parts = nullptr)
+{
+    const bool batch = (round ? round : kb) > 1;
     const CovSpec& cs = c.cov;
     const int32_t* dcov = c.d_cov.as<int32_t>();
     const CovBlock* dblk = c.d_blocks.as<CovBlock>();
     const int ld = W.ld, dmax = round_up(c.maxdim_large, 16);
-    Bat bt; bt.n = kb; bt.sA = (size_t)ld * dmax; bt.sL = linv_size(dmax); bt.err = flags;
+    Bat bt; bt.n = kb; bt.sA = (size_t)ld * dmax; bt.sL = linv_size(dmax); bt.err = flags; bt.round = round;
     ThetaBatch tb;
     memset(&tb, 0, sizeof tb);
     for (int j = 0; j < kb; ++j) tb.t[j] = th[j];
@@ -901,7 +911,7 @@
         const int dp = round_up(d, 16);
         c.mvn_ws[&W == &c.Dbatch] = Ctx::MvnWs{d, dp, m, ld, kb};
         const dim3 gb((dp + 63) / 64, (dp + 15) / 16, kb);
-        if (kb == 1)
+        if (!batch)
             hipLaunchKernelGGL(k_build_dense, gb, dim3(256), 0, c.stream, W.d(), ld, b, dblk, dcov, cs.rows, c.d_data.d(),
                                th[0], 0, dp);
         else
@@ -914,7 +924,7 @@
             for (int j = 0; j < kb; ++j)
                 MCML_HIP(hipMemset2DAsync(W.d() + j * bt.sA + dp + (size_t)d * ld, sizeof(double) * ld, 0, sizeof(double) * m, dp - d, c.stream));
         MCML_TRY(leaf_prepare(c, dmax, kb));
-        MCML_TRY(kb > 1 ? potrf_blocked(c, W.d(), ld, dp, m, bt) : potrf_graphed(c, W.d(), ld, dp, m, bt));
+        MCML_TRY(batch ? potrf_blocked(c, W.d(), ld, dp, m, bt) : potrf_graphed(c, W.d(), ld, dp, m, bt));
         const int gx = (m + 255) / 256, gy = d < 64 ? d : 64;
         MCML_TRY(c.partials.ensure(sizeof(double) * (size_t)(gx * gy + 16)));
         for (int j = 0; j < kb; ++j) {
@@ -925,6 +935,7 @@
             hipLaunchKernelGGL(k_logdet, dim3(1), dim3(256), 0, c.stream, Aj, ld, d, sj + 1);
             hipLaunchKernelGGL(k_finish_large, dim3(1), dim3(1), 0, c.stream, sj, d, m);
         }
+        if (parts) hipLaunchKernelGGL(k_accum_parts, dim3(1), dim3(kb), 0, c.stream, scal, sstride, parts);
         MCML_HIP(hipGetLastError());
     }
     return MCML_OK;
@@ -985,19 +996,12 @@
     return MCML_OK;
 }
 
-int mvn_loglik_batch(Ctx& c, const double* thetas, int k, const double* Us, int ldu, int m, double* sums, int* rcs)
-{
-    MCML_REQUIRE(k >= 1 && thetas && sums && rcs && m > 0 && Us, "mvn_ll batch: bad arguments");
+static bool mvn_batchable(const Ctx& c) { return c.maxdim_large > 0 && c.n_small == 0 && c.n_diag_rows == 0; }
+
+static int mvn_batch_pass(Ctx& c, const double* thetas, int k, int round, const double* Us, int ldu, int m, double* sums,
+                          int* rcs, double* parts)
+{
     const int R = c.cov.npar;
-    const bool batchable = k > 1 && c.maxdim_large > 0 && c.n_small == 0 && c.n_diag_rows == 0;
-    if (!batchable) {
-        int first_rc = MCML_OK;
-        for (int j = 0; j < k; ++j) {
-            rcs[j] = mvn_loglik_sum_on(c, thetas + (size_t)j * R, Us, ldu, m, sums + j);
-            if (rcs[j] != MCML_OK && rcs[j] != MCML_ENOTPD && first_rc == MCML_OK) first_rc = rcs[j];
-        }
-        return first_rc;
-    }
     for (int j0 = 0; j0 < k; j0 += MVN_MAXBATCH) {
         const int kb = (k - j0 < MVN_MAXBATCH) ? k - j0 : MVN_MAXBATCH;
         ThetaArg th[MVN_MAXBATCH];
@@ -1007,17 +1011,43 @@
             MCML_TRY(c.Dbatch.alloc(dmax + m, MVN_MAXBATCH * dmax));
             MCML_HIP(hipMemsetAsync(c.Dbatch.d(), 0, sizeof(double) * (size_t)c.Dbatch.ld * MVN_MAXBATCH * dmax, c.stream));
         }
-        MCML_TRY(c.bscal.ensure(sizeof(double) * 5 * MVN_MAXBATCH));
-        MCML_HIP(hipMemsetAsync(c.bscal.p, 0, sizeof(double) * 5 * MVN_MAXBATCH, c.stream));
+        MCML_TRY(c.bscal.ensure(sizeof(double) * 7 * MVN_MAXBATCH));
+        MCML_HIP(hipMemsetAsync(c.bscal.p, 0, sizeof(double) * 7 * MVN_MAXBATCH, c.stream));
         int* bflags = reinterpret_cast<int*>(c.bscal.d() + 4 * MVN_MAXBATCH);
-        MCML_TRY(mvn_large_blocks(c, c.Dbatch, kb, th, Us, ldu, m, c.bscal.d(), 4, bflags));
+        double* bparts = c.bscal.d() + 5 * MVN_MAXBATCH;
+        MCML_TRY(mvn_large_blocks(c, c.Dbatch, kb, th, Us, ldu, m, c.bscal.d(), 4, bflags, round, parts ? bparts : nullptr));
         double hs[4 * MVN_MAXBATCH]; int hf[MVN_MAXBATCH];
         MCML_TRY(copy_d2h(hs, c.bscal.p, sizeof(double) * 4 * kb, c.stream));
         MCML_TRY(copy_d2h(hf, bflags, sizeof(int) * kb, c.stream));
+        if (parts) MCML_TRY(copy_d2h(parts + 2 * (size_t)j0, bparts, sizeof(double) * 2 * kb, c.stream));
         MCML_HIP(hipStreamSynchronize(c.stream));
         for (int j = 0; j < kb; ++j) { sums[j0 + j] = hs[4 * j]; rcs[j0 + j] = hf[j] ? MCML_ENOTPD : MCML_OK; }
     }
     return MCML_OK;
+}
+
+int mvn_loglik_batch(Ctx& c, const double* thetas, int k, const double* Us, int ldu, int m, double* sums, int* rcs)
+{
+    MCML_REQUIRE(k >= 1 && thetas && sums && rcs && m > 0 && Us, "mvn_ll batch: bad arguments");
+    const int R = c.cov.npar;
+    const bool batchable = k > 1 && mvn_batchable(c);
+    if (!batchable) {
+        int first_rc = MCML_OK;
+        for (int j = 0; j < k; ++j) {
+            rcs[j] = mvn_loglik_sum_on(c, thetas + (size_t)j * R, Us, ldu, m, sums + j);
+            if (rcs[j] != MCML_OK && rcs[j] != MCML_ENOTPD && first_rc == MCML_OK) first_rc = rcs[j];
+        }
+        return first_rc;
+    }
+    return mvn_batch_pass(c, thetas, k, 0, Us, ldu, m, sums, rcs, nullptr);
+}
+
+int mvn_loglik_batch_parts(Ctx& c, const double* thetas, int k, int round, const double* Us, int ldu, int m, double* sums,
+                           int* rcs, double* parts)
+{
+    MCML_REQUIRE(k >= 1 && round >= k && round > 1 && thetas && sums && rcs && parts && m > 0 && Us, "mvn_ll batch parts: bad arguments");
+    MCML_REQUIRE(mvn_batchable(c), "mvn_ll batch parts: the model has blocks that are not factorised side by side");
+    return mvn_batch_pass(c, thetas, k, round, Us, ldu, m, sums, rcs, parts);
 }
 
 __global__ void k_diag_fill(double* L, int ldl, int Q, const int* rowblock, const CovBlock* blocks,
diff --git a/glmmrmcml_amd/csrc/theta_scale.h b/glmmrmcml_amd/csrc/theta_scale.h
--- /dev/null
+++ b/glmmrmcml_amd/csrc/theta_scale.h
@@ -0,0 +1,120 @@
+#pragma once
+#include "covspec.h"
+#include <cmath>
+#include <cstring>
+#include <map>
+
+namespace mcml {
+
+inline std::vector<int> theta_scale_exponents(const CovSpec& cs)
+{
+    std::vector<int> p(cs.npar > 0 ? cs.npar : 0, 0);
+    if (cs.blocks.empty() || p.empty()) return p;
+    std::vector<char> other(p.size(), 0);
+    std::vector<int> deg;
+    for (size_t b = 0; b < cs.blocks.size(); ++b) {
+        deg.assign(p.size(), 0);
+        for (int r = cs.blocks[b].r0; r < cs.blocks[b].r1; ++r) {
+            const int fn = cs.c(r, 2), pi = cs.c(r, 4), np = CovSpec::fn_npar(fn), e = CovSpec::fn_scale_exp(fn);
+            for (int q = 0; q < np; ++q) {
+                if (pi + q < 0 || pi + q >= (int)p.size()) return std::vector<int>(p.size(), 0);
+                if (q == 0 && e > 0) deg[pi] += e; else other[pi + q] = 1;
+            }
+        }
+        for (size_t i = 0; i < p.size(); ++i) {
+            if (b == 0) p[i] = deg[i];
+            else if (p[i] != deg[i]) p[i] = -1;
+        }
+    }
+    for (size_t i = 0; i < p.size(); ++i) if (p[i] < 0 || other[i]) p[i] = 0;
+    return p;
+}
+
+inline bool theta_scale_any(const std::vector<int>& p)
+{
+    for (int e : p) if (e > 0) return true;
+    return false;
+}
+
+inline double theta_scale_value(int dim, int m, double logdet, double sumsq)
+{
+    return (double)m * (-0.5 * dim * 1.8378770664093454835606594728112 - 0.5 * logdet) - 0.5 * sumsq;
+}
+
+struct ThetaScaleEntry { double logdet = 0, sumsq = 0; std::vector<double> zref; int rc = MCML_OK; };
+
+struct ThetaScaleMemo {
+    typedef std::vector<uint64_t> Key;
+    std::vector<int> p;
+    bool logcoords = true;
+    std::map<Key, ThetaScaleEntry> known;
+    long long factorised = 0;
+
+    void reset(const std::vector<int>& p_, bool logcoords_) { p = p_; logcoords = logcoords_; clear(); }
+    void clear() { known.clear(); }
+
+    Key key(const double* x) const
+    {
+        Key k;
+        for (size_t i = 0; i < p.size(); ++i)
+            if (p[i] == 0) { uint64_t u; memcpy(&u, x + i, sizeof u); k.push_back(u); }
+        return k;
+    }
+    std::vector<double> zscale(const double* x) const
+    {
+        std::vector<double> z(p.size(), 0.0);
+        for (size_t i = 0; i < p.size(); ++i) if (p[i] > 0) z[i] = logcoords ? x[i] : std::log(x[i]);
+        return z;
+    }
+
+    std::vector<int> plan(const double* X, int stride, int k) const
+    {
+        std::vector<int> reps;
+        if (!theta_scale_any(p)) { for (int j = 0; j < k; ++j) reps.push_back(j); return reps; }
+        std::map<Key, int> seen;
+        for (int j = 0; j < k; ++j) {
+            const Key kj = key(X + (size_t)j * stride);
+            if (known.count(kj) || seen.count(kj)) continue;
+            seen[kj] = j;
+            reps.push_back(j);
+        }
+        return reps;
+    }
+
+    void finish(const double* X, int stride, int k, const std::vector<int>& reps, const double* rep_sums,
+                const double* rep_parts, const int* rep_rcs, int dim, int m, double* sums, int* rcs)
+    {
+        factorised += (long long)reps.size();
+        if (!theta_scale_any(p)) {
+            for (size_t q = 0; q < reps.size(); ++q) { sums[reps[q]] = rep_sums[q]; rcs[reps[q]] = rep_rcs[q]; }
+            return;
+        }
+        std::vector<int> pos(k, -1);
+        for (size_t q = 0; q < reps.size(); ++q) {
+            const double* x = X + (size_t)reps[q] * stride;
+            pos[reps[q]] = (int)q;
+            ThetaScaleEntry e;
+            e.logdet = rep_parts[2 * q]; e.sumsq = rep_parts[2 * q + 1]; e.zref = zscale(x); e.rc = rep_rcs[q];
+            known[key(x)] = e;
+        }
+        for (int j = 0; j < k; ++j) {
+            if (pos[j] >= 0) { sums[j] = rep_sums[pos[j]]; rcs[j] = rep_rcs[pos[j]]; continue; }
+            const double* x = X + (size_t)j * stride;
+            const ThetaScaleEntry& e = known.find(key(x))->second;
+            rcs[j] = e.rc; sums[j] = 0.0;
+            if (e.rc != MCML_OK) continue;
+            const std::vector<double> z = zscale(x);
+            double lr = 0.0;
+            for (size_t i = 0; i < p.size(); ++i) if (p[i] > 0) lr += p[i] * (z[i] - e.zref[i]);
+            sums[j] = theta_scale_value(dim, m, e.logdet + dim * lr, e.sumsq * std::exp(-lr));
+        }
+    }
+};
+
+inline bool theta_scale_enabled()
+{
+    const char* e = getenv("GLMMR_MCML_THETA_SCALE");
+    return !(e && !strcmp(e, "0"));
+}
+
+}
diff --git a/include/glmmr_mcml_c.h b/include/glmmr_mcml_c.h
--- a/include/glmmr_mcml_c.h
+++ b/include/glmmr_mcml_c.h
@@ -253,6 +253,13 @@
 int glmmr_mcml_dbg_bobyqa_rounds(glmmr_mcml_batch_objective fb, void* user, int n, const double* x0, const double* lower,
                                  const double* upper, double rhobeg, double rhoend, int maxfun, int width,
                                  double* x_out, double* f_out, int* nfev_out, int* rounds_out);
+typedef int (*glmmr_mcml_parts_objective)(const double* X, int n, int k, double* logdet, double* sumsq, int* status,
+                                          void* user);
+int glmmr_mcml_dbg_theta_scale_rounds(glmmr_mcml_parts_objective fb, void* user, int n, const int* exps, int dim, int m,
+                                      int grouped, const double* x0, const double* lower, const double* upper,
+                                      double rhobeg, double rhoend, int maxfun, int width, double* x_out, double* f_out,
+                                      int* nfev_out, int* rounds_out, long long* factorised_out);
+int glmmr_mcml_dbg_theta_round(glmmr_mcml_ctx* ctx, const double* thetas, int k, double* out);
 int glmmr_mcml_dbg_copy_roundtrip(const double* in, long long ld_in, double* out, long long ld_out, long long rows, long long cols);
 int glmmr_mcml_dbg_fd_hessian(glmmr_mcml_objective f, void* user, int n, const double* x, double ndeps,
                               int usebounds, const double* lower, const double* upper, double* H);
```

After: 1162 (median of 6 runs). 2.0% higher.
